# FrozenWolf-Cyber/Indic-CL-ASR

Hardware: AMD Instinct MI355X
Metric: utterances/sec (15 s @16 kHz) Conformer-M RNNT-CTC+EWC train step (higher is better)
Workload: dtype bf16; 1 GPU; BASELINE configs[1]: Conformer-medium (d=256, 16L, H=640) hybrid RNNT-CTC + EWC, bs=32/GPU x 15 s, bf16 projections, freeze_encoder_till=12, 22x257 heads, fused_batch_size=4; global_batch=32, parallelism=dp1

## Files before the change

include/indicasr.h:

```cpp
#ifndef INDICASR_H
#define INDICASR_H

#include <stddef.h>
#include <stdint.h>

#ifdef __cplusplus
extern "C" {
#endif

typedef void* ia_stream_t;

enum ia_status {
    IA_OK = 0,
    IA_INVALID_VALUE = -1,
    IA_WORKSPACE_TOO_SMALL = -2,
    IA_LAUNCH_FAILED = -3,
    IA_UNSUPPORTED = -4,
};

const char* ia_version(void);

size_t ia_rnnt_workspace_bytes(int B, int T, int U1);
int ia_rnnt_loss(const float* logits, const int64_t* labels, const int64_t* act_lens, const int64_t* label_lens,
                 int B, int T, int U1, int V, int blank, float fastemit_lambda, float clamp,
                 float* costs, float* grads, void* workspace, size_t workspace_bytes, ia_stream_t stream);
int ia_rnnt_forward(const float* logits, const int64_t* labels, const int64_t* act_lens, const int64_t* label_lens,
                    int B, int T, int U1, int V, int blank, float fastemit_lambda, int need_backward, float* costs,
                    void* workspace, size_t workspace_bytes, ia_stream_t stream);
int ia_rnnt_backward(const float* logits, const int64_t* labels, const int64_t* act_lens, const int64_t* label_lens,
                     int B, int T, int U1, int V, int blank, float fastemit_lambda, float clamp,
                     const float* cost_grad, float* grads, void* workspace, size_t workspace_bytes, ia_stream_t stream,
                     void* grad_kernel_start_event, void* grad_kernel_stop_event);
int ia_rnnt_export_alphas_betas(const void* workspace, size_t workspace_bytes, const int64_t* act_lens,
                                const int64_t* label_lens, int B, int T, int U1, float* alphas, float* betas,
                                ia_stream_t stream);

int ia_joint_ld(int V);
int ia_joint_fwd(const void* f, const void* g, const void* W, const float* bias, const int64_t* labels,
                 const int64_t* act_lens, const int64_t* label_lens, int B, int T, int U1, int H, int V, int blank,
                 float dropout_p, unsigned seed, void* logits, int LD, void* workspace, size_t workspace_bytes,
                 ia_stream_t stream);
int ia_joint_fwd_box(const void* f, const void* g, const void* W, const float* bias, const int64_t* labels,
                     const int64_t* act_lens, const int64_t* label_lens, const int64_t* box_t, const int64_t* box_u, int B,
                     int T, int U1, int H, int V, int blank, float dropout_p, unsigned seed, void* logits, int LD,
                     void* workspace, size_t workspace_bytes, ia_stream_t stream);
int64_t ia_joint_extra_scratch_elems(void);
int ia_joint_extra_reduce(const void* logits, const void* teacher, const int64_t* box_t, const int64_t* box_u,
                          const float* w_sq, const float* w_kd, int B, int T, int U1, int V, int LD, float* sums4,
                          float* scratch, ia_stream_t stream);
int ia_joint_extra_grad(const void* logits, const void* teacher, const int64_t* box_t, const int64_t* box_u, const float* w_sq,
                        const float* w_kd, const float* upstream2, int B, int T, int U1, int V, int LD, void* E,
                        ia_stream_t stream);
int ia_lattice_add_f16(void* G, const void* E, int64_t n, ia_stream_t stream);
int ia_rnnt_lattice(const int64_t* act_lens, const int64_t* label_lens, int B, int T, int U1, float fastemit_lambda,
                    int need_backward, float* costs, void* workspace, size_t workspace_bytes, ia_stream_t stream);
int ia_joint_backward_g(void* logits_inout, const int64_t* labels, const int64_t* act_lens, const int64_t* label_lens,
                        int B, int T, int U1, int V, int LD, int blank, float fastemit_lambda, const float* cost_grad,
                        float kappa, void* gt_out, int S, int Kc, float* dbias_out, float* dbias_scratch, void* workspace,
                        size_t workspace_bytes, ia_stream_t stream, void* grad_kernel_start_event,
                        void* grad_kernel_stop_event);
int ia_joint_backward_g_skip(void* logits_inout, const int64_t* labels, const int64_t* act_lens, const int64_t* label_lens, int B,
                             int T, int U1, int V, int LD, int blank, float fastemit, const float* cost_grad, float kappa,
                             void* gt_out, int S, int Kc, float* dbias_out, float* dbias_scratch, void* workspace,
                             size_t workspace_bytes, int skip_dead_frames, ia_stream_t stream, void* ev_start, void* ev_stop);
int64_t ia_joint_backward_g_dbias_scratch_elems(int LD);
int ia_joint_hidden_t(const void* f, const void* g, void* hidden_t, int B, int T, int U1, int H, int LDH, int S, int Kc,
                      float dropout_p, unsigned seed, ia_stream_t stream);
int ia_joint_hidden(const void* f, const void* g, void* hidden, int B, int T, int U1, int H, int LDH, float dropout_p,
                    unsigned seed, ia_stream_t stream);
int ia_joint_dh_reduce(const void* dh, const void* f, const void* g, const int64_t* act_lens,
                       const int64_t* label_lens, float* df, float* dg, int B, int T, int U1, int H, float inv_kappa,
                       float dropout_p, unsigned seed, void* scratch, ia_stream_t stream);
size_t ia_joint_dh_reduce_scratch_bytes(int B, int T, int U1, int H);
int ia_joint_dh_fused_supported(int U1, int H, int LD);
int ia_joint_dh_k(void);
size_t ia_joint_dh_fused_scratch_bytes(int B, int T, int U1, int H);
int ia_joint_dh_fused(const void* G, const void* Wt, const void* f, const void* g, const int64_t* act_lens,
                      const int64_t* label_lens, float* df, float* dg, int B, int T, int U1, int H, int LD,
                      float inv_kappa, float dropout_p, unsigned seed, void* scratch, ia_stream_t stream);
int ia_joint_dh_fused_ex(const void* G, const void* Wt, const void* f, const void* g, const int64_t* act_lens,
                         const int64_t* label_lens, float* df, float* dg, void* df_bf16, void* dg_bf16, int zero_dead_df, int B,
                         int T, int U1, int H, int LD, float inv_kappa, float dropout_p, unsigned seed, void* scratch,
                         ia_stream_t stream);
int ia_joint_dw_fused_supported(int U1, int H, int LD);
int64_t ia_joint_dw_fused_scratch_elems(int B, int T, int U1, int H, int LD);
int ia_joint_dw_fused(const void* G, const void* f, const void* g, const int64_t* act_lens, int B, int T, int U1, int H, int LD,
                      float dropout_p, unsigned seed, float* dW, float* scratch, ia_stream_t stream);
int ia_joint_dw_fused_ex(const void* G, const void* f, const void* g, const int64_t* act_lens, const int64_t* label_lens, int B,
                         int T, int U1, int H, int LD, float dropout_p, unsigned seed, float* dW, float* scratch,
                         ia_stream_t stream);

int ia_gemm_bf16(const void* A, int lda, const void* W, int ldw, int M, int N, int K, const float* bias, int act,
                 float dropout_p, unsigned seed, float alpha, const float* R, int ldr, float* outF, int ldof,
                 void* outH, int ldoh, ia_stream_t stream);
int ia_gemm_bf16_ex(const void* A, int lda, const void* W, int ldw, int M, int N, int K, const float* bias, int act,
                    float dropout_p, unsigned seed, float alpha, const float* R, int ldr, float* outF, int ldof, void* outH,
                    int ldoh, void* out_pre, int ldpre, const void* aux, int ldaux, ia_stream_t stream);
int ia_gemm_bf16_ex2(const void* A, int lda, const void* W, int ldw, int M, int N, int K, const float* bias, int act,
                     float dropout_p, unsigned seed, float alpha, const float* R, int ldr, float* outF, int ldof, void* outH,
                     int ldoh, void* out_pre, int ldpre, const void* aux, int ldaux, int flags, ia_stream_t stream);
int ia_quantize_mxfp8(const void* x, int is_f32, int ld, int64_t M, int K, void* q, int ldq, void* scales, int lds, ia_stream_t stream);
int ia_gemm_mxfp8(const void* Aq, int lda, const void* a_scales, int ldsa, const void* Wq, int ldw, const void* w_scales, int ldsw,
                  int M, int N, int K, const float* bias, int act, float dropout_p, unsigned seed, float alpha, const float* R, int ldr,
                  float* outF, int ldof, void* outH, int ldoh, ia_stream_t stream);

int ia_greedy_decode_lds_bytes(int Hp, int Hj, int V);
int ia_greedy_rnnt_decode(const float* f_all, const int64_t* out_len, const float* EW, const float* Whh, const float* Wpred,
                          const float* bpred, const float* Whead, const float* bhead, int B, int T, int Hp, int Hj, int V,
                          int blank, int row_blank, int row_sos, int max_symbols, int* tokens, int cap, int* counts,
                          int* overflow, ia_stream_t stream);
int ia_greedy_rnnt_decode_bf16w(const float* f_all, const int64_t* out_len, const float* EW, const void* Whh_bf16,
                                const void* Wpred_bf16, const float* bpred, const void* Whead_bf16, const float* bhead, int B, int T,
                                int Hp, int Hj, int V, int blank, int row_blank, int row_sos, int max_symbols, int* tokens, int cap,
                                int* counts, int* overflow, ia_stream_t stream);
size_t ia_greedy_decode_scratch_bytes(int B, int Hp, int Hj);
int ia_greedy_decode_cluster(int B, int Hp, int Hj);
int ia_greedy_rnnt_decode_bf16w_ex(const float* f_all, const int64_t* out_len, const float* EW, const void* Whh_bf16,
                                   const void* Wpred_bf16, const float* bpred, const void* Whead_bf16, const float* bhead, int B,
                                   int T, int Hp, int Hj, int V, int blank, int row_blank, int row_sos, int max_symbols, int* tokens,
                                   int cap, int* counts, int* overflow, int cluster, void* scratch, size_t scratch_bytes,
                                   ia_stream_t stream);

int ia_edit_distance_batch(const int32_t* a, const int64_t* a_off, const int32_t* b, const int64_t* b_off, int n, int64_t* out);

int ia_quantize_fp8_rows(const void* x, int is_f32, int ld, int64_t M, int K, void* q, int ldq, float* scale, ia_stream_t stream);
int ia_gemm_fp8(const void* Aq, int lda, const float* a_scale, const void* Wq, int ldw, const float* w_scale, int M, int N, int K,
                const float* bias, int act, float dropout_p, unsigned seed, float alpha, const float* R, int ldr, float* outF,
                int ldof, void* outH, int ldoh, ia_stream_t stream);
int ia_subsample_conv1(const float* feats, int B, int Fm, int Tm, int C, const float* w1, const float* b1, void* out,
                       ia_stream_t stream);
int ia_subsample_conv2(const void* in_cl, int B, int T1, int F1, int C, const void* w2r, const float* b2, int N, void* out,
                       ia_stream_t stream);
int ia_gemm_bf16_ln_supported(int N, int K);
int ia_gemm_bf16_ln(const void* A, int lda, const void* W, int ldw, int M, int N, int K, const float* bias, float dropout_p,
                    unsigned seed, float alpha, const float* R, int ldr, float* outF, int ldof, const float* ln_g,
                    const float* ln_b, float ln_eps, void* outH, int ldoh, ia_stream_t stream);
int ia_layernorm(const float* x, int ldx, int N, int d, const float* g1, const float* b1, float eps, float* outF,
                 int ldf, const float* g2, const float* b2, void* outH, int ldh, ia_stream_t stream);
int ia_glu_dwconv(const void* x2, const int64_t* lens, int B, int T, int d, int ksz, const float* w, const float* bias,
                  float* z, float* bn_sum, float* bn_sumsq, float* scratch, ia_stream_t stream);
int64_t ia_dwconv_scratch_elems(int B, int T, int d, int ksz);
int ia_colsum_bf16(const void* x, int M, int N, int ld, float* out, ia_stream_t stream);
int ia_dwconv_time(const float* x, int B, int T, int d, int ksz, const float* w, const float* bias, int flip, float* y,
                   ia_stream_t stream);
int ia_dwconv_time_wgrad(const float* x, const float* dy, int B, int T, int d, int ksz, float* dw, float* db,
                         float* scratch, ia_stream_t stream);
int ia_dwconv_glu_bwd(const float* dz, const void* c2, const int64_t* lens, int B, int T, int d, int ksz, const float* w, void* dc2,
                      ia_stream_t stream);
int ia_dwconv_glu_wgrad(const void* c2, const int64_t* lens, const float* dy, int B, int T, int d, int ksz, float* dw, float* db,
                        float* scratch, ia_stream_t stream);
int ia_bn_silu(const float* z, int64_t n_rows, int d, const float* bn_sum, const float* bn_sumsq, const float* gamma,
               const float* beta, float* running_mean, float* running_var, int64_t* num_batches_tracked,
               float momentum, float eps, int training, void* out, ia_stream_t stream);

int ia_gemm_bnsilu_supported(int K);
int ia_gemm_bnsilu_bf16(const float* z, int ldz, int64_t n_rows, const float* bn_sum, const float* bn_sumsq,
                        const float* gamma, const float* beta, float* running_mean, float* running_var,
                        int64_t* num_batches_tracked, float momentum, float eps, int training, const void* W, int ldw, int M,
                        int N, int K, const float* bias, float dropout_p, unsigned seed, float alpha, const float* R, int ldr,
                        float* outF, int ldof, void* outH, int ldoh, const long long* bn_sums_fixed, ia_stream_t stream);
int ia_gemm_bnsilu_bf16_keep(const float* z, int ldz, int64_t n_rows, const float* bn_sum, const float* bn_sumsq,
                             const float* gamma, const float* beta, float* running_mean, float* running_var,
                             int64_t* num_batches_tracked, float momentum, float eps, int training, const void* W, int ldw, int M,
                             int N, int K, const float* bias, float dropout_p, unsigned seed, float alpha, const float* R, int ldr,
                             float* outF, int ldof, void* outH, int ldoh, const long long* bn_sums_fixed, void* outA, int ldoa,
                             ia_stream_t stream);
int ia_dwconv_gated_fixed(const void* g, const int64_t* lens, int B, int T, int d, int ksz, const float* w, const float* bias,
                          float* z, long long* bn_sums_fixed, ia_stream_t stream);
int ia_glu_dwconv_fixed(const void* x2, const int64_t* lens, int B, int T, int d, int ksz, const float* w, const float* bias,
                        float* z, long long* bn_sums_fixed, ia_stream_t stream);

int ia_relpos_attention_flash_supported(int T, int dk);
int ia_relpos_attention_flash(const void* qkv, const void* pos_proj, const float* bias_u, const float* bias_v,
                              const int64_t* lens, int B, int T, int H, int dk, float dropout_p, unsigned seed, void* ctx,
                              ia_stream_t stream);
int ia_relpos_attention_flash_lse(const void* qkv, const void* pos_proj, const float* bias_u, const float* bias_v,
                                  const int64_t* lens, int B, int T, int H, int dk, float dropout_p, unsigned seed, void* ctx,
                                  float* lse, ia_stream_t stream);
int ia_relpos_attention_flash_bwd_dims(int T, int* Rs, int* pad0);
int64_t ia_relpos_attention_flash_bwd_ws_elems(int B, int T, int H, int dk);
int ia_relpos_attention_flash_bwd(const void* qkv, const void* pos_proj, const float* bias_u, const float* bias_v,
                                  const int64_t* lens, const void* ctx, const void* dctx, const float* lse, int B, int T, int H,
                                  int dk, float dropout_p, unsigned seed, void* dqkv, void* dpl, int pl_rows, float* dbias_u,
                                  float* dbias_v, void* dBand, void* QvHM, float* ws, ia_stream_t stream);
size_t ia_attn_vt_elems(int B, int T, int H);
int ia_relpos_attention(const void* qkv, const void* pos_proj, const float* bias_u, const float* bias_v,
                        const int64_t* lens, int B, int T, int H, int dk, float dropout_p, unsigned seed,
                        void* vt_scratch, void* ctx, ia_stream_t stream);

size_t ia_lstm_scratch_bytes(int B, int H);
int ia_lstm_lds_bytes(int H, int backward);
int ia_lstm_forward(const float* Gx, const void* Whh_bf16, float* Hout, float* gates, float* Cs, int U, int B, int H,
                    void* scratch, size_t scratch_bytes, ia_stream_t stream);
int ia_lstm_backward(const float* dHout, const float* gates, const float* Cs, const void* WhhT_bf16, float* dG, int U,
                     int B, int H, void* scratch, size_t scratch_bytes, ia_stream_t stream);

int ia_feat_frames(const float* audio, int B, int L, int Tm, int win, int n_fft, int hop, float preemph, float dither,
                   unsigned seed, float* frames, int ldf, ia_stream_t stream);
int ia_gemm_f32(const float* A, int lda, const float* W, int ldw, int M, int N, int K, float* C, int ldc,
                ia_stream_t stream);
int ia_feat_power(const float* spec, int64_t M, int lds, int half, int nbins, float* power, int ldp, ia_stream_t stream);
int ia_feat_logmel_t(const float* mel, int B, int Tm, int F, int ldm, float guard, float* out, ia_stream_t stream);
int ia_feat_preemph(const float* audio, int B, int L, float preemph, float dither, unsigned seed, float* y,
                    ia_stream_t stream);
int ia_feat_logmel_fft_supported(int n_fft, int win, int n_mels, int n_chunks);
int ia_feat_logmel_fft(const float* y, int B, int L, int Tm, const float* window, int win, int n_fft, int hop,
                       const float* twiddle, const int* chunk_start, const float* chunk_vals, const int* filt_chunks,
                       int n_mels, int n_chunks, float guard, float* out, ia_stream_t stream);
int ia_feat_normalize(const float* x, const int64_t* seq_len, int B, int F, int T, float eps, const int* freq_starts,
                      const int* freq_widths, int n_freq_masks, const int* time_starts, const int* time_widths,
                      int n_time_masks, float mask_value, float* y, ia_stream_t stream);

size_t ia_ctc_workspace_bytes(int B, int T, int S);
int ia_ctc_forward(const float* log_probs, const int64_t* targets, const int64_t* input_lens, const int64_t* target_lens,
                   int B, int T, int V, int S, int blank, int zero_infinity, float* nll, void* workspace,
                   size_t workspace_bytes, ia_stream_t stream);
int ia_ctc_backward(const float* log_probs, const int64_t* targets, const int64_t* input_lens, const int64_t* target_lens,
                    int B, int T, int V, int S, int blank, const float* nll_grad, float* grad, void* workspace,
                    size_t workspace_bytes, ia_stream_t stream);

typedef struct ia_tn_problem {
    const void* dY; const void* X; float* dW; float* db;
    int ldy, ldx, M, n, k;
} ia_tn_problem;
int64_t ia_gemm_tn_grouped_scratch_elems(const ia_tn_problem* problems, int count);
int ia_gemm_tn_bf16_grouped(const ia_tn_problem* problems, int count, float* scratch, ia_stream_t stream);
int64_t ia_gemm_tn_scratch_elems(int M, int n, int k);
int ia_gemm_tn_bf16(const void* dY, int ldy, const void* X, int ldx, int M, int n, int k, float* dW, float* db,
                    float* scratch, ia_stream_t stream);

int ia_ffn_fused_supported(int d, int d_ff);
int ia_ffn_fused(float* x, int N, int d, int d_ff, const float* ln_g, const float* ln_b, float eps, const void* W1,
                 const float* b1, const void* W2, const float* b2, float alpha, float p_ff, unsigned seed_ff, float p_res,
                 unsigned seed_res, const float* ln2_g, const float* ln2_b, void* y_out, int ln2_to_y_only,
                 ia_stream_t stream);
int ia_ffn_fused_tail_supported(int d, int d_ff, int nt);
int ia_ffn_fused_tail(float* x, int N, int d, int d_ff, const float* ln_g, const float* ln_b, float eps, const void* W1,
                      const float* b1, const void* W2, const float* b2, float alpha, float p_ff, unsigned seed_ff, float p_res,
                      unsigned seed_res, const float* ln2_g, const float* ln2_b, void* y_out, int ln2_to_y_only, const void* Wt,
                      const float* bt, void* t_out, int nt, ia_stream_t stream);

typedef struct ia_block_params {
    const void *w_ff1a, *w_ff1b, *w_qkv, *w_pos, *w_out, *w_pw1, *w_pw2, *w_ff2a, *w_ff2b;
    const float *b_ff1a, *b_ff1b, *b_qkv, *b_out, *b_pw1, *b_pw2, *b_ff2a, *b_ff2b;
    const float *ln_ff1_g, *ln_ff1_b, *ln_att_g, *ln_att_b, *ln_conv_g, *ln_conv_b, *ln_ff2_g, *ln_ff2_b, *ln_out_g, *ln_out_b;
    const float *pos_u, *pos_v, *dw_w, *dw_b, *bn_g, *bn_b;
    float *bn_rm, *bn_rv;
    int64_t* bn_nbt;
    float ln_eps, bn_eps, bn_momentum, p_drop, p_ff, p_att, fc_factor;
    int d, d_ff, n_heads, ksz;
    const void* pl_cached;
    const void* w_pw1_glu;
    const float* b_pw1_glu;
} ia_block_params;
size_t ia_conformer_prefix_ws_bytes(int B, int T, int d, int d_ff, int H, int ksz, int pos_rows);
int ia_conformer_prefix_fwd(const ia_block_params* layers, int n_layers, float* x, const void* pos_emb, int pos_rows,
                            const int64_t* lens, int B, int T, unsigned seed_base, unsigned seed_stride, int training,
                            void* workspace, size_t workspace_bytes, ia_stream_t stream);
size_t ia_conformer_prefix_ws_sums_offset(int B, int T, int d, int d_ff, int H, int ksz, int pos_rows);
int ia_conformer_prefix_fwd_seg(const ia_block_params* layers, int n_layers, float* x, const void* pos_emb, int pos_rows,
                                const int64_t* lens, int B, int T, unsigned seed_base, unsigned seed_stride, int training,
                                int seg_begin, int seg_end, int bn_synced, void* workspace, size_t workspace_bytes,
                                ia_stream_t stream);

typedef struct ia_block_saved {
    void *y1, *h1p, *h1; float* x1;
    void *y2, *qkv, *pl, *ctxv; float* x2;
    void *y3, *c2; float *z, *sums; void* c3; float* x3;
    void *y4, *h4p, *h4; float* x4;
    float* lse;
} ia_block_saved;
typedef struct ia_block_grads {
    float *w_ff1a, *b_ff1a, *w_ff1b, *b_ff1b, *w_qkv, *b_qkv, *w_pos, *w_out, *b_out, *w_pw1, *b_pw1, *w_pw2, *b_pw2;
    float *w_ff2a, *b_ff2a, *w_ff2b, *b_ff2b;
    float *ln_ff1_g, *ln_ff1_b, *ln_att_g, *ln_att_b, *ln_conv_g, *ln_conv_b, *ln_ff2_g, *ln_ff2_b, *ln_out_g, *ln_out_b;
    float *dw_w, *dw_b, *bn_g, *bn_b;
} ia_block_grads;
struct ia_block_params;
int ia_conformer_block_supported(int d, int d_ff, int H, int ksz, int T);
size_t ia_conformer_block_bwd_ws_bytes(int B, int T, int d, int d_ff, int ksz);
int ia_conformer_block_fwd(const struct ia_block_params* layer, const float* x0, const void* pos_emb, int pos_rows,
                           const int64_t* lens, int B, int T, unsigned seed, const ia_block_saved* saved, float* out,
                           float* dw_scratch, ia_stream_t stream);
int ia_conformer_block_bwd_a(const struct ia_block_params* layer, const ia_block_saved* saved, const ia_block_grads* grads,
                             const float* dout, const int64_t* lens, int B, int T, unsigned seed, void* workspace,
                             size_t workspace_bytes, float** dx2_out, void** dctx_out, ia_stream_t stream);
int ia_conformer_block_fwd_phase(const struct ia_block_params* layer, const float* x0, const void* pos_emb, int pos_rows,
                                 const int64_t* lens, int B, int T, unsigned seed, const ia_block_saved* saved, float* out,
                                 float* dw_scratch, int phase, ia_stream_t stream);
int ia_conformer_block_bwd_a_phase(const struct ia_block_params* layer, const ia_block_saved* saved, const ia_block_grads* grads,
                                   const float* dout, const int64_t* lens, int B, int T, unsigned seed, void* workspace,
                                   size_t workspace_bytes, float** dx2_out, void** dctx_out, int phase, const float* bn_S12,
                                   ia_stream_t stream);
int ia_conformer_block_bwd_b(const struct ia_block_params* layer, const ia_block_saved* saved, const ia_block_grads* grads,
                             const float* x0, const void* pos_emb, int pos_rows, const void* dqkv, const void* dpl, int B,
                             int T, unsigned seed, void* workspace, size_t workspace_bytes, float* dx0,
                             const void* add_table, int n_add, ia_stream_t stream);

int ia_layernorm_bwd(const float* x, int ldx, const float* dy_f32, const void* dy_bf16, int ldy, int N, int d,
                     const float* gamma, float eps, const float* dx_in, float* dx_out, int lddx, float* dgamma,
                     float* dbeta, float* scratch, ia_stream_t stream);
int ia_layernorm_bwd_drop(const float* x, int ldx, const float* dy_f32, const void* dy_bf16, int ldy, int N, int d,
                          const float* gamma, float eps, const float* dx_in, float* dx_out, int lddx, float* dgamma,
                          float* dbeta, float alpha, float dropout_p, unsigned seed, void* dx_bf16, int lddxh, float* scratch,
                          ia_stream_t stream);
typedef struct ia_finish_job { const float* part; int G, C, C0; float* out0; float* out1; } ia_finish_job;
int ia_layernorm_bwd_partial_rows(int N);
int ia_partials_finish_multi(const ia_finish_job* jobs, int count, ia_stream_t stream);
int64_t ia_layernorm_bwd_scratch_elems(int N, int d);
int ia_silu_dropout(const void* h_pre, int64_t M, int N, float dropout_p, unsigned seed, void* out, ia_stream_t stream);
int ia_silu_dropout_bwd(const void* h_pre, const void* dh, int64_t M, int N, float dropout_p, unsigned seed, void* out,
                        ia_stream_t stream);
int ia_scale_dropout_bf16(const float* dy, int64_t M, int N, float alpha, float dropout_p, unsigned seed, void* out,
                          ia_stream_t stream);
int ia_cast_pad_bf16(const float* src, int lds, int64_t M, int N, void* dst, int ldd, ia_stream_t stream);
int ia_bn_silu_bwd(const float* z, const void* dc3, int64_t n_rows, int d, const float* bn_sum, const float* bn_sumsq,
                   const float* gamma, const float* beta, float eps, float* S1, float* S2, float* dz, float* scratch,
                   ia_stream_t stream);
int64_t ia_bn_silu_bwd_scratch_elems(int64_t n_rows, int d);
int ia_bn_sync_finish(float* sums_and_count, int d, int64_t n_local_rows, float* running_mean, float* running_var,
                      int64_t* num_batches_tracked, float momentum, ia_stream_t stream);
int ia_bn_silu_bwd_reduce(const float* z, const void* dc3, int64_t n_rows, int d, const float* bn_sum, const float* bn_sumsq,
                          const float* gamma, const float* beta, float eps, float* S1, float* S2, float* scratch,
                          ia_stream_t stream);
int ia_bn_silu_bwd_apply(const float* z, const void* dc3, int64_t n_rows, int d, const float* bn_sum, const float* bn_sumsq,
                         const float* gamma, const float* beta, float eps, const float* S1, const float* S2, float* dz,
                         ia_stream_t stream);
int ia_glu_mask(const void* c2, const int64_t* lens, int B, int T, int d, float* G, ia_stream_t stream);
int ia_glu_bwd(const void* c2, const float* dG, const int64_t* lens, int B, int T, int d, void* dc2, ia_stream_t stream);

int ia_cl_chunk_elems(void);
int ia_cl_penalty(const float* theta, const float* theta_star, const float* weight, float coef, float* grad,
                  int accumulate, const int32_t* chunk_table, int nchunks, const float* seg_inv_numel,
                  float* seg_abs_mean, float* penalty_sum, ia_stream_t stream);
int ia_cl_fisher_accumulate(float* fisher, const float* grad, const float* loss_scalar, int64_t n, ia_stream_t stream);
int ia_cl_abs_accumulate(float* omega, const float* grad, int64_t n, ia_stream_t stream);
int ia_adamw_step(float* theta, const float* grad, float* exp_avg, float* exp_avg_sq, int64_t n, float lr, float beta1,
                  float beta2, float eps, float weight_decay, int step, float grad_scale, void* shadow_bf16,
                  ia_stream_t stream);
int ia_adamw_step_segmented(float* theta, const float* grad, float* exp_avg, float* exp_avg_sq, const int32_t* chunk_table,
                            int nchunks, int32_t* seg_active, int32_t* seg_step, int nseg, int all_active, float lr,
                            float beta1, float beta2, float eps, float weight_decay, float grad_scale, void* shadow_bf16,
                            ia_stream_t stream);
size_t ia_grad_norm_workspace_bytes(int nchunks);
int ia_grad_norm(const float* grad, const int32_t* chunk_table, int nchunks, const int32_t* seg_chunk_begin, int nseg,
                 float grad_scale, float max_norm, int32_t* seg_active, float* seg_norm, float* norm_state, void* workspace,
                 size_t workspace_bytes, ia_stream_t stream);
int ia_adamw_step_segmented_clipped(float* theta, const float* grad, float* exp_avg, float* exp_avg_sq,
                                    const int32_t* chunk_table, int nchunks, int32_t* seg_active, int32_t* seg_step, int nseg,
                                    int all_active, float lr, float beta1, float beta2, float eps, float weight_decay,
                                    float grad_scale, void* shadow_bf16, const float* norm_state, int skip_nonfinite,
                                    int32_t* counters, ia_stream_t stream);
int ia_adamw_step_segmented_si(float* theta, const float* grad, float* exp_avg, float* exp_avg_sq, const int32_t* chunk_table,
                               int nchunks, int32_t* seg_active, int32_t* seg_step, int nseg, int all_active, float lr,
                               float beta1, float beta2, float eps, float weight_decay, float grad_scale, void* shadow_bf16,
                               const float* norm_state, int skip_nonfinite, int32_t* counters, float* path_w,
                               const float* omega, const float* theta_star, float penalty_coef, ia_stream_t stream);
int ia_si_consolidate(const float* theta, float* theta_star, float* path_w, float* omega, float xi, int64_t n,
                      ia_stream_t stream);
size_t ia_agem_workspace_bytes(int nchunks);
int ia_agem_dots(const float* grad, const float* ref, const int32_t* chunk_table, int nchunks, int nseg, float grad_scale,
                 int32_t* seg_active, float* proj_state, void* workspace, size_t workspace_bytes, ia_stream_t stream);
int ia_grad_norm_projected(const float* grad, const int32_t* chunk_table, int nchunks, const int32_t* seg_chunk_begin, int nseg,
                           float grad_scale, float max_norm, const int32_t* seg_active, float* seg_norm, float* norm_state,
                           void* workspace, size_t workspace_bytes, const float* ref, const float* proj_state,
                           ia_stream_t stream);
int ia_adamw_step_segmented_projected(float* theta, const float* grad, float* exp_avg, float* exp_avg_sq,
                                      const int32_t* chunk_table, int nchunks, int32_t* seg_active, int32_t* seg_step, int nseg,
                                      int all_active, float lr, float beta1, float beta2, float eps, float weight_decay,
                                      float grad_scale, void* shadow_bf16, const float* norm_state, int skip_nonfinite,
                                      int32_t* counters, const float* ref, const float* proj_state, int32_t* proj_counters,
                                      ia_stream_t stream);
#define IA_GEM_MAX_TASKS 16
#define IA_GEM_STATE_FLOATS 20
#define IA_GEM_SUMS_DOUBLES 272
size_t ia_gem_workspace_bytes(int nchunks, int max_tasks);
int ia_gem_dots(const float* x, const float* refs, int64_t stride, int ntasks, const int32_t* chunk_table, int nchunks, int nseg,
                float grad_scale, int32_t* seg_active, int gram_row, double* gem_sums, void* workspace, size_t workspace_bytes,
                ia_stream_t stream);
int ia_gem_solve(const double* gem_sums, float* gem_state, int ntasks, float memory_strength, float eps, ia_stream_t stream);
int ia_grad_norm_gem(const float* grad, const int32_t* chunk_table, int nchunks, const int32_t* seg_chunk_begin, int nseg,
                     float grad_scale, float max_norm, const int32_t* seg_active, float* seg_norm, float* norm_state,
                     void* workspace, size_t workspace_bytes, const float* refs, int64_t stride, int ntasks,
                     const float* gem_state, ia_stream_t stream);
int ia_adamw_step_segmented_gem(float* theta, const float* grad, float* exp_avg, float* exp_avg_sq, const int32_t* chunk_table,
                                int nchunks, int32_t* seg_active, int32_t* seg_step, int nseg, int all_active, float beta1,
                                float beta2, float eps, float grad_scale, void* shadow_bf16, const int32_t* seg_group, int ngroups,
                                const float* group_lr, const float* group_weight_decay, const float* norm_state,
                                int skip_nonfinite, int32_t* counters, const float* refs, int64_t stride, int ntasks,
                                const float* gem_state, int32_t* gem_counters, ia_stream_t stream);
#define IA_MAX_PARAM_GROUPS 64
int ia_adamw_step_segmented_grouped(float* theta, const float* grad, float* exp_avg, float* exp_avg_sq,
                                    const int32_t* chunk_table, int nchunks, int32_t* seg_active, int32_t* seg_step, int nseg,
                                    int all_active, float beta1, float beta2, float eps, float grad_scale, void* shadow_bf16,
                                    const int32_t* seg_group, int ngroups, const float* group_lr,
                                    const float* group_weight_decay, const float* norm_state, int skip_nonfinite,
                                    int32_t* counters, float* path_w, const float* omega, const float* theta_star,
                                    float penalty_coef, const float* ref, const float* proj_state, int32_t* proj_counters,
                                    ia_stream_t stream);
#define IA_MASK_FREE 0
#define IA_MASK_MASKED 1
#define IA_MASK_FROZEN 2
int ia_adamw_step_segmented_masked(float* theta, const float* grad, float* exp_avg, float* exp_avg_sq, const int32_t* chunk_table,
                                   int nchunks, int32_t* seg_active, int32_t* seg_step, int nseg, int all_active, float beta1,
                                   float beta2, float eps, float grad_scale, void* shadow_bf16, const int32_t* seg_group,
                                   int ngroups, const float* group_lr, const float* group_weight_decay, const float* norm_state,
                                   int skip_nonfinite, int32_t* counters, const float* base, float* scores,
                                   const int32_t* seg_kind, float threshold, ia_stream_t stream);
int ia_mask_pack(const float* scores, const int32_t* chunk_table, int nchunks, const int32_t* seg_kind, int nseg, float threshold,
                 uint64_t* bits, int64_t nwords, int32_t* seg_kept, ia_stream_t stream);
int ia_mask_apply(float* theta, const float* base, const uint64_t* bits, int64_t nwords, const int32_t* chunk_table, int nchunks,
                  const int32_t* seg_kind, int nseg, void* shadow_bf16, ia_stream_t stream);
int ia_adamw_step_segmented_packed(float* theta, const float* grad, float* exp_avg, float* exp_avg_sq, const int32_t* chunk_table,
                                   int nchunks, int32_t* seg_active, int32_t* seg_step, int nseg, int all_active, float beta1,
                                   float beta2, float eps, float grad_scale, void* shadow_bf16, const int32_t* seg_group,
                                   int ngroups, const float* group_lr, const float* group_weight_decay, const float* norm_state,
                                   int skip_nonfinite, int32_t* counters, const uint8_t* owner, const int32_t* seg_kind,
                                   int train_owner, ia_stream_t stream);
int ia_grad_norm_packed(const float* grad, const int32_t* chunk_table, int nchunks, const int32_t* seg_chunk_begin, int nseg,
                        float grad_scale, float max_norm, int32_t* seg_active, float* seg_norm, float* norm_state,
                        void* workspace, size_t workspace_bytes, const uint8_t* owner, const int32_t* seg_kind, int train_owner,
                        ia_stream_t stream);
size_t ia_pack_prune_workspace_bytes(int nseg);
int ia_pack_prune(float* theta, float* exp_avg, float* exp_avg_sq, uint8_t* owner, const int32_t* chunk_table, int nchunks,
                  const int32_t* seg_kind, int nseg, float fraction, int task, void* shadow_bf16, int32_t* seg_counts,
                  void* workspace, size_t workspace_bytes, ia_stream_t stream);
int ia_pack_apply(float* theta, const float* base, const uint8_t* owner, const int32_t* chunk_table, int nchunks,
                  const int32_t* seg_kind, int nseg, int lo, int hi, void* shadow_bf16, ia_stream_t stream);

int ia_ctc_row_lse(const float* logits, int ld, int64_t M, int V, float* lse, ia_stream_t stream);
int ia_ctc_forward_logits(const float* logits, int ld, const float* lse, const int64_t* targets, const int64_t* input_lens,
                          const int64_t* target_lens, int B, int T, int V, int S, int blank, int zero_infinity, float* nll,
                          void* workspace, size_t workspace_bytes, ia_stream_t stream);
int ia_ctc_backward_logits(const float* logits, int ld, const float* lse, const int64_t* targets, const int64_t* input_lens,
                           const int64_t* target_lens, int B, int T, int V, int S, int blank, const float* nll_grad,
                           float grad_scale, void* grad_bf16, int ldg, void* workspace, size_t workspace_bytes, ia_stream_t stream);

typedef struct ia_axpy_row {
    float* dst; const float* src; long long n; float scale; int pad;
} ia_axpy_row;
typedef struct ia_tr_job { const void* in; void* out; int rows, cols; } ia_tr_job;
int ia_transpose16_multi(const ia_tr_job* jobs_host, int njobs, ia_stream_t stream);
int ia_swap01_cast(const void* in, int in_bf16, int n0, int n1, int H, void* out, int out_bf16, ia_stream_t stream);
int ia_select_rows_cast(const float* W, int ldw, const float* bias, int row0, int nrows, int extra_row, int K, int rows_out,
                        float scale, int out_f16, void* out, void* outT, int ldt, float* bias_out, ia_stream_t stream);
int ia_rows_scatter_add(float* dst, int ldd, const float* src, int lds, int row0, int nrows, int extra_row, int K, float scale,
                        float* bias_dst, const float* bias_src, ia_stream_t stream);
int ia_loss_combine(const float* costs, const float* nll, int B, float ctc_weight, const int* flag0, const int* flag1,
                    const int* flag2, const int* flag3, float* out4, float* total, ia_stream_t stream);
int ia_loss_combine_bwd(const float* gout, int B, float ctc_weight, float* g_costs, float* g_nll, ia_stream_t stream);
int ia_embed_sos(const float* E, const int64_t* tokens, int B, int U, int H, int n_rows, int time_major, int out_bf16, void* out,
                 ia_stream_t stream);
int ia_embed_sos_bwd(const void* dX, int dx_bf16, const int64_t* tokens, int B, int U, int H, int n_rows, int pad_row,
                     int time_major, float scale, float* dE, ia_stream_t stream);
int ia_multi_axpy(const ia_axpy_row* rows_host, int nrows, int max_blocks_per_row, ia_stream_t stream);

int ia_peak_stream_copy(const void* src, void* dst, size_t bytes, ia_stream_t stream);
int ia_peak_mfma_bf16(float* sink, int workgroups, int iters, ia_stream_t stream);
double ia_peak_mfma_bf16_flops(int workgroups, int iters);

#ifdef __cplusplus
}
#endif
#endif
```

indic_cl_asr_amd/_lib.py:

```python
import ctypes
import os
import subprocess

_HERE = os.path.dirname(os.path.abspath(__file__))
LIB_PATH = os.environ.get("IA_LIB_PATH") or os.path.join(_HERE, "libindicasr_hip.so")

IA_OK = 0
_STATUS = {-1: "IA_INVALID_VALUE", -2: "IA_WORKSPACE_TOO_SMALL", -3: "IA_LAUNCH_FAILED", -4: "IA_UNSUPPORTED"}

_c = ctypes
_vp, _i, _f, _sz = _c.c_void_p, _c.c_int, _c.c_float, _c.c_size_t
_i64 = _c.c_int64

class BlockParams(_c.Structure):
    _fields_ = ([(n, _c.c_void_p) for n in (
        "w_ff1a", "w_ff1b", "w_qkv", "w_pos", "w_out", "w_pw1", "w_pw2", "w_ff2a", "w_ff2b",
        "b_ff1a", "b_ff1b", "b_qkv", "b_out", "b_pw1", "b_pw2", "b_ff2a", "b_ff2b",
        "ln_ff1_g", "ln_ff1_b", "ln_att_g", "ln_att_b", "ln_conv_g", "ln_conv_b", "ln_ff2_g", "ln_ff2_b", "ln_out_g", "ln_out_b",
        "pos_u", "pos_v", "dw_w", "dw_b", "bn_g", "bn_b", "bn_rm", "bn_rv", "bn_nbt")]
        + [(n, _c.c_float) for n in ("ln_eps", "bn_eps", "bn_momentum", "p_drop", "p_ff", "p_att", "fc_factor")]
        + [(n, _c.c_int) for n in ("d", "d_ff", "n_heads", "ksz")]
        + [("pl_cached", _c.c_void_p), ("w_pw1_glu", _c.c_void_p), ("b_pw1_glu", _c.c_void_p)])


class BlockSaved(_c.Structure):
    _fields_ = [(n, _c.c_void_p) for n in ("y1", "h1p", "h1", "x1", "y2", "qkv", "pl", "ctxv", "x2", "y3", "c2", "z", "sums",
                                           "c3", "x3", "y4", "h4p", "h4", "x4", "lse")]


class TnProblem(_c.Structure):
    _fields_ = [("dY", _c.c_void_p), ("X", _c.c_void_p), ("dW", _c.c_void_p), ("db", _c.c_void_p),
                ("ldy", _c.c_int), ("ldx", _c.c_int), ("M", _c.c_int), ("n", _c.c_int), ("k", _c.c_int)]


class BlockGrads(_c.Structure):
    _fields_ = [(n, _c.c_void_p) for n in (
        "w_ff1a", "b_ff1a", "w_ff1b", "b_ff1b", "w_qkv", "b_qkv", "w_pos", "w_out", "b_out", "w_pw1", "b_pw1", "w_pw2", "b_pw2",
        "w_ff2a", "b_ff2a", "w_ff2b", "b_ff2b",
        "ln_ff1_g", "ln_ff1_b", "ln_att_g", "ln_att_b", "ln_conv_g", "ln_conv_b", "ln_ff2_g", "ln_ff2_b", "ln_out_g", "ln_out_b",
        "dw_w", "dw_b", "bn_g", "bn_b")]


SIGNATURES = {
    "ia_version": (_c.c_char_p, []),
    "ia_gemm_bf16_ex2": (_i, [_vp, _i, _vp, _i, _i, _i, _i, _vp, _i, _f, _c.c_uint, _f, _vp, _i, _vp, _i, _vp, _i, _vp, _i, _vp, _i, _i, _vp]),
    "ia_transpose16_multi": (_i, [_vp, _i, _vp]),
    "ia_swap01_cast": (_i, [_vp, _i, _i, _i, _i, _vp, _i, _vp]),
    "ia_ctc_row_lse": (_i, [_vp, _i, _i64, _i, _vp, _vp]),
    "ia_ctc_forward_logits": (_i, [_vp, _i, _vp, _vp, _vp, _vp, _i, _i, _i, _i, _i, _i, _vp, _vp, _sz, _vp]),
    "ia_ctc_backward_logits": (_i, [_vp, _i, _vp, _vp, _vp, _vp, _i, _i, _i, _i, _i, _vp, _f, _vp, _i, _vp, _sz, _vp]),
    "ia_select_rows_cast": (_i, [_vp, _i, _vp, _i, _i, _i, _i, _i, _f, _i, _vp, _vp, _i, _vp, _vp]),
    "ia_rows_scatter_add": (_i, [_vp, _i, _vp, _i, _i, _i, _i, _i, _f, _vp, _vp, _vp]),
    "ia_loss_combine": (_i, [_vp, _vp, _i, _f, _vp, _vp, _vp, _vp, _vp, _vp, _vp]),
    "ia_loss_combine_bwd": (_i, [_vp, _i, _f, _vp, _vp, _vp]),
    "ia_embed_sos": (_i, [_vp, _vp, _i, _i, _i, _i, _i, _i, _vp, _vp]),
    "ia_embed_sos_bwd": (_i, [_vp, _i, _vp, _i, _i, _i, _i, _i, _i, _f, _vp, _vp]),
    "ia_multi_axpy": (_i, [_vp, _i, _i, _vp]),
    "ia_peak_stream_copy": (_i, [_vp, _vp, _sz, _vp]),
    "ia_peak_mfma_bf16": (_i, [_vp, _i, _i, _vp]),
    "ia_peak_mfma_bf16_flops": (_c.c_double, [_i, _i]),
    "ia_rnnt_workspace_bytes": (_sz, [_i, _i, _i]),
    "ia_rnnt_loss": (_i, [_vp, _vp, _vp, _vp, _i, _i, _i, _i, _i, _f, _f, _vp, _vp, _vp, _sz, _vp]),
    "ia_rnnt_forward": (_i, [_vp, _vp, _vp, _vp, _i, _i, _i, _i, _i, _f, _i, _vp, _vp, _sz, _vp]),
    "ia_rnnt_backward": (_i, [_vp, _vp, _vp, _vp, _i, _i, _i, _i, _i, _f, _f, _vp, _vp, _vp, _sz, _vp, _vp, _vp]),
    "ia_rnnt_export_alphas_betas": (_i, [_vp, _sz, _vp, _vp, _i, _i, _i, _vp, _vp, _vp]),
    "ia_joint_ld": (_i, [_i]),
    "ia_joint_fwd": (_i, [_vp, _vp, _vp, _vp, _vp, _vp, _vp, _i, _i, _i, _i, _i, _i, _f, _c.c_uint, _vp, _i, _vp, _sz, _vp]),
    "ia_joint_fwd_box": (_i, [_vp, _vp, _vp, _vp, _vp, _vp, _vp, _vp, _vp, _i, _i, _i, _i, _i, _i, _f, _c.c_uint, _vp, _i, _vp, _sz, _vp]),
    "ia_joint_extra_scratch_elems": (_i64, []),
    "ia_joint_extra_reduce": (_i, [_vp, _vp, _vp, _vp, _vp, _vp, _i, _i, _i, _i, _i, _vp, _vp, _vp]),
    "ia_joint_extra_grad": (_i, [_vp, _vp, _vp, _vp, _vp, _vp, _vp, _i, _i, _i, _i, _i, _vp, _vp]),
    "ia_lattice_add_f16": (_i, [_vp, _vp, _i64, _vp]),
    "ia_relpos_attention_flash_lse": (_i, [_vp, _vp, _vp, _vp, _vp, _i, _i, _i, _i, _f, _c.c_uint, _vp, _vp, _vp]),
    "ia_relpos_attention_flash_bwd_dims": (_i, [_i, _c.POINTER(_c.c_int), _c.POINTER(_c.c_int)]),
    "ia_relpos_attention_flash_bwd_ws_elems": (_i64, [_i, _i, _i, _i]),
    "ia_relpos_attention_flash_bwd": (_i, [_vp, _vp, _vp, _vp, _vp, _vp, _vp, _vp, _i, _i, _i, _i, _f, _c.c_uint, _vp, _vp, _i, _vp,
                                           _vp, _vp, _vp, _vp, _vp]),
    "ia_quantize_fp8_rows": (_i, [_vp, _i, _i, _i64, _i, _vp, _i, _vp, _vp]),
    "ia_gemm_fp8": (_i, [_vp, _i, _vp, _vp, _i, _vp, _i, _i, _i, _vp, _i, _f, _c.c_uint, _f, _vp, _i, _vp, _i, _vp, _i, _vp]),
    "ia_gemm_tn_grouped_scratch_elems": (_i64, [_vp, _i]),
    "ia_gemm_tn_bf16_grouped": (_i, [_vp, _i, _vp, _vp]),
    "ia_greedy_decode_lds_bytes": (_i, [_i, _i, _i]),
    "ia_greedy_rnnt_decode": (_i, [_vp, _vp, _vp, _vp, _vp, _vp, _vp, _vp, _i, _i, _i, _i, _i, _i, _i, _i, _i, _vp, _i, _vp, _vp, _vp]),
    "ia_greedy_rnnt_decode_bf16w": (_i, [_vp, _vp, _vp, _vp, _vp, _vp, _vp, _vp, _i, _i, _i, _i, _i, _i, _i, _i, _i, _vp, _i, _vp, _vp, _vp]),
    "ia_edit_distance_batch": (_i, [_vp, _vp, _vp, _vp, _i, _vp]),
    "ia_greedy_decode_scratch_bytes": (_sz, [_i, _i, _i]),
    "ia_greedy_decode_cluster": (_i, [_i, _i, _i]),
    "ia_greedy_rnnt_decode_bf16w_ex": (_i, [_vp, _vp, _vp, _vp, _vp, _vp, _vp, _vp, _i, _i, _i, _i, _i, _i, _i, _i, _i, _vp, _i, _vp, _vp, _i, _vp, _sz, _vp]),
    "ia_quantize_mxfp8": (_i, [_vp, _i, _i, _i64, _i, _vp, _i, _vp, _i, _vp]),
    "ia_gemm_mxfp8": (_i, [_vp, _i, _vp, _i, _vp, _i, _vp, _i, _i, _i, _i, _vp, _i, _f, _c.c_uint, _f, _vp, _i, _vp, _i, _vp, _i, _vp]),
    "ia_cast_pad_bf16": (_i, [_vp, _i, _i64, _i, _vp, _i, _vp]),
    "ia_rnnt_lattice": (_i, [_vp, _vp, _i, _i, _i, _f, _i, _vp, _vp, _sz, _vp]),
    "ia_joint_backward_g": (_i, [_vp, _vp, _vp, _vp, _i, _i, _i, _i, _i, _i, _f, _vp, _f, _vp, _i, _i, _vp, _vp, _vp, _sz, _vp, _vp,
                                 _vp]),
    "ia_joint_backward_g_skip": (_i, [_vp, _vp, _vp, _vp, _i, _i, _i, _i, _i, _i, _f, _vp, _f, _vp, _i, _i, _vp, _vp, _vp, _sz, _i, _vp,
                                      _vp, _vp]),
    "ia_joint_backward_g_dbias_scratch_elems": (_i64, [_i]),
    "ia_joint_hidden_t": (_i, [_vp, _vp, _vp, _i, _i, _i, _i, _i, _i, _i, _f, _c.c_uint, _vp]),
    "ia_joint_hidden": (_i, [_vp, _vp, _vp, _i, _i, _i, _i, _i, _f, _c.c_uint, _vp]),
    "ia_joint_dh_reduce": (_i, [_vp, _vp, _vp, _vp, _vp, _vp, _vp, _i, _i, _i, _i, _f, _f, _c.c_uint, _vp, _vp]),
    "ia_joint_dh_reduce_scratch_bytes": (_sz, [_i, _i, _i, _i]),
    "ia_joint_dh_fused_supported": (_i, [_i, _i, _i]),
    "ia_joint_dh_k": (_i, []),
    "ia_joint_dh_fused": (_i, [_vp, _vp, _vp, _vp, _vp, _vp, _vp, _vp, _i, _i, _i, _i, _i, _f, _f, _c.c_uint, _vp, _vp]),
    "ia_joint_dh_fused_ex": (_i, [_vp, _vp, _vp, _vp, _vp, _vp, _vp, _vp, _vp, _vp, _i, _i, _i, _i, _i, _i, _f, _f, _c.c_uint, _vp, _vp]),
    "ia_joint_dh_fused_scratch_bytes": (_sz, [_i, _i, _i, _i]),
    "ia_joint_dw_fused_supported": (_i, [_i, _i, _i]),
    "ia_joint_dw_fused_scratch_elems": (_i64, [_i, _i, _i, _i, _i]),
    "ia_joint_dw_fused": (_i, [_vp, _vp, _vp, _vp, _i, _i, _i, _i, _i, _f, _c.c_uint, _vp, _vp, _vp]),
    "ia_gemm_bf16_ln_supported": (_i, [_i, _i]),
    "ia_gemm_bf16_ln": (_i, [_vp, _i, _vp, _i, _i, _i, _i, _vp, _f, _c.c_uint, _f, _vp, _i, _vp, _i, _vp, _vp, _f, _vp, _i, _vp]),
    "ia_joint_dw_fused_ex": (_i, [_vp, _vp, _vp, _vp, _vp, _i, _i, _i, _i, _i, _f, _c.c_uint, _vp, _vp, _vp]),
    "ia_gemm_bf16": (_i, [_vp, _i, _vp, _i, _i, _i, _i, _vp, _i, _f, _c.c_uint, _f, _vp, _i, _vp, _i, _vp, _i, _vp]),
    "ia_gemm_bf16_ex": (_i, [_vp, _i, _vp, _i, _i, _i, _i, _vp, _i, _f, _c.c_uint, _f, _vp, _i, _vp, _i, _vp, _i, _vp, _i, _vp, _i, _vp]),
    "ia_subsample_conv1": (_i, [_vp, _i, _i, _i, _i, _vp, _vp, _vp, _vp]),
    "ia_subsample_conv2": (_i, [_vp, _i, _i, _i, _i, _vp, _vp, _i, _vp, _vp]),
    "ia_layernorm": (_i, [_vp, _i, _i, _i, _vp, _vp, _f, _vp, _i, _vp, _vp, _vp, _i, _vp]),
    "ia_glu_dwconv": (_i, [_vp, _vp, _i, _i, _i, _i, _vp, _vp, _vp, _vp, _vp, _vp, _vp]),
    "ia_dwconv_scratch_elems": (_i64, [_i, _i, _i, _i]),
    "ia_colsum_bf16": (_i, [_vp, _i, _i, _i, _vp, _vp]),
    "ia_dwconv_time": (_i, [_vp, _i, _i, _i, _i, _vp, _vp, _i, _vp, _vp]),
    "ia_dwconv_time_wgrad": (_i, [_vp, _vp, _i, _i, _i, _i, _vp, _vp, _vp, _vp]),
    "ia_dwconv_glu_bwd": (_i, [_vp, _vp, _vp, _i, _i, _i, _i, _vp, _vp, _vp]),
    "ia_dwconv_glu_wgrad": (_i, [_vp, _vp, _vp, _i, _i, _i, _i, _vp, _vp, _vp, _vp]),
    "ia_bn_silu": (_i, [_vp, _i64, _i, _vp, _vp, _vp, _vp, _vp, _vp, _vp, _f, _f, _i, _vp, _vp]),
    "ia_gemm_bnsilu_supported": (_i, [_i]),
    "ia_gemm_bnsilu_bf16": (_i, [_vp, _i, _i64, _vp, _vp, _vp, _vp, _vp, _vp, _vp, _f, _f, _i, _vp, _i, _i, _i, _i, _vp, _f, _c.c_uint, _f,
                                 _vp, _i, _vp, _i, _vp, _i, _vp, _vp]),
    "ia_gemm_bnsilu_bf16_keep": (_i, [_vp, _i, _i64, _vp, _vp, _vp, _vp, _vp, _vp, _vp, _f, _f, _i, _vp, _i, _i, _i, _i, _vp, _f, _c.c_uint,
                                      _f, _vp, _i, _vp, _i, _vp, _i, _vp, _vp, _i, _vp]),
    "ia_glu_dwconv_fixed": (_i, [_vp, _vp, _i, _i, _i, _i, _vp, _vp, _vp, _vp, _vp]),
    "ia_dwconv_gated_fixed": (_i, [_vp, _vp, _i, _i, _i, _i, _vp, _vp, _vp, _vp, _vp]),
    "ia_attn_vt_elems": (_sz, [_i, _i, _i]),
    "ia_relpos_attention": (_i, [_vp, _vp, _vp, _vp, _vp, _i, _i, _i, _i, _f, _c.c_uint, _vp, _vp, _vp]),
    "ia_relpos_attention_flash_supported": (_i, [_i, _i]),
    "ia_relpos_attention_flash": (_i, [_vp, _vp, _vp, _vp, _vp, _i, _i, _i, _i, _f, _c.c_uint, _vp, _vp]),
    "ia_lstm_scratch_bytes": (_sz, [_i, _i]),
    "ia_lstm_lds_bytes": (_i, [_i, _i]),
    "ia_lstm_forward": (_i, [_vp, _vp, _vp, _vp, _vp, _i, _i, _i, _vp, _sz, _vp]),
    "ia_lstm_backward": (_i, [_vp, _vp, _vp, _vp, _vp, _i, _i, _i, _vp, _sz, _vp]),
    "ia_feat_frames": (_i, [_vp, _i, _i, _i, _i, _i, _i, _f, _f, _c.c_uint, _vp, _i, _vp]),
    "ia_gemm_f32": (_i, [_vp, _i, _vp, _i, _i, _i, _i, _vp, _i, _vp]),
    "ia_feat_power": (_i, [_vp, _i64, _i, _i, _i, _vp, _i, _vp]),
    "ia_feat_logmel_t": (_i, [_vp, _i, _i, _i, _i, _f, _vp, _vp]),
    "ia_feat_preemph": (_i, [_vp, _i, _i, _f, _f, _c.c_uint, _vp, _vp]),
    "ia_feat_logmel_fft_supported": (_i, [_i, _i, _i, _i]),
    "ia_feat_logmel_fft": (_i, [_vp, _i, _i, _i, _vp, _i, _i, _i, _vp, _vp, _vp, _vp, _i, _i, _f, _vp, _vp]),
    "ia_feat_normalize": (_i, [_vp, _vp, _i, _i, _i, _f, _vp, _vp, _i, _vp, _vp, _i, _f, _vp, _vp]),
    "ia_ctc_workspace_bytes": (_sz, [_i, _i, _i]),
    "ia_ctc_forward": (_i, [_vp, _vp, _vp, _vp, _i, _i, _i, _i, _i, _i, _vp, _vp, _sz, _vp]),
    "ia_ctc_backward": (_i, [_vp, _vp, _vp, _vp, _i, _i, _i, _i, _i, _vp, _vp, _vp, _sz, _vp]),
    "ia_gemm_tn_scratch_elems": (_i64, [_i, _i, _i]),
    "ia_gemm_tn_bf16": (_i, [_vp, _i, _vp, _i, _i, _i, _i, _vp, _vp, _vp, _vp]),
    "ia_ffn_fused_supported": (_i, [_i, _i]),
    "ia_ffn_fused": (_i, [_vp, _i, _i, _i, _vp, _vp, _f, _vp, _vp, _vp, _vp, _f, _f, _c.c_uint, _f, _c.c_uint, _vp, _vp, _vp, _i, _vp]),
    "ia_ffn_fused_tail_supported": (_i, [_i, _i, _i]),
    "ia_ffn_fused_tail": (_i, [_vp, _i, _i, _i, _vp, _vp, _f, _vp, _vp, _vp, _vp, _f, _f, _c.c_uint, _f, _c.c_uint, _vp, _vp, _vp, _i,
                               _vp, _vp, _vp, _i, _vp]),
    "ia_conformer_prefix_ws_bytes": (_sz, [_i, _i, _i, _i, _i, _i, _i]),
    "ia_conformer_prefix_ws_sums_offset": (_sz, [_i, _i, _i, _i, _i, _i, _i]),
    "ia_conformer_prefix_fwd_seg": (_i, [_vp, _i, _vp, _vp, _i, _vp, _i, _i, _c.c_uint, _c.c_uint, _i, _i, _i, _i, _vp, _sz, _vp]),
    "ia_conformer_prefix_fwd": (_i, [_vp, _i, _vp, _vp, _i, _vp, _i, _i, _c.c_uint, _c.c_uint, _i, _vp, _sz, _vp]),
    "ia_conformer_block_supported": (_i, [_i, _i, _i, _i, _i]),
    "ia_conformer_block_bwd_ws_bytes": (_sz, [_i, _i, _i, _i, _i]),
    "ia_conformer_block_fwd": (_i, [_vp, _vp, _vp, _i, _vp, _i, _i, _c.c_uint, _vp, _vp, _vp, _vp]),
    "ia_conformer_block_fwd_phase": (_i, [_vp, _vp, _vp, _i, _vp, _i, _i, _c.c_uint, _vp, _vp, _vp, _i, _vp]),
    "ia_conformer_block_bwd_a": (_i, [_vp, _vp, _vp, _vp, _vp, _i, _i, _c.c_uint, _vp, _sz, _vp, _vp, _vp]),
    "ia_conformer_block_bwd_a_phase": (_i, [_vp, _vp, _vp, _vp, _vp, _i, _i, _c.c_uint, _vp, _sz, _vp, _vp, _i, _vp, _vp]),
    "ia_conformer_block_bwd_b": (_i, [_vp, _vp, _vp, _vp, _vp, _i, _vp, _vp, _i, _i, _c.c_uint, _vp, _sz, _vp, _vp, _i, _vp]),
    "ia_layernorm_bwd": (_i, [_vp, _i, _vp, _vp, _i, _i, _i, _vp, _f, _vp, _vp, _i, _vp, _vp, _vp, _vp]),
    "ia_layernorm_bwd_drop": (_i, [_vp, _i, _vp, _vp, _i, _i, _i, _vp, _f, _vp, _vp, _i, _vp, _vp, _f, _f, _c.c_uint, _vp, _i, _vp, _vp]),
    "ia_layernorm_bwd_partial_rows": (_i, [_i]),
    "ia_partials_finish_multi": (_i, [_vp, _i, _vp]),
    "ia_layernorm_bwd_scratch_elems": (_i64, [_i, _i]),
    "ia_silu_dropout": (_i, [_vp, _i64, _i, _f, _c.c_uint, _vp, _vp]),
    "ia_silu_dropout_bwd": (_i, [_vp, _vp, _i64, _i, _f, _c.c_uint, _vp, _vp]),
    "ia_scale_dropout_bf16": (_i, [_vp, _i64, _i, _f, _f, _c.c_uint, _vp, _vp]),
    "ia_bn_silu_bwd": (_i, [_vp, _vp, _i64, _i, _vp, _vp, _vp, _vp, _f, _vp, _vp, _vp, _vp, _vp]),
    "ia_bn_silu_bwd_scratch_elems": (_i64, [_i64, _i]),
    "ia_bn_sync_finish": (_i, [_vp, _i, _i64, _vp, _vp, _vp, _f, _vp]),
    "ia_bn_silu_bwd_reduce": (_i, [_vp, _vp, _i64, _i, _vp, _vp, _vp, _vp, _f, _vp, _vp, _vp, _vp]),
    "ia_bn_silu_bwd_apply": (_i, [_vp, _vp, _i64, _i, _vp, _vp, _vp, _vp, _f, _vp, _vp, _vp, _vp]),
    "ia_glu_mask": (_i, [_vp, _vp, _i, _i, _i, _vp, _vp]),
    "ia_glu_bwd": (_i, [_vp, _vp, _vp, _i, _i, _i, _vp, _vp]),
    "ia_cl_chunk_elems": (_i, []),
    "ia_cl_penalty": (_i, [_vp, _vp, _vp, _f, _vp, _i, _vp, _i, _vp, _vp, _vp, _vp]),
    "ia_cl_fisher_accumulate": (_i, [_vp, _vp, _vp, _i64, _vp]),
    "ia_cl_abs_accumulate": (_i, [_vp, _vp, _i64, _vp]),
    "ia_adamw_step": (_i, [_vp, _vp, _vp, _vp, _i64, _f, _f, _f, _f, _f, _i, _f, _vp, _vp]),
    "ia_adamw_step_segmented": (_i, [_vp, _vp, _vp, _vp, _vp, _i, _vp, _vp, _i, _i, _f, _f, _f, _f, _f, _f, _vp, _vp]),
    "ia_grad_norm_workspace_bytes": (_sz, [_i]),
    "ia_grad_norm": (_i, [_vp, _vp, _i, _vp, _i, _f, _f, _vp, _vp, _vp, _vp, _sz, _vp]),
    "ia_adamw_step_segmented_clipped": (_i, [_vp, _vp, _vp, _vp, _vp, _i, _vp, _vp, _i, _i, _f, _f, _f, _f, _f, _f, _vp, _vp, _i,
                                             _vp, _vp]),
    "ia_adamw_step_segmented_si": (_i, [_vp, _vp, _vp, _vp, _vp, _i, _vp, _vp, _i, _i, _f, _f, _f, _f, _f, _f, _vp, _vp, _i,
                                        _vp, _vp, _vp, _vp, _f, _vp]),
    "ia_si_consolidate": (_i, [_vp, _vp, _vp, _vp, _f, _i64, _vp]),
    "ia_agem_workspace_bytes": (_sz, [_i]),
    "ia_agem_dots": (_i, [_vp, _vp, _vp, _i, _i, _f, _vp, _vp, _vp, _sz, _vp]),
    "ia_grad_norm_projected": (_i, [_vp, _vp, _i, _vp, _i, _f, _f, _vp, _vp, _vp, _vp, _sz, _vp, _vp, _vp]),
    "ia_adamw_step_segmented_projected": (_i, [_vp, _vp, _vp, _vp, _vp, _i, _vp, _vp, _i, _i, _f, _f, _f, _f, _f, _f, _vp, _vp, _i,
                                               _vp, _vp, _vp, _vp, _vp]),
    "ia_gem_workspace_bytes": (_sz, [_i, _i]),
    "ia_gem_dots": (_i, [_vp, _vp, _i64, _i, _vp, _i, _i, _f, _vp, _i, _vp, _vp, _sz, _vp]),
    "ia_gem_solve": (_i, [_vp, _vp, _i, _f, _f, _vp]),
    "ia_grad_norm_gem": (_i, [_vp, _vp, _i, _vp, _i, _f, _f, _vp, _vp, _vp, _vp, _sz, _vp, _i64, _i, _vp, _vp]),
    "ia_adamw_step_segmented_gem": (_i, [_vp, _vp, _vp, _vp, _vp, _i, _vp, _vp, _i, _i, _f, _f, _f, _f, _vp, _vp, _i, _vp, _vp,
                                         _vp, _i, _vp, _vp, _i64, _i, _vp, _vp, _vp]),
    "ia_adamw_step_segmented_grouped": (_i, [_vp, _vp, _vp, _vp, _vp, _i, _vp, _vp, _i, _i, _f, _f, _f, _f, _vp, _vp, _i, _vp, _vp,
                                             _vp, _i, _vp, _vp, _vp, _vp, _f, _vp, _vp, _vp, _vp]),
    "ia_adamw_step_segmented_masked": (_i, [_vp, _vp, _vp, _vp, _vp, _i, _vp, _vp, _i, _i, _f, _f, _f, _f, _vp, _vp, _i, _vp, _vp,
                                            _vp, _i, _vp, _vp, _vp, _vp, _f, _vp]),
    "ia_mask_pack": (_i, [_vp, _vp, _i, _vp, _i, _f, _vp, _i64, _vp, _vp]),
    "ia_mask_apply": (_i, [_vp, _vp, _vp, _i64, _vp, _i, _vp, _i, _vp, _vp]),
    "ia_adamw_step_segmented_packed": (_i, [_vp, _vp, _vp, _vp, _vp, _i, _vp, _vp, _i, _i, _f, _f, _f, _f, _vp, _vp, _i, _vp, _vp,
                                            _vp, _i, _vp, _vp, _vp, _i, _vp]),
    "ia_grad_norm_packed": (_i, [_vp, _vp, _i, _vp, _i, _f, _f, _vp, _vp, _vp, _vp, _sz, _vp, _vp, _i, _vp]),
    "ia_pack_prune_workspace_bytes": (_sz, [_i]),
    "ia_pack_prune": (_i, [_vp, _vp, _vp, _vp, _vp, _i, _vp, _i, _f, _i, _vp, _vp, _vp, _sz, _vp]),
    "ia_pack_apply": (_i, [_vp, _vp, _vp, _vp, _i, _vp, _i, _i, _i, _vp, _vp]),
}

_lib = None


def build(verbose=False):
    out = None if verbose else subprocess.DEVNULL
    subprocess.check_call(["make", "-C", os.path.join(_HERE, "csrc")], stdout=out)


def lib():
    global _lib
    if _lib is None:
        if not os.path.exists(LIB_PATH):
            raise RuntimeError(
                f"{LIB_PATH} is missing: the HIP extension is the product path and has no fallback. "
                "Build it with `python -c 'import __graft_entry__ as g; g.build()'` or `make -C indic_cl_asr_amd/csrc`.")
        import torch
        l = ctypes.CDLL(LIB_PATH)
        for name, (res, args) in SIGNATURES.items():
            fn = getattr(l, name)
            fn.restype, fn.argtypes = res, args
        _lib = l
    return _lib


def check(status, what):
    if status != IA_OK:
        raise RuntimeError(f"{what} failed with status {status} ({_STATUS.get(status, 'unknown')})")


def version():
    return lib().ia_version().decode()


def stream_ptr():
    import torch
    return ctypes.c_void_p(torch.cuda.current_stream().cuda_stream)


def ptr(t):
    return ctypes.c_void_p(t.data_ptr()) if t is not None else None
```

indic_cl_asr_amd/csrc/block_train.hip:

```cpp
#include <hip/hip_bf16.h>
#include <hip/hip_runtime.h>

#include <cstdint>

#include <cstdlib>

#include "ia_common.h"

namespace {

inline size_t up256(size_t x) { return (x + 255) / 256 * 256; }

#define IA_TRY(call)                  \
    do {                              \
        const int rc_ = (call);       \
        if (rc_ != IA_OK) return rc_; \
    } while (0)

__global__ __launch_bounds__(256) void transpose_bf16_kernel(const unsigned short* __restrict__ in, int rows, int cols,
                                                             unsigned short* __restrict__ out) {
    __shared__ unsigned short tile[64][72];
    const int tiles_c = (cols + 63) / 64;
    const int tr = blockIdx.x / tiles_c, tc = blockIdx.x - tr * tiles_c;
    const int r0 = tr * 64, c0 = tc * 64;
    for (int i = threadIdx.x; i < 64 * 8; i += 256) {
        const int r = i >> 3, v = i & 7;
        uint4 x = make_uint4(0, 0, 0, 0);
        if (r0 + r < rows && c0 + v * 8 < cols) x = *reinterpret_cast<const uint4*>(in + (size_t)(r0 + r) * cols + c0 + v * 8);
        *reinterpret_cast<uint4*>(&tile[r][v * 8]) = x;
    }
    __syncthreads();
    for (int i = threadIdx.x; i < 64 * 8; i += 256) {
        const int c = i >> 3, v = i & 7;
        if (c0 + c < cols && r0 + v * 8 < rows) {
            union { uint4 u; unsigned short h[8]; } o;
#pragma unroll
            for (int j = 0; j < 8; ++j) o.h[j] = tile[v * 8 + j][c];
            *reinterpret_cast<uint4*>(out + (size_t)(c0 + c) * rows + r0 + v * 8) = o.u;
        }
    }
}

int transpose_bf16(const void* in, int rows, int cols, void* out, hipStream_t st) {
    if (rows % 8 != 0 || cols % 8 != 0) return IA_UNSUPPORTED;
    const int grid = ((rows + 63) / 64) * ((cols + 63) / 64);
    hipLaunchKernelGGL(transpose_bf16_kernel, dim3(grid), dim3(256), 0, st, (const unsigned short*)in, rows, cols, (unsigned short*)out);
    IA_RETURN_IF_LAUNCH_FAILED();
    return IA_OK;
}

struct TrJob { const unsigned short* in; unsigned short* out; int rows, cols, tile_begin, tiles_c; };
struct TrJobs { TrJob j[8]; int count; };
__global__ __launch_bounds__(256) void transpose_bf16_multi_kernel(TrJobs jobs) {
    __shared__ unsigned short tile[64][72];
    int ji = 0;
#pragma unroll
    for (int i = 1; i < 8; ++i)
        if (i < jobs.count && (int)blockIdx.x >= jobs.j[i].tile_begin) ji = i;
    const TrJob& J = jobs.j[ji];
    const int local = blockIdx.x - J.tile_begin;
    const int tr = local / J.tiles_c, tc = local - tr * J.tiles_c;
    const int r0 = tr * 64, c0 = tc * 64, rows = J.rows, cols = J.cols;
    for (int i = threadIdx.x; i < 64 * 8; i += 256) {
        const int r = i >> 3, v = i & 7;
        uint4 x = make_uint4(0, 0, 0, 0);
        if (r0 + r < rows && c0 + v * 8 < cols) x = *reinterpret_cast<const uint4*>(J.in + (size_t)(r0 + r) * cols + c0 + v * 8);
        *reinterpret_cast<uint4*>(&tile[r][v * 8]) = x;
    }
    __syncthreads();
    for (int i = threadIdx.x; i < 64 * 8; i += 256) {
        const int c = i >> 3, v = i & 7;
        if (c0 + c < cols && r0 + v * 8 < rows) {
            union { uint4 u; unsigned short h[8]; } o;
#pragma unroll
            for (int j = 0; j < 8; ++j) o.h[j] = tile[v * 8 + j][c];
            *reinterpret_cast<uint4*>(J.out + (size_t)(c0 + c) * rows + r0 + v * 8) = o.u;
        }
    }
}
struct TrList { TrJobs jobs; int tiles; };
inline void tr_add(TrList* l, const void* in, int rows, int cols, void* out) {
    TrJob& J = l->jobs.j[l->jobs.count++];
    J.in = (const unsigned short*)in; J.out = (unsigned short*)out; J.rows = rows; J.cols = cols;
    J.tile_begin = l->tiles; J.tiles_c = (cols + 63) / 64;
    l->tiles += ((rows + 63) / 64) * J.tiles_c;
}
int tr_launch(const TrList& l, hipStream_t st) {
    for (int i = 0; i < l.jobs.count; ++i)
        if (l.jobs.j[i].rows % 8 != 0 || l.jobs.j[i].cols % 8 != 0) return IA_UNSUPPORTED;
    hipLaunchKernelGGL(transpose_bf16_multi_kernel, dim3(l.tiles), dim3(256), 0, st, l.jobs);
    IA_RETURN_IF_LAUNCH_FAILED();
    return IA_OK;
}

struct AddRow { float* dst; const float* src; int64_t n; };
__global__ __launch_bounds__(256) void multi_add_kernel(const AddRow* __restrict__ table, int rows) {
    for (int k = blockIdx.y; k < rows; k += gridDim.y) {
        const AddRow r = table[k];
        const int64_t n4 = ((reinterpret_cast<uintptr_t>(r.dst) | reinterpret_cast<uintptr_t>(r.src)) & 15) ? 0 : (r.n >> 2);
        for (int64_t i = (int64_t)blockIdx.x * 256 + threadIdx.x; i < n4; i += (int64_t)gridDim.x * 256) {
            float4 a = reinterpret_cast<float4*>(r.dst)[i];
            const float4 b = reinterpret_cast<const float4*>(r.src)[i];
            a.x += b.x; a.y += b.y; a.z += b.z; a.w += b.w;
            reinterpret_cast<float4*>(r.dst)[i] = a;
        }
        for (int64_t i = (n4 << 2) + (int64_t)blockIdx.x * 256 + threadIdx.x; i < r.n; i += (int64_t)gridDim.x * 256) r.dst[i] += r.src[i];
    }
}

struct BwdWs {
    size_t dxa, dxb, dB, dB1, dB2, dB3, dh, dhp, dy, dc3, dz, dG, dc2, dctx, wt, scr, total;
};

size_t max3(size_t a, size_t b, size_t c) { return a > b ? (a > c ? a : c) : (b > c ? b : c); }

BwdWs bwd_ws(int B, int T, int d, int d_ff, int ksz) {
    const size_t N = (size_t)B * T;
    BwdWs w;
    size_t o = 0;
    w.dxa = o;  o = up256(o + N * d * 4);
    w.dxb = o;  o = up256(o + N * d * 4);
    w.dB = o;   o = up256(o + N * d * 2);
    w.dB1 = o;  o = up256(o + N * d * 2);
    w.dB2 = o;  o = up256(o + N * d * 2);
    w.dB3 = o;  o = up256(o + N * d * 2);
    w.dh = o;   o = up256(o + N * d_ff * 2);
    w.dhp = o;  o = up256(o + N * d_ff * 2);
    w.dy = o;   o = up256(o + N * d * 2);
    w.dc3 = o;  o = up256(o + N * d * 2);
    w.dz = o;   o = up256(o + N * d * 4);
    w.dG = o;   o = up256(o + (size_t)5 * (size_t)ia_layernorm_bwd_scratch_elems((int)N, d) * 4);
    w.dc2 = o;  o = up256(o + N * 2 * d * 2);
    w.dctx = o; o = up256(o + N * d * 2);
    w.wt = o;   o = up256(o + ((size_t)4 * d_ff * d + (size_t)7 * d * d) * 2);
    size_t scr = (size_t)ia_layernorm_bwd_scratch_elems((int)N, d);
    const int shapes[5][2] = {{d, d_ff}, {d_ff, d}, {d, d}, {2 * d, d}, {3 * d, d}};
    for (int i = 0; i < 5; ++i) {
        const size_t e = (size_t)ia_gemm_tn_scratch_elems((int)N, shapes[i][0], shapes[i][1]);
        scr = e > scr ? e : scr;
    }
    scr = max3(scr, (size_t)ia_bn_silu_bwd_scratch_elems((int64_t)N, d), (size_t)ia_dwconv_scratch_elems(B, T, d, ksz));
    {
        const ia_tn_problem ga[5] = {{nullptr, nullptr, nullptr, nullptr, d, d_ff, (int)N, d, d_ff},
                                     {nullptr, nullptr, nullptr, nullptr, d_ff, d, (int)N, d_ff, d},
                                     {nullptr, nullptr, nullptr, nullptr, d, d, (int)N, d, d},
                                     {nullptr, nullptr, nullptr, nullptr, 2 * d, d, (int)N, 2 * d, d},
                                     {nullptr, nullptr, nullptr, nullptr, d, d, (int)N, d, d}};
        const ia_tn_problem gb[4] = {{nullptr, nullptr, nullptr, nullptr, 3 * d, d, (int)N, 3 * d, d},
                                     {nullptr, nullptr, nullptr, nullptr, d, d, (int)(N > (size_t)64 * 512 ? N : (size_t)64 * 512), d, d},
                                     {nullptr, nullptr, nullptr, nullptr, d, d_ff, (int)N, d, d_ff},
                                     {nullptr, nullptr, nullptr, nullptr, d_ff, d, (int)N, d_ff, d}};
        scr = max3(scr, (size_t)ia_gemm_tn_grouped_scratch_elems(ga, 5), (size_t)ia_gemm_tn_grouped_scratch_elems(gb, 4));
        scr = max3(scr, (size_t)ia_gemm_tn_grouped_scratch_elems(gb, 2), (size_t)ia_gemm_tn_grouped_scratch_elems(gb + 2, 2));
        ia_tn_problem gall[9];
        for (int i = 0; i < 5; ++i) gall[i] = ga[i];
        for (int i = 0; i < 4; ++i) gall[5 + i] = gb[i];
        scr = scr > (size_t)ia_gemm_tn_grouped_scratch_elems(gall, 9) ? scr : (size_t)ia_gemm_tn_grouped_scratch_elems(gall, 9);
    }
    w.scr = o;  o = up256(o + scr * 4);
    w.total = o;
    return w;
}

int linear_bwd(const void* dY, const void* X, const void* W, int M, int n, int k, void* dX, float* dW, float* db, void* wt,
               float* scr, ia_stream_t stream) {
    if (dX) {
        IA_TRY(transpose_bf16(W, n, k, wt, (hipStream_t)stream));
        IA_TRY(ia_gemm_bf16(dY, n, wt, n, M, k, n, nullptr, 0, 0.f, 0, 1.f, nullptr, 0, nullptr, 0, dX, k, stream));
    }
    return ia_gemm_tn_bf16(dY, n, X, k, M, n, k, dW, db, scr, stream);
}

bool tn_grouping_enabled() {
    static const bool on = [] { const char* e = getenv("IA_TN_GROUPED"); return !(e && e[0] == '0'); }();
    return on;
}
int flush_group(const ia_tn_problem* grp, int ngrp, float* scr, ia_stream_t stream) {
    if (tn_grouping_enabled()) return ia_gemm_tn_bf16_grouped(grp, ngrp, scr, stream);
    for (int i = 0; i < ngrp; ++i)
        IA_TRY(ia_gemm_tn_bf16(grp[i].dY, grp[i].ldy, grp[i].X, grp[i].ldx, grp[i].M, grp[i].n, grp[i].k, grp[i].dW, grp[i].db, scr, stream));
    return IA_OK;
}
int linear_bwd_deferred(const void* dY, const void* X, const void* W, int M, int n, int k, void* dX, float* dW, float* db, const void* wt,
                        ia_tn_problem* grp, int* ngrp, ia_stream_t stream) {
    (void)W;
    if (dX) IA_TRY(ia_gemm_bf16(dY, n, wt, n, M, k, n, nullptr, 0, 0.f, 0, 1.f, nullptr, 0, nullptr, 0, dX, k, stream));
    grp[*ngrp] = ia_tn_problem{dY, X, dW, db, n, k, M, n, k};
    ++*ngrp;
    return IA_OK;
}

struct SideCtx {
    hipStream_t s = nullptr;
    hipEvent_t ev[8] = {};
    bool ok = false, tried = false;
    bool a_pending = false;
};
SideCtx* side_ctx() {
    static SideCtx ctx[16];
    const char* e = getenv("IA_WGRAD_SIDE");
    if (!(e && e[0] == '1')) return nullptr;
    int dev = 0;
    if (hipGetDevice(&dev) != hipSuccess || dev < 0 || dev >= 16) return nullptr;
    SideCtx& c = ctx[dev];
    if (!c.tried) {
        c.tried = true;
        bool ok = hipStreamCreateWithFlags(&c.s, hipStreamNonBlocking) == hipSuccess;
        for (int i = 0; ok && i < 8; ++i) ok = hipEventCreateWithFlags(&c.ev[i], hipEventDisableTiming) == hipSuccess;
        c.ok = ok;
    }
    return c.ok ? &c : nullptr;
}
struct PendingGroup { ia_tn_problem grp[8]; int n = 0; const void* ws = nullptr; };
PendingGroup* pending_group() {
    static PendingGroup pg[16];
    int dev = 0;
    if (hipGetDevice(&dev) != hipSuccess || dev < 0 || dev >= 16) return nullptr;
    return &pg[dev];
}
bool merged_wgrads() {
    const char* e = getenv("IA_TN_MERGE");
    return !(e && e[0] == '0') && tn_grouping_enabled();
}

int stream_after(hipStream_t from, hipStream_t to, hipEvent_t ev) {
    if (hipEventRecord(ev, from) != hipSuccess || hipStreamWaitEvent(to, ev, 0) != hipSuccess) return IA_LAUNCH_FAILED;
    return IA_OK;
}

}

extern "C" size_t ia_conformer_block_bwd_ws_bytes(int B, int T, int d, int d_ff, int ksz) {
    if (B <= 0 || T <= 0 || d <= 0 || d_ff <= 0 || ksz <= 0) return 0;
    return bwd_ws(B, T, d, d_ff, ksz).total;
}

extern "C" int ia_conformer_block_supported(int d, int d_ff, int H, int ksz, int T) {
    if (d <= 0 || H <= 0 || d % H != 0) return 0;
    const int dk = d / H;
    return (d % 8 == 0 && d <= 1024 && d_ff % 8 == 0 && ksz <= 31 && (ksz & 1) == 1 && dk <= 64 && dk % 4 == 0 && T >= 1) ? 1 : 0;
}

extern "C" int ia_conformer_block_fwd(const ia_block_params* Lp, const float* x0, const void* pos_emb, int pos_rows,
                                      const int64_t* lens, int B, int T, unsigned seed, const ia_block_saved* Sp, float* out,
                                      float* dw_scratch, ia_stream_t stream) {
    return ia_conformer_block_fwd_phase(Lp, x0, pos_emb, pos_rows, lens, B, T, seed, Sp, out, dw_scratch, 0, stream);
}

extern "C" int ia_conformer_block_fwd_phase(const ia_block_params* Lp, const float* x0, const void* pos_emb, int pos_rows,
                                            const int64_t* lens, int B, int T, unsigned seed, const ia_block_saved* Sp,
                                            float* out, float* dw_scratch, int phase, ia_stream_t stream) {
    if (phase < 0 || phase > 2) return IA_INVALID_VALUE;
    if (!Lp || !x0 || !pos_emb || !lens || !Sp || !out || !dw_scratch || B <= 0 || T <= 0) return IA_INVALID_VALUE;
    const ia_block_params& L = *Lp;
    const ia_block_saved& S = *Sp;
    const int d = L.d, d_ff = L.d_ff, H = L.n_heads, dk = d / (H > 0 ? H : 1), ksz = L.ksz, N = B * T;
    if (!ia_conformer_block_supported(d, d_ff, H, ksz, T) || pos_rows < 2 * T - 1) return IA_UNSUPPORTED;
    const float p = L.p_drop, pff = L.p_ff, patt = L.p_att;
    if (phase != 2) {
    IA_TRY(ia_layernorm(x0, d, N, d, L.ln_ff1_g, L.ln_ff1_b, L.ln_eps, nullptr, 0, nullptr, nullptr, S.y1, d, stream));
    IA_TRY(ia_gemm_bf16_ex(S.y1, d, L.w_ff1a, d, N, d_ff, d, L.b_ff1a, 1, pff, seed + 1, 1.f, nullptr, 0, nullptr, 0, S.h1, d_ff,
                           S.h1p, d_ff, nullptr, 0, stream));
    IA_TRY(ia_gemm_bf16(S.h1, d_ff, L.w_ff1b, d_ff, N, d, d_ff, L.b_ff1b, 0, p, seed + 2, L.fc_factor, x0, d, S.x1, d, nullptr, 0, stream));
    IA_TRY(ia_layernorm(S.x1, d, N, d, L.ln_att_g, L.ln_att_b, L.ln_eps, nullptr, 0, nullptr, nullptr, S.y2, d, stream));
    IA_TRY(ia_gemm_bf16(S.y2, d, L.w_qkv, d, N, 3 * d, d, L.b_qkv, 0, 0.f, 0, 1.f, nullptr, 0, nullptr, 0, S.qkv, 3 * d, stream));
    IA_TRY(ia_gemm_bf16(pos_emb, d, L.w_pos, d, pos_rows, d, d, nullptr, 0, 0.f, 0, 1.f, nullptr, 0, nullptr, 0, S.pl, d, stream));
    IA_TRY(ia_relpos_attention_flash_lse(S.qkv, S.pl, L.pos_u, L.pos_v, lens, B, T, H, dk, patt, seed + 7, S.ctxv, S.lse, stream));
    IA_TRY(ia_gemm_bf16(S.ctxv, d, L.w_out, d, N, d, d, L.b_out, 0, p, seed + 3, 1.f, S.x1, d, S.x2, d, nullptr, 0, stream));
    IA_TRY(ia_layernorm(S.x2, d, N, d, L.ln_conv_g, L.ln_conv_b, L.ln_eps, nullptr, 0, nullptr, nullptr, S.y3, d, stream));
    IA_TRY(ia_gemm_bf16(S.y3, d, L.w_pw1, d, N, 2 * d, d, L.b_pw1, 0, 0.f, 0, 1.f, nullptr, 0, nullptr, 0, S.c2, 2 * d, stream));
    IA_TRY(ia_glu_dwconv(S.c2, lens, B, T, d, ksz, L.dw_w, L.dw_b, S.z, S.sums, S.sums + d, dw_scratch, stream));
    }
    if (phase == 1) return IA_OK;
    const bool synced = phase == 2;
    if (ia_gemm_bnsilu_supported(d)) {
        IA_TRY(ia_gemm_bnsilu_bf16_keep(S.z, d, N, S.sums, S.sums + d, L.bn_g, L.bn_b, synced ? nullptr : L.bn_rm,
                                        synced ? nullptr : L.bn_rv, synced ? nullptr : L.bn_nbt, L.bn_momentum, L.bn_eps, 1, L.w_pw2,
                                        d, N, d, d, L.b_pw2, p, seed + 4, 1.f, S.x2, d, S.x3, d, nullptr, 0, nullptr, S.c3, d, stream));
    } else {
        IA_TRY(ia_bn_silu(S.z, N, d, S.sums, S.sums + d, L.bn_g, L.bn_b, synced ? nullptr : L.bn_rm, synced ? nullptr : L.bn_rv,
                          synced ? nullptr : L.bn_nbt, L.bn_momentum, L.bn_eps, 1, S.c3, stream));
        IA_TRY(ia_gemm_bf16(S.c3, d, L.w_pw2, d, N, d, d, L.b_pw2, 0, p, seed + 4, 1.f, S.x2, d, S.x3, d, nullptr, 0, stream));
    }
    IA_TRY(ia_layernorm(S.x3, d, N, d, L.ln_ff2_g, L.ln_ff2_b, L.ln_eps, nullptr, 0, nullptr, nullptr, S.y4, d, stream));
    IA_TRY(ia_gemm_bf16_ex(S.y4, d, L.w_ff2a, d, N, d_ff, d, L.b_ff2a, 1, pff, seed + 5, 1.f, nullptr, 0, nullptr, 0, S.h4, d_ff,
                           S.h4p, d_ff, nullptr, 0, stream));
    IA_TRY(ia_gemm_bf16(S.h4, d_ff, L.w_ff2b, d_ff, N, d, d_ff, L.b_ff2b, 0, p, seed + 6, L.fc_factor, S.x3, d, S.x4, d, nullptr, 0, stream));
    return ia_layernorm(S.x4, d, N, d, L.ln_out_g, L.ln_out_b, L.ln_eps, out, d, nullptr, nullptr, nullptr, 0, stream);
}

extern "C" int ia_conformer_block_bwd_a(const ia_block_params* Lp, const ia_block_saved* Sp, const ia_block_grads* Gp,
                                        const float* dout, const int64_t* lens, int B, int T, unsigned seed, void* workspace,
                                        size_t workspace_bytes, float** dx2_out, void** dctx_out, ia_stream_t stream) {
    return ia_conformer_block_bwd_a_phase(Lp, Sp, Gp, dout, lens, B, T, seed, workspace, workspace_bytes, dx2_out, dctx_out, 0, nullptr,
                                          stream);
}

extern "C" int ia_conformer_block_bwd_a_phase(const ia_block_params* Lp, const ia_block_saved* Sp, const ia_block_grads* Gp,
                                              const float* dout, const int64_t* lens, int B, int T, unsigned seed,
                                              void* workspace, size_t workspace_bytes, float** dx2_out, void** dctx_out,
                                              int phase, const float* bn_S12, ia_stream_t stream) {
    if (phase < 0 || phase > 2 || (phase == 2 && !bn_S12)) return IA_INVALID_VALUE;
    if (!Lp || !Sp || !Gp || !dout || !lens || !workspace || !dx2_out || !dctx_out || B <= 0 || T <= 0) return IA_INVALID_VALUE;
    const ia_block_params& L = *Lp;
    const ia_block_saved& S = *Sp;
    const ia_block_grads& G = *Gp;
    const int d = L.d, d_ff = L.d_ff, ksz = L.ksz, N = B * T;
    const BwdWs w = bwd_ws(B, T, d, d_ff, ksz);
    if (workspace_bytes < w.total) return IA_WORKSPACE_TOO_SMALL;
    char* ws = (char*)workspace;
    float *dxa = (float*)(ws + w.dxa), *dxb = (float*)(ws + w.dxb), *dz = (float*)(ws + w.dz), *scr = (float*)(ws + w.scr);
    float* lnp = (float*)(ws + w.dG);
    const size_t lnp_set = (size_t)ia_layernorm_bwd_scratch_elems(N, d);
    void *dB = ws + w.dB, *dB1 = ws + w.dB1, *dB2 = ws + w.dB2, *dhp = ws + w.dhp, *dy = ws + w.dy, *dc3 = ws + w.dc3, *dc2 = ws + w.dc2,
         *dctx = ws + w.dctx, *wt = ws + w.wt;
    const float p = L.p_drop, pff = L.p_ff;
    ia_tn_problem grp[8];
    int ngrp = 0;
    char* wtb = (char*)wt;
    void *wt_ff2b = wtb, *wt_ff2a = wtb + (size_t)d * d_ff * 2, *wt_pw2 = wtb + (size_t)2 * d * d_ff * 2,
         *wt_pw1 = wtb + ((size_t)2 * d * d_ff + (size_t)d * d) * 2, *wt_out = wtb + ((size_t)2 * d * d_ff + (size_t)3 * d * d) * 2;
    if (phase != 2) {
        TrList tl{};
        tr_add(&tl, L.w_ff2b, d, d_ff, wt_ff2b); tr_add(&tl, L.w_ff2a, d_ff, d, wt_ff2a); tr_add(&tl, L.w_pw2, d, d, wt_pw2);
        tr_add(&tl, L.w_pw1, 2 * d, d, wt_pw1); tr_add(&tl, L.w_out, d, d, wt_out);
        IA_TRY(tr_launch(tl, (hipStream_t)stream));
    }
    if (phase != 2) {
    IA_TRY(ia_layernorm_bwd_drop(S.x4, d, dout, nullptr, d, N, d, L.ln_out_g, L.ln_eps, nullptr, dxa, d, nullptr, nullptr,
                                 L.fc_factor, p, seed + 6, dB, d, lnp + 0 * lnp_set, stream));
    IA_TRY(ia_gemm_bf16_ex(dB, d, wt_ff2b, d, N, d_ff, d, nullptr, 3, pff, seed + 5, 1.f, nullptr, 0, nullptr, 0, dhp, d_ff, nullptr, 0,
                           S.h4p, d_ff, stream));
    IA_TRY(linear_bwd_deferred(dB, S.h4, L.w_ff2b, N, d, d_ff, nullptr, G.w_ff2b, G.b_ff2b, wt_ff2b, grp, &ngrp, stream));
    IA_TRY(linear_bwd_deferred(dhp, S.y4, L.w_ff2a, N, d_ff, d, dy, G.w_ff2a, G.b_ff2a, wt_ff2a, grp, &ngrp, stream));
    IA_TRY(ia_layernorm_bwd_drop(S.x3, d, nullptr, dy, d, N, d, L.ln_ff2_g, L.ln_eps, dxa, dxb, d, nullptr, nullptr, 1.f, p,
                                 seed + 4, dB1, d, lnp + 1 * lnp_set, stream));
    IA_TRY(linear_bwd_deferred(dB1, S.c3, L.w_pw2, N, d, d, dc3, G.w_pw2, G.b_pw2, wt_pw2, grp, &ngrp, stream));
    if (phase == 0)
        IA_TRY(ia_bn_silu_bwd(S.z, dc3, N, d, S.sums, S.sums + d, L.bn_g, L.bn_b, L.bn_eps, G.bn_b, G.bn_g, dz, scr, stream));
    else
        IA_TRY(ia_bn_silu_bwd_reduce(S.z, dc3, N, d, S.sums, S.sums + d, L.bn_g, L.bn_b, L.bn_eps, G.bn_b, G.bn_g, scr, stream));
    }
    if (phase == 1) {
        IA_TRY(flush_group(grp, ngrp, scr, stream));
        return IA_OK;
    }
    if (phase == 2)
        IA_TRY(ia_bn_silu_bwd_apply(S.z, dc3, N, d, S.sums, S.sums + d, L.bn_g, L.bn_b, L.bn_eps, bn_S12, bn_S12 + d, dz, stream));
    IA_TRY(ia_dwconv_glu_bwd(dz, S.c2, lens, B, T, d, ksz, L.dw_w, dc2, stream));
    SideCtx* side = phase == 0 ? side_ctx() : nullptr;
    hipStream_t main = (hipStream_t)stream;
    if (side) {
        IA_TRY(stream_after(main, side->s, side->ev[0]));
        IA_TRY(ia_dwconv_glu_wgrad(S.c2, lens, dz, B, T, d, ksz, G.dw_w, G.dw_b, scr, (ia_stream_t)side->s));
    } else {
        IA_TRY(ia_dwconv_glu_wgrad(S.c2, lens, dz, B, T, d, ksz, G.dw_w, G.dw_b, scr, stream));
    }
    IA_TRY(linear_bwd_deferred(dc2, S.y3, L.w_pw1, N, 2 * d, d, dy, G.w_pw1, G.b_pw1, wt_pw1, grp, &ngrp, stream));
    IA_TRY(ia_layernorm_bwd_drop(S.x2, d, nullptr, dy, d, N, d, L.ln_conv_g, L.ln_eps, dxb, dxa, d, nullptr, nullptr, 1.f, p,
                                 seed + 3, dB2, d, lnp + 2 * lnp_set, stream));
    IA_TRY(linear_bwd_deferred(dB2, S.ctxv, L.w_out, N, d, d, dctx, G.w_out, G.b_out, wt_out, grp, &ngrp, stream));
    if (side) {
        IA_TRY(stream_after(main, side->s, side->ev[1]));
        IA_TRY(flush_group(grp, ngrp, scr, (ia_stream_t)side->s));
        if (hipEventRecord(side->ev[2], side->s) != hipSuccess) return IA_LAUNCH_FAILED;
        side->a_pending = true;
    } else if (phase == 0 && merged_wgrads() && pending_group()) {
        PendingGroup* pg = pending_group();
        for (int i = 0; i < ngrp; ++i) pg->grp[i] = grp[i];
        pg->n = ngrp; pg->ws = workspace;
    } else {
        IA_TRY(flush_group(grp, ngrp, scr, stream));
    }
    *dx2_out = dxa;
    *dctx_out = dctx;
    return IA_OK;
}

extern "C" int ia_conformer_block_bwd_b(const ia_block_params* Lp, const ia_block_saved* Sp, const ia_block_grads* Gp,
                                        const float* x0, const void* pos_emb, int pos_rows, const void* dqkv, const void* dpl,
                                        int B, int T, unsigned seed, void* workspace, size_t workspace_bytes, float* dx0,
                                        const void* add_table, int n_add, ia_stream_t stream) {
    if (!Lp || !Sp || !Gp || !x0 || !pos_emb || !dqkv || !dpl || !workspace || !dx0 || B <= 0 || T <= 0) return IA_INVALID_VALUE;
    const ia_block_params& L = *Lp;
    const ia_block_saved& S = *Sp;
    const ia_block_grads& G = *Gp;
    const int d = L.d, d_ff = L.d_ff, ksz = L.ksz, N = B * T;
    const BwdWs w = bwd_ws(B, T, d, d_ff, ksz);
    if (workspace_bytes < w.total) return IA_WORKSPACE_TOO_SMALL;
    char* ws = (char*)workspace;
    float *dxa = (float*)(ws + w.dxa), *dxb = (float*)(ws + w.dxb), *scr = (float*)(ws + w.scr);
    float* lnp = (float*)(ws + w.dG);
    const size_t lnp_set = (size_t)ia_layernorm_bwd_scratch_elems(N, d);
    PendingGroup* pg = pending_group();
    const bool carried = pg && pg->n > 0 && pg->ws == workspace;
    void *dB = ws + (carried ? w.dB3 : w.dB), *dhp = ws + (carried ? w.dh : w.dhp), *dy = ws + w.dy, *wt = ws + w.wt;
    const float p = L.p_drop, pff = L.p_ff;
    ia_tn_problem grp[12];
    int ngrp = 0;
    if (carried) {
        for (int i = 0; i < pg->n; ++i) grp[ngrp++] = pg->grp[i];
        pg->n = 0;
    }
    char* wtb = (char*)wt + ((size_t)2 * d * d_ff + (size_t)4 * d * d) * 2;
    void *wt_qkv = wtb, *wt_ff1b = wtb + (size_t)3 * d * d * 2, *wt_ff1a = wtb + ((size_t)3 * d * d + (size_t)d * d_ff) * 2;
    {
        TrList tl{};
        tr_add(&tl, L.w_qkv, 3 * d, d, wt_qkv); tr_add(&tl, L.w_ff1b, d, d_ff, wt_ff1b); tr_add(&tl, L.w_ff1a, d_ff, d, wt_ff1a);
        IA_TRY(tr_launch(tl, (hipStream_t)stream));
    }
    SideCtx* side = carried ? nullptr : side_ctx();
    hipStream_t main = (hipStream_t)stream;
    IA_TRY(linear_bwd_deferred(dqkv, S.y2, L.w_qkv, N, 3 * d, d, dy, G.w_qkv, G.b_qkv, wt_qkv, grp, &ngrp, stream));
    grp[ngrp++] = ia_tn_problem{dpl, pos_emb, G.w_pos, nullptr, d, d, pos_rows, d, d};
    if (side) {
        IA_TRY(stream_after(main, side->s, side->ev[3]));
        IA_TRY(flush_group(grp, ngrp, scr, (ia_stream_t)side->s));
        ngrp = 0;
        if (side->a_pending) {
            if (hipStreamWaitEvent(main, side->ev[2], 0) != hipSuccess) return IA_LAUNCH_FAILED;
            side->a_pending = false;
        }
    }
    IA_TRY(ia_layernorm_bwd_drop(S.x1, d, nullptr, dy, d, N, d, L.ln_att_g, L.ln_eps, dxa, dxb, d, nullptr, nullptr, L.fc_factor,
                                 p, seed + 2, dB, d, lnp + 3 * lnp_set, stream));
    IA_TRY(ia_gemm_bf16_ex(dB, d, wt_ff1b, d, N, d_ff, d, nullptr, 3, pff, seed + 1, 1.f, nullptr, 0, nullptr, 0, dhp, d_ff, nullptr, 0,
                           S.h1p, d_ff, stream));
    IA_TRY(linear_bwd_deferred(dB, S.h1, L.w_ff1b, N, d, d_ff, nullptr, G.w_ff1b, G.b_ff1b, wt_ff1b, grp, &ngrp, stream));
    if (side) {
        grp[ngrp++] = ia_tn_problem{dhp, S.y1, G.w_ff1a, G.b_ff1a, d_ff, d, N, d_ff, d};
        IA_TRY(stream_after(main, side->s, side->ev[4]));
        IA_TRY(flush_group(grp, ngrp, scr, (ia_stream_t)side->s));
        ngrp = 0;
        IA_TRY(ia_gemm_bf16(dhp, d_ff, wt_ff1a, d_ff, N, d, d_ff, nullptr, 0, 0.f, 0, 1.f, nullptr, 0, nullptr, 0, dy, d, stream));
    } else {
        IA_TRY(linear_bwd_deferred(dhp, S.y1, L.w_ff1a, N, d_ff, d, dy, G.w_ff1a, G.b_ff1a, wt_ff1a, grp, &ngrp, stream));
    }
    IA_TRY(ia_layernorm_bwd(x0, d, nullptr, dy, d, N, d, L.ln_ff1_g, L.ln_eps, dxb, dx0, d, nullptr, nullptr, lnp + 4 * lnp_set, stream));
    if (side) {
        IA_TRY(stream_after(main, side->s, side->ev[5]));
        stream = (ia_stream_t)side->s;
    } else {
        IA_TRY(flush_group(grp, ngrp, scr, stream));
    }
    {
        const int rows = ia_layernorm_bwd_partial_rows(N);
        const ia_finish_job jobs[5] = {{lnp + 0 * lnp_set, rows, 2 * d, d, G.ln_out_g, G.ln_out_b},
                                       {lnp + 1 * lnp_set, rows, 2 * d, d, G.ln_ff2_g, G.ln_ff2_b},
                                       {lnp + 2 * lnp_set, rows, 2 * d, d, G.ln_conv_g, G.ln_conv_b},
                                       {lnp + 3 * lnp_set, rows, 2 * d, d, G.ln_att_g, G.ln_att_b},
                                       {lnp + 4 * lnp_set, rows, 2 * d, d, G.ln_ff1_g, G.ln_ff1_b}};
        IA_TRY(ia_partials_finish_multi(jobs, 5, stream));
    }
    if (add_table && n_add > 0) {
        hipLaunchKernelGGL(multi_add_kernel, dim3(64, n_add < 64 ? n_add : 64), dim3(256), 0, (hipStream_t)stream,
                           (const AddRow*)add_table, n_add);
        IA_RETURN_IF_LAUNCH_FAILED();
    }
    if (side) IA_TRY(stream_after(side->s, main, side->ev[6]));
    return IA_OK;
}
```

indic_cl_asr_amd/csrc/dwconv.hip:

```cpp
#include <hip/hip_bf16.h>

#include <cstdint>
#include <cstdlib>

#include "ia_common.h"
#include "indicasr.h"
#include "partials.h"

namespace {

constexpr int DW_TT = 16;
constexpr int DW_TB = 4 * DW_TT;

template <int KMAX>
__device__ __forceinline__ void load_taps(float (&wt)[KMAX], const float* __restrict__ w, int c, int ksz, int flip) {
    const int off = (KMAX - 1) / 2 - (ksz - 1) / 2;
#pragma unroll
    for (int jj = 0; jj < KMAX; ++jj) {
        const int j = jj - off;
        wt[jj] = (j >= 0 && j < ksz) ? w[c * ksz + (flip ? ksz - 1 - j : j)] : 0.f;
    }
}

template <int KMAX, int GLU>
__global__ __launch_bounds__(256) void dwconv_fwd_kernel(const void* __restrict__ xin, const int64_t* __restrict__ lens, int B,
                                                         int T, int d, int ksz, const float* __restrict__ w,
                                                         const float* __restrict__ bias, int flip, float* __restrict__ y,
                                                         float* __restrict__ part, long long* __restrict__ acc,
                                                         const __bf16* __restrict__ c2 = nullptr, __bf16* __restrict__ dc2 = nullptr) {
    constexpr int HM = (KMAX - 1) / 2, WIN = DW_TT + KMAX - 1;
    const int lane = threadIdx.x & 63, wv = threadIdx.x >> 6;
    const int ntb = (T + DW_TB - 1) / DW_TB;
    const int b = blockIdx.x / ntb, t0 = (blockIdx.x - b * ntb) * DW_TB + wv * DW_TT;
    const int c = blockIdx.y * 64 + lane;
    const bool cok = c < d;
    const int cc = cok ? c : d - 1;
    int tmax = T;
    if (GLU == 1 || GLU == 2) { const int len = (int)lens[b]; tmax = len < T ? len : T; }
    float wt[KMAX];
    load_taps<KMAX>(wt, w, cc, ksz, flip);
    float win[WIN];
#pragma unroll
    for (int r = 0; r < WIN; ++r) {
        const int t = t0 - HM + r;
        const bool ok = t >= 0 && t < tmax;
        const int tt = t < 0 ? 0 : (t >= T ? T - 1 : t);
        float v;
        if (GLU == 1) {
            const __bf16* p = reinterpret_cast<const __bf16*>(xin) + ((size_t)b * T + tt) * (2 * d);
            const float a = (float)p[cc], gate = (float)p[d + cc];
            v = a * ia_sigmoid_fast(gate);
        } else if (GLU == 2) {
            v = (float)reinterpret_cast<const __bf16*>(xin)[((size_t)b * T + tt) * d + cc];
        } else {
            v = reinterpret_cast<const float*>(xin)[((size_t)b * T + tt) * d + cc];
        }
        win[r] = ok ? v : 0.f;
    }
    const float bb = bias ? bias[cc] : 0.f;
    float s = 0.f, s2 = 0.f;
#pragma unroll
    for (int i = 0; i < DW_TT; ++i) {
        float acc = bb;
#pragma unroll
        for (int jj = 0; jj < KMAX; ++jj) acc += wt[jj] * win[i + jj];
        const int t = t0 + i;
        if (t < T && cok) {
            if (GLU == 3) {
                const size_t row = (size_t)b * T + t;
                const float av = (float)c2[row * 2 * d + c], gv = (float)c2[row * 2 * d + d + c];
                const float sg = ia_sigmoid_fast(gv);
                const float dg = (t < (int)lens[b]) ? acc : 0.f;
                dc2[row * 2 * d + c] = (__bf16)(dg * sg);
                dc2[row * 2 * d + d + c] = (__bf16)(dg * av * sg * (1.f - sg));
            } else {
                y[((size_t)b * T + t) * d + c] = acc;
                s += acc; s2 += acc * acc;
            }
        }
    }
    if (GLU == 1 || GLU == 2) {
        __shared__ float red[4][2][64];
        red[wv][0][lane] = s; red[wv][1][lane] = s2;
        __syncthreads();
        if (wv == 0 && cok) {
            const float t1 = (red[0][0][lane] + red[1][0][lane]) + (red[2][0][lane] + red[3][0][lane]);
            const float t2 = (red[0][1][lane] + red[1][1][lane]) + (red[2][1][lane] + red[3][1][lane]);
            if (acc) {
                long long* mine = acc + (size_t)(blockIdx.x & (IA_BN_ACC_COPIES - 1)) * 2 * d;
                atomicAdd(reinterpret_cast<unsigned long long*>(mine + c), (unsigned long long)__float2ll_rn(t1 * 16777216.f));
                atomicAdd(reinterpret_cast<unsigned long long*>(mine + d + c), (unsigned long long)__float2ll_rn(t2 * 16777216.f));
            } else {
                part[(size_t)blockIdx.x * 2 * d + c] = t1;
                part[(size_t)blockIdx.x * 2 * d + d + c] = t2;
            }
        }
    }
}

template <int KMAX, bool XGLU>
__global__ __launch_bounds__(256) void dwconv_wgrad_kernel(const float* __restrict__ x, const float* __restrict__ dy, int B,
                                                           int T, int d, int nsplit, float* __restrict__ part,
                                                           const __bf16* __restrict__ c2 = nullptr,
                                                           const int64_t* __restrict__ lens = nullptr) {
    constexpr int HM = (KMAX - 1) / 2, WIN = DW_TT + KMAX - 1;
    const int lane = threadIdx.x & 63, wv = threadIdx.x >> 6;
    const int b = blockIdx.x / nsplit, sp = blockIdx.x - b * nsplit;
    const int per = (((T + nsplit - 1) / nsplit + DW_TT - 1) / DW_TT) * DW_TT;
    const int ts = sp * per, te = (ts + per < T) ? ts + per : T;
    const int c = blockIdx.y * 64 + lane;
    const bool cok = c < d;
    const int cc = cok ? c : d - 1;
    float acc[KMAX];
#pragma unroll
    for (int jj = 0; jj < KMAX; ++jj) acc[jj] = 0.f;
    float sb = 0.f;
    int tlen = T;
    if constexpr (XGLU) { const int len = (int)lens[b]; tlen = len < T ? len : T; }
    for (int t0 = ts + wv * DW_TT; t0 < te; t0 += 4 * DW_TT) {
        float g[DW_TT], win[WIN];
#pragma unroll
        for (int i = 0; i < DW_TT; ++i) {
            const int t = t0 + i;
            const float v = dy[((size_t)b * T + (t < T ? t : T - 1)) * d + cc];
            g[i] = (t < te) ? v : 0.f;
        }
#pragma unroll
        for (int r = 0; r < WIN; ++r) {
            const int t = t0 - HM + r;
            const int tt = t < 0 ? 0 : (t >= T ? T - 1 : t);
            if constexpr (XGLU) {
                const size_t row = (size_t)b * T + tt;
                const float av = (float)c2[row * 2 * d + cc], gv = (float)c2[row * 2 * d + d + cc];
                win[r] = (t >= 0 && t < tlen) ? av * ia_sigmoid_fast(gv) : 0.f;
            } else {
                const float v = x[((size_t)b * T + tt) * d + cc];
                win[r] = (t >= 0 && t < T) ? v : 0.f;
            }
        }
#pragma unroll
        for (int i = 0; i < DW_TT; ++i) {
            sb += g[i];
#pragma unroll
            for (int jj = 0; jj < KMAX; ++jj) acc[jj] += g[i] * win[i + jj];
        }
    }
    __shared__ float red[3][KMAX + 1][64];
    if (wv > 0) {
#pragma unroll
        for (int jj = 0; jj < KMAX; ++jj) red[wv - 1][jj][lane] = acc[jj];
        red[wv - 1][KMAX][lane] = sb;
    }
    __syncthreads();
    if (wv == 0 && cok) {
        float* row = part + (size_t)blockIdx.x * (KMAX + 1) * d;
#pragma unroll
        for (int jj = 0; jj < KMAX; ++jj)
            row[(size_t)jj * d + c] = (acc[jj] + red[0][jj][lane]) + (red[1][jj][lane] + red[2][jj][lane]);
        row[(size_t)KMAX * d + c] = (sb + red[0][KMAX][lane]) + (red[1][KMAX][lane] + red[2][KMAX][lane]);
    }
}

__global__ __launch_bounds__(256) void dwconv_wgrad_finish_kernel(const float* __restrict__ part, int G, int d, int kmax, int ksz,
                                                                  float* __restrict__ dw, float* __restrict__ db) {
    __shared__ float red[8][32];
    const int o = threadIdx.x & 31, sl = threadIdx.x >> 5;
    const int idx = blockIdx.x * 32 + o, total = (kmax + 1) * d;
    float a0 = 0.f, a1 = 0.f;
    if (idx < total) {
        int g = sl;
        for (; g + 8 < G; g += 16) { a0 += part[(size_t)g * total + idx]; a1 += part[(size_t)(g + 8) * total + idx]; }
        for (; g < G; g += 8) a0 += part[(size_t)g * total + idx];
    }
    red[sl][o] = a0 + a1;
    __syncthreads();
    if (sl != 0 || idx >= total) return;
    const float s = ((red[0][o] + red[1][o]) + (red[2][o] + red[3][o])) + ((red[4][o] + red[5][o]) + (red[6][o] + red[7][o]));
    const int jj = idx / d, c = idx - jj * d;
    if (jj == kmax) {
        if (db) db[c] = s;
    } else {
        const int j = jj - ((kmax - 1) / 2 - (ksz - 1) / 2);
        if (j >= 0 && j < ksz) dw[c * ksz + j] = s;
    }
}

inline int kmax_for(int ksz) { return ksz <= 9 ? 9 : (ksz <= 15 ? 15 : 31); }

inline int wgrad_splits(int B, int T, int d) {
    const int cg = (d + 63) / 64;
    int ns = (768 + B * cg - 1) / (B * cg);
    const int cap = (T + DW_TB - 1) / DW_TB;
    if (ns > cap) ns = cap;
    return ns < 1 ? 1 : ns;
}

inline bool dw_shape_ok(int d, int ksz) { return d > 0 && d <= 4096 && ksz >= 1 && ksz <= 31 && (ksz & 1) == 1; }

}

extern "C" int64_t ia_dwconv_scratch_elems(int B, int T, int d, int ksz) {
    if (B <= 0 || T <= 0 || !dw_shape_ok(d, ksz)) return 0;
    const int64_t fwd = (int64_t)B * ((T + DW_TB - 1) / DW_TB) * 2 * d;
    const int64_t wg = (int64_t)B * wgrad_splits(B, T, d) * (kmax_for(ksz) + 1) * d;
    return fwd > wg ? fwd : wg;
}

extern "C" int ia_glu_dwconv(const void* x2, const int64_t* lens, int B, int T, int d, int ksz, const float* w,
                             const float* bias, float* z, float* bn_sum, float* bn_sumsq, float* scratch,
                             ia_stream_t stream) {
    if (!x2 || !lens || !w || !bias || !z || !bn_sum || !bn_sumsq || !scratch || B <= 0 || T <= 0) return IA_INVALID_VALUE;
    if (!dw_shape_ok(d, ksz)) return IA_UNSUPPORTED;
    hipStream_t st = (hipStream_t)stream;
    const dim3 grid(B * ((T + DW_TB - 1) / DW_TB), (d + 63) / 64), blk(256);
#define IA_DWF(K) hipLaunchKernelGGL((dwconv_fwd_kernel<K, 1>), grid, blk, 0, st, x2, lens, B, T, d, ksz, w, bias, 0, z, scratch, (long long*)nullptr)
    switch (kmax_for(ksz)) {
        case 9: IA_DWF(9); break;
        case 15: IA_DWF(15); break;
        default: IA_DWF(31); break;
    }
#undef IA_DWF
    IA_RETURN_IF_LAUNCH_FAILED();
    ia_partials_finish(scratch, (int)grid.x, 2 * d, d, bn_sum, bn_sumsq, st);
    IA_RETURN_IF_LAUNCH_FAILED();
    return IA_OK;
}

extern "C" int ia_glu_dwconv_fixed(const void* x2, const int64_t* lens, int B, int T, int d, int ksz, const float* w,
                                   const float* bias, float* z, long long* bn_sums_fixed, ia_stream_t stream) {
    if (!x2 || !lens || !w || !bias || !z || !bn_sums_fixed || B <= 0 || T <= 0) return IA_INVALID_VALUE;
    if (!dw_shape_ok(d, ksz)) return IA_UNSUPPORTED;
    hipStream_t st = (hipStream_t)stream;
    const dim3 grid(B * ((T + DW_TB - 1) / DW_TB), (d + 63) / 64), blk(256);
#define IA_DWF(K) hipLaunchKernelGGL((dwconv_fwd_kernel<K, 1>), grid, blk, 0, st, x2, lens, B, T, d, ksz, w, bias, 0, z, (float*)nullptr, bn_sums_fixed)
    switch (kmax_for(ksz)) {
        case 9: IA_DWF(9); break;
        case 15: IA_DWF(15); break;
        default: IA_DWF(31); break;
    }
#undef IA_DWF
    IA_RETURN_IF_LAUNCH_FAILED();
    return IA_OK;
}

extern "C" int ia_dwconv_gated_fixed(const void* g, const int64_t* lens, int B, int T, int d, int ksz, const float* w,
                                     const float* bias, float* z, long long* bn_sums_fixed, ia_stream_t stream) {
    if (!g || !lens || !w || !bias || !z || !bn_sums_fixed || B <= 0 || T <= 0) return IA_INVALID_VALUE;
    if (!dw_shape_ok(d, ksz)) return IA_UNSUPPORTED;
    hipStream_t st = (hipStream_t)stream;
    const dim3 grid(B * ((T + DW_TB - 1) / DW_TB), (d + 63) / 64), blk(256);
#define IA_DWF(K) hipLaunchKernelGGL((dwconv_fwd_kernel<K, 2>), grid, blk, 0, st, g, lens, B, T, d, ksz, w, bias, 0, z, (float*)nullptr, bn_sums_fixed)
    switch (kmax_for(ksz)) {
        case 9: IA_DWF(9); break;
        case 15: IA_DWF(15); break;
        default: IA_DWF(31); break;
    }
#undef IA_DWF
    IA_RETURN_IF_LAUNCH_FAILED();
    return IA_OK;
}

extern "C" int ia_dwconv_time(const float* x, int B, int T, int d, int ksz, const float* w, const float* bias, int flip,
                              float* y, ia_stream_t stream) {
    if (!x || !w || !y || B <= 0 || T <= 0) return IA_INVALID_VALUE;
    if (!dw_shape_ok(d, ksz)) return IA_UNSUPPORTED;
    hipStream_t st = (hipStream_t)stream;
    const dim3 grid(B * ((T + DW_TB - 1) / DW_TB), (d + 63) / 64), blk(256);
#define IA_DWF(K) hipLaunchKernelGGL((dwconv_fwd_kernel<K, 0>), grid, blk, 0, st, (const void*)x, (const int64_t*)nullptr, B, T, d, ksz, w, bias, flip, y, (float*)nullptr, (long long*)nullptr)
    switch (kmax_for(ksz)) {
        case 9: IA_DWF(9); break;
        case 15: IA_DWF(15); break;
        default: IA_DWF(31); break;
    }
#undef IA_DWF
    IA_RETURN_IF_LAUNCH_FAILED();
    return IA_OK;
}

extern "C" int ia_dwconv_time_wgrad(const float* x, const float* dy, int B, int T, int d, int ksz, float* dw, float* db,
                                    float* scratch, ia_stream_t stream) {
    if (!x || !dy || !dw || !scratch || B <= 0 || T <= 0) return IA_INVALID_VALUE;
    if (!dw_shape_ok(d, ksz)) return IA_UNSUPPORTED;
    hipStream_t st = (hipStream_t)stream;
    const int ns = wgrad_splits(B, T, d), kmax = kmax_for(ksz);
    const dim3 grid(B * ns, (d + 63) / 64), blk(256);
#define IA_DWG(K) hipLaunchKernelGGL((dwconv_wgrad_kernel<K, false>), grid, blk, 0, st, x, dy, B, T, d, ns, scratch, (const __bf16*)nullptr, (const int64_t*)nullptr)
    switch (kmax) {
        case 9: IA_DWG(9); break;
        case 15: IA_DWG(15); break;
        default: IA_DWG(31); break;
    }
#undef IA_DWG
    IA_RETURN_IF_LAUNCH_FAILED();
    hipLaunchKernelGGL(dwconv_wgrad_finish_kernel, dim3(((kmax + 1) * d + 31) / 32), dim3(256), 0, st, scratch, (int)grid.x, d,
                       kmax, ksz, dw, db);
    IA_RETURN_IF_LAUNCH_FAILED();
    return IA_OK;
}

extern "C" int ia_dwconv_glu_bwd(const float* dz, const void* c2, const int64_t* lens, int B, int T, int d, int ksz, const float* w,
                                 void* dc2, ia_stream_t stream) {
    if (!dz || !c2 || !lens || !w || !dc2 || B <= 0 || T <= 0) return IA_INVALID_VALUE;
    if (!dw_shape_ok(d, ksz)) return IA_UNSUPPORTED;
    hipStream_t st = (hipStream_t)stream;
    const dim3 grid(B * ((T + DW_TB - 1) / DW_TB), (d + 63) / 64), blk(256);
#define IA_DWF(K) hipLaunchKernelGGL((dwconv_fwd_kernel<K, 3>), grid, blk, 0, st, (const void*)dz, lens, B, T, d, ksz, w, (const float*)nullptr, 1, (float*)nullptr, (float*)nullptr, (long long*)nullptr, (const __bf16*)c2, (__bf16*)dc2)
    switch (kmax_for(ksz)) {
        case 9: IA_DWF(9); break;
        case 15: IA_DWF(15); break;
        default: IA_DWF(31); break;
    }
#undef IA_DWF
    IA_RETURN_IF_LAUNCH_FAILED();
    return IA_OK;
}

extern "C" int ia_dwconv_glu_wgrad(const void* c2, const int64_t* lens, const float* dy, int B, int T, int d, int ksz, float* dw,
                                   float* db, float* scratch, ia_stream_t stream) {
    if (!c2 || !lens || !dy || !dw || !scratch || B <= 0 || T <= 0) return IA_INVALID_VALUE;
    if (!dw_shape_ok(d, ksz)) return IA_UNSUPPORTED;
    hipStream_t st = (hipStream_t)stream;
    const int ns = wgrad_splits(B, T, d), kmax = kmax_for(ksz);
    const dim3 grid(B * ns, (d + 63) / 64), blk(256);
#define IA_DWG(K) hipLaunchKernelGGL((dwconv_wgrad_kernel<K, true>), grid, blk, 0, st, (const float*)nullptr, dy, B, T, d, ns, scratch, (const __bf16*)c2, lens)
    switch (kmax) {
        case 9: IA_DWG(9); break;
        case 15: IA_DWG(15); break;
        default: IA_DWG(31); break;
    }
#undef IA_DWG
    IA_RETURN_IF_LAUNCH_FAILED();
    hipLaunchKernelGGL(dwconv_wgrad_finish_kernel, dim3(((kmax + 1) * d + 31) / 32), dim3(256), 0, st, scratch, (int)grid.x, d,
                       kmax, ksz, dw, db);
    IA_RETURN_IF_LAUNCH_FAILED();
    return IA_OK;
}
```

indic_cl_asr_amd/csrc/encoder_bwd.hip:

```cpp
#include <hip/hip_bf16.h>

#include "dropout_mask.h"
#include <stdlib.h>

#include "ia_common.h"
#include "partials.h"

namespace {

__device__ __forceinline__ float silu_grad(float x) {
    const float s = ia_sigmoid_fast(x);
    return s * (1.f + x * (1.f - s));
}

template <int NV>
__global__ __launch_bounds__(256) void layernorm_bwd_kernel(const float* __restrict__ x, int ldx, const float* __restrict__ dyF,
                                                            const __bf16* __restrict__ dyH, int ldy, int N, int d,
                                                            const float* __restrict__ gamma, float eps,
                                                            const float* __restrict__ dx_in, float* __restrict__ dx_out,
                                                            int lddx, float* __restrict__ part, __bf16* __restrict__ dxh,
                                                            int lddxh, float hscale, unsigned hseed, unsigned hthr, float hks) {
    const int lane = threadIdx.x & 63;
    const int wave0 = blockIdx.x * 4 + (threadIdx.x >> 6), nwaves = gridDim.x * 4;
    const float inv_d = 1.f / (float)d;
    float4 gam[NV], dg[NV], db[NV];
#pragma unroll
    for (int i = 0; i < NV; ++i) {
        const int col = (lane + 64 * i) * 4;
        gam[i] = (col < d) ? *reinterpret_cast<const float4*>(gamma + col) : make_float4(0.f, 0.f, 0.f, 0.f);
        dg[i] = db[i] = make_float4(0.f, 0.f, 0.f, 0.f);
    }
    for (int row = wave0; row < N; row += nwaves) {
        float4 v[NV], g[NV];
        float s = 0.f;
#pragma unroll
        for (int i = 0; i < NV; ++i) {
            const int col = (lane + 64 * i) * 4;
            v[i] = g[i] = make_float4(0.f, 0.f, 0.f, 0.f);
            if (col < d) {
                v[i] = *reinterpret_cast<const float4*>(x + (size_t)row * ldx + col);
                if (dyF) g[i] = *reinterpret_cast<const float4*>(dyF + (size_t)row * ldy + col);
                else {
                    union { uint2 u; __bf16 h[4]; } t;
                    t.u = *reinterpret_cast<const uint2*>(dyH + (size_t)row * ldy + col);
                    g[i] = make_float4((float)t.h[0], (float)t.h[1], (float)t.h[2], (float)t.h[3]);
                }
            }
            s += v[i].x + v[i].y + v[i].z + v[i].w;
        }
        const float mean = ia_wave_sum_dpp(s) * inv_d;
        float q = 0.f;
#pragma unroll
        for (int i = 0; i < NV; ++i)
            if ((lane + 64 * i) * 4 < d) {
                const float a = v[i].x - mean, b = v[i].y - mean, c = v[i].z - mean, e = v[i].w - mean;
                q += a * a + b * b + c * c + e * e;
            }
        const float rstd = rsqrtf(ia_wave_sum_dpp(q) * inv_d + eps);
        float s1 = 0.f, s2 = 0.f;
#pragma unroll
        for (int i = 0; i < NV; ++i)
            if ((lane + 64 * i) * 4 < d) {
                v[i] = make_float4((v[i].x - mean) * rstd, (v[i].y - mean) * rstd, (v[i].z - mean) * rstd, (v[i].w - mean) * rstd);
                dg[i].x += g[i].x * v[i].x; dg[i].y += g[i].y * v[i].y; dg[i].z += g[i].z * v[i].z; dg[i].w += g[i].w * v[i].w;
                db[i].x += g[i].x; db[i].y += g[i].y; db[i].z += g[i].z; db[i].w += g[i].w;
                g[i] = make_float4(g[i].x * gam[i].x, g[i].y * gam[i].y, g[i].z * gam[i].z, g[i].w * gam[i].w);
                s1 += g[i].x + g[i].y + g[i].z + g[i].w;
                s2 += g[i].x * v[i].x + g[i].y * v[i].y + g[i].z * v[i].z + g[i].w * v[i].w;
            }
        const float m1 = ia_wave_sum_dpp(s1) * inv_d, m2 = ia_wave_sum_dpp(s2) * inv_d;
#pragma unroll
        for (int i = 0; i < NV; ++i) {
            const int col = (lane + 64 * i) * 4;
            if (col < d) {
                float4 o = make_float4(rstd * (g[i].x - m1 - v[i].x * m2), rstd * (g[i].y - m1 - v[i].y * m2),
                                       rstd * (g[i].z - m1 - v[i].z * m2), rstd * (g[i].w - m1 - v[i].w * m2));
                if (dx_in) {
                    const float4 p = *reinterpret_cast<const float4*>(dx_in + (size_t)row * lddx + col);
                    o.x += p.x; o.y += p.y; o.z += p.z; o.w += p.w;
                }
                *reinterpret_cast<float4*>(dx_out + (size_t)row * lddx + col) = o;
                if (dxh) {
                    const unsigned m = hthr > 0 ? (ia_keep8(hseed, (unsigned)row, (unsigned)d, (unsigned)(col & ~7), hthr) >> (col & 4)) : 0xFu;
                    union { uint2 u; __bf16 h[4]; } t;
                    t.h[0] = (__bf16)((m & 1u) ? o.x * hscale * hks : 0.f);
                    t.h[1] = (__bf16)((m & 2u) ? o.y * hscale * hks : 0.f);
                    t.h[2] = (__bf16)((m & 4u) ? o.z * hscale * hks : 0.f);
                    t.h[3] = (__bf16)((m & 8u) ? o.w * hscale * hks : 0.f);
                    *reinterpret_cast<uint2*>(dxh + (size_t)row * lddxh + col) = t.u;
                }
            }
        }
    }
    __shared__ float4 red[3][2][NV * 64];
    const int wv = threadIdx.x >> 6;
    if (wv > 0) {
#pragma unroll
        for (int i = 0; i < NV; ++i) { red[wv - 1][0][lane + 64 * i] = dg[i]; red[wv - 1][1][lane + 64 * i] = db[i]; }
    }
    __syncthreads();
    if (wv == 0) {
#pragma unroll
        for (int i = 0; i < NV; ++i) {
            const int col = (lane + 64 * i) * 4;
#pragma unroll
            for (int w = 0; w < 3; ++w) {
                const float4 a = red[w][0][lane + 64 * i], b = red[w][1][lane + 64 * i];
                dg[i].x += a.x; dg[i].y += a.y; dg[i].z += a.z; dg[i].w += a.w;
                db[i].x += b.x; db[i].y += b.y; db[i].z += b.z; db[i].w += b.w;
            }
            if (col < d) {
                *reinterpret_cast<float4*>(part + (size_t)blockIdx.x * 2 * d + col) = dg[i];
                *reinterpret_cast<float4*>(part + (size_t)blockIdx.x * 2 * d + d + col) = db[i];
            }
        }
    }
}

template <int MODE>
__global__ __launch_bounds__(256) void silu_dropout_kernel(const __bf16* __restrict__ a, const __bf16* __restrict__ b, int64_t M,
                                                           int N, unsigned seed, unsigned thr, float keep_scale,
                                                           __bf16* __restrict__ out) {
    const int nv = N / 8;
    const int64_t total = M * nv;
    for (int64_t i = (int64_t)blockIdx.x * 256 + threadIdx.x; i < total; i += (int64_t)gridDim.x * 256) {
        const int64_t gm = i / nv;
        const int gn = (int)(i - gm * nv) * 8;
        union { uint4 u; __bf16 h[8]; } x, y, o;
        x.u = reinterpret_cast<const uint4*>(a)[i];
        if (MODE == 1) y.u = reinterpret_cast<const uint4*>(b)[i];
        const unsigned m = thr > 0 ? ia_keep8(seed, (unsigned)gm, (unsigned)N, (unsigned)gn, thr) : 0xFFu;
#pragma unroll
        for (int j = 0; j < 8; ++j) {
            const float v = (float)x.h[j];
            float r;
            if (MODE == 0) r = ia_silu_fast(v);
            else r = (float)y.h[j] * silu_grad(v);
            o.h[j] = (__bf16)(((m >> j) & 1u) ? r * keep_scale : 0.f);
        }
        reinterpret_cast<uint4*>(out)[i] = o.u;
    }
}

__global__ __launch_bounds__(256) void scale_dropout_bf16_kernel(const float* __restrict__ dy, int64_t M, int N, float alpha,
                                                                 unsigned seed, unsigned thr, float keep_scale,
                                                                 __bf16* __restrict__ out) {
    const int nv = N / 8;
    const int64_t total = M * nv;
    for (int64_t i = (int64_t)blockIdx.x * 256 + threadIdx.x; i < total; i += (int64_t)gridDim.x * 256) {
        const int64_t gm = i / nv;
        const int gn = (int)(i - gm * nv) * 8;
        const float4 p0 = reinterpret_cast<const float4*>(dy)[2 * i], p1 = reinterpret_cast<const float4*>(dy)[2 * i + 1];
        const float v[8] = {p0.x, p0.y, p0.z, p0.w, p1.x, p1.y, p1.z, p1.w};
        const unsigned m = thr > 0 ? ia_keep8(seed, (unsigned)gm, (unsigned)N, (unsigned)gn, thr) : 0xFFu;
        union { uint4 u; __bf16 h[8]; } o;
#pragma unroll
        for (int j = 0; j < 8; ++j) o.h[j] = (__bf16)(((m >> j) & 1u) ? v[j] * alpha * keep_scale : 0.f);
        reinterpret_cast<uint4*>(out)[i] = o.u;
    }
}

__global__ __launch_bounds__(256) void bn_silu_bwd_reduce_kernel(const float* __restrict__ z, const __bf16* __restrict__ dc3,
                                                                 int64_t n_rows, int d, const float* __restrict__ bn_sum,
                                                                 const float* __restrict__ bn_sumsq, const float* __restrict__ gamma,
                                                                 const float* __restrict__ beta, float eps,
                                                                 float* __restrict__ part, int rows_per_block) {
    const int cg = d / 4, nrl = 256 / cg;
    const bool active = (int)threadIdx.x < nrl * cg;
    const int c0 = (active ? (int)threadIdx.x % cg : 0) * 4, rl = active ? (int)threadIdx.x / cg : nrl;
    const float inv_n = 1.f / (float)n_rows;
    float mean[4], rstd[4], gm[4], bt[4], a1[4] = {0, 0, 0, 0}, a2[4] = {0, 0, 0, 0};
#pragma unroll
    for (int j = 0; j < 4; ++j) {
        mean[j] = bn_sum[c0 + j] * inv_n;
        rstd[j] = rsqrtf(fmaxf(bn_sumsq[c0 + j] * inv_n - mean[j] * mean[j], 0.f) + eps);
        gm[j] = gamma[c0 + j]; bt[j] = beta[c0 + j];
    }
    const int64_t r0 = (int64_t)blockIdx.x * rows_per_block;
    const int64_t r1 = (r0 + rows_per_block < n_rows) ? r0 + rows_per_block : n_rows;
    for (int64_t r = r0 + rl; active && r < r1; r += nrl) {
        const float4 zz = *reinterpret_cast<const float4*>(z + r * d + c0);
        union { uint2 u; __bf16 h[4]; } g;
        g.u = *reinterpret_cast<const uint2*>(dc3 + r * d + c0);
        const float zv[4] = {zz.x, zz.y, zz.z, zz.w};
#pragma unroll
        for (int j = 0; j < 4; ++j) {
            const float xh = (zv[j] - mean[j]) * rstd[j];
            const float dyb = (float)g.h[j] * silu_grad(xh * gm[j] + bt[j]);
            a1[j] += dyb; a2[j] += dyb * xh;
        }
    }
    __shared__ float red[2][256][4];
#pragma unroll
    for (int j = 0; j < 4; ++j) { red[0][threadIdx.x][j] = a1[j]; red[1][threadIdx.x][j] = a2[j]; }
    __syncthreads();
    if (rl == 0) {
        for (int k = 1; k < nrl; ++k)
#pragma unroll
            for (int j = 0; j < 4; ++j) { a1[j] += red[0][threadIdx.x + k * cg][j]; a2[j] += red[1][threadIdx.x + k * cg][j]; }
        float* row = part + (size_t)blockIdx.x * 2 * d;
        *reinterpret_cast<float4*>(row + c0) = make_float4(a1[0], a1[1], a1[2], a1[3]);
        *reinterpret_cast<float4*>(row + d + c0) = make_float4(a2[0], a2[1], a2[2], a2[3]);
    }
}
__global__ __launch_bounds__(256) void bn_silu_bwd_apply_kernel(const float* __restrict__ z, const __bf16* __restrict__ dc3,
                                                                int64_t n_rows, int d, const float* __restrict__ bn_sum,
                                                                const float* __restrict__ bn_sumsq, const float* __restrict__ gamma,
                                                                const float* __restrict__ beta, float eps, const float* __restrict__ S1,
                                                                const float* __restrict__ S2, float* __restrict__ dz) {
    const int64_t total4 = n_rows * d / 4;
    const float inv_n = 1.f / (float)n_rows;
    for (int64_t i = (int64_t)blockIdx.x * 256 + threadIdx.x; i < total4; i += (int64_t)gridDim.x * 256) {
        const int c0 = (int)((i * 4) % d);
        const float4 zz = reinterpret_cast<const float4*>(z)[i];
        union { uint2 u; __bf16 h[4]; } g;
        g.u = reinterpret_cast<const uint2*>(dc3)[i];
        const float zv[4] = {zz.x, zz.y, zz.z, zz.w};
        float o[4];
#pragma unroll
        for (int j = 0; j < 4; ++j) {
            const float mean = bn_sum[c0 + j] * inv_n;
            const float rstd = rsqrtf(fmaxf(bn_sumsq[c0 + j] * inv_n - mean * mean, 0.f) + eps);
            const float xh = (zv[j] - mean) * rstd;
            const float dyb = (float)g.h[j] * silu_grad(xh * gamma[c0 + j] + beta[c0 + j]);
            o[j] = gamma[c0 + j] * rstd * (dyb - S1[c0 + j] * inv_n - xh * S2[c0 + j] * inv_n);
        }
        reinterpret_cast<float4*>(dz)[i] = make_float4(o[0], o[1], o[2], o[3]);
    }
}

template <int MODE>
__global__ __launch_bounds__(256) void glu_kernel(const __bf16* __restrict__ c2, const float* __restrict__ dG,
                                                  const int64_t* __restrict__ lens, int B, int T, int d,
                                                  float* __restrict__ G, __bf16* __restrict__ dc2) {
    const int64_t total = (int64_t)B * T * d;
    for (int64_t i = (int64_t)blockIdx.x * 256 + threadIdx.x; i < total; i += (int64_t)gridDim.x * 256) {
        const int c = (int)(i % d);
        const int64_t row = i / d;
        const int t = (int)(row % T), b = (int)(row / T);
        const bool valid = t < (int)lens[b];
        const float a = (float)c2[row * 2 * d + c], g = (float)c2[row * 2 * d + d + c];
        const float sg = ia_sigmoid_fast(g);
        if (MODE == 0) {
            G[i] = valid ? a * sg : 0.f;
        } else {
            const float dg = valid ? dG[i] : 0.f;
            dc2[row * 2 * d + c] = (__bf16)(dg * sg);
            dc2[row * 2 * d + d + c] = (__bf16)(dg * a * sg * (1.f - sg));
        }
    }
}

inline int ew_grid(int64_t items) {
    const int64_t b = (items + 255) / 256;
    return (int)(b < 1 ? 1 : (b > 8192 ? 8192 : b));
}

inline int lnb_blocks(int N) {
    const int b = (N + 7) / 8;
    return b < 1 ? 1 : (b > 1024 ? 1024 : b);
}
}

extern "C" int64_t ia_layernorm_bwd_scratch_elems(int N, int d) { return (N <= 0 || d <= 0) ? 0 : (int64_t)lnb_blocks(N) * 2 * d; }

extern "C" int ia_layernorm_bwd(const float* x, int ldx, const float* dy_f32, const void* dy_bf16, int ldy, int N, int d,
                                const float* gamma, float eps, const float* dx_in, float* dx_out, int lddx, float* dgamma,
                                float* dbeta, float* scratch, ia_stream_t stream) {
    return ia_layernorm_bwd_drop(x, ldx, dy_f32, dy_bf16, ldy, N, d, gamma, eps, dx_in, dx_out, lddx, dgamma, dbeta, 1.f, 0.f, 0,
                                 nullptr, 0, scratch, stream);
}

extern "C" int ia_layernorm_bwd_drop(const float* x, int ldx, const float* dy_f32, const void* dy_bf16, int ldy, int N, int d,
                                     const float* gamma, float eps, const float* dx_in, float* dx_out, int lddx, float* dgamma,
                                     float* dbeta, float alpha, float dropout_p, unsigned seed, void* dx_bf16, int lddxh,
                                     float* scratch, ia_stream_t stream) {
    if (!x || (!dy_f32 && !dy_bf16) || !gamma || !dx_out || ((dgamma == nullptr) != (dbeta == nullptr)) || !scratch || N <= 0 || d <= 0)
        return IA_INVALID_VALUE;
    if (d % 4 != 0 || d > 1024 || ldx % 4 != 0 || ldy % 4 != 0 || lddx % 4 != 0) return IA_UNSUPPORTED;
    if (dx_bf16 && (d % 8 != 0 || lddxh % 4 != 0 || dropout_p < 0.f || dropout_p >= 1.f)) return IA_INVALID_VALUE;
    static const bool split = [] { const char* e = getenv("IA_LN_DROP"); return e && e[0] == '0'; }();
    if (split && dx_bf16) {
        const int st0 = ia_layernorm_bwd_drop(x, ldx, dy_f32, dy_bf16, ldy, N, d, gamma, eps, dx_in, dx_out, lddx, dgamma, dbeta, 1.f, 0.f,
                                              0, nullptr, 0, scratch, stream);
        if (st0 != IA_OK) return st0;
        if (lddx != d || lddxh != d) return IA_UNSUPPORTED;
        return ia_scale_dropout_bf16(dx_out, N, d, alpha, dropout_p, seed, dx_bf16, stream);
    }
    const auto [hthr, hks] = ia_dropout_rule(dropout_p);
    const int G = lnb_blocks(N);
    const dim3 grid(G), blk(256);
    hipStream_t st = (hipStream_t)stream;
    const int nv = (d + 255) / 256;
#define IA_LNB(NV) hipLaunchKernelGGL((layernorm_bwd_kernel<NV>), grid, blk, 0, st, x, ldx, dy_f32, (const __bf16*)dy_bf16, ldy, N, d, gamma, eps, dx_in, dx_out, lddx, scratch, (__bf16*)dx_bf16, lddxh, alpha, seed, hthr, hks)
    switch (nv) {
        case 1: IA_LNB(1); break;
        case 2: IA_LNB(2); break;
        case 3: IA_LNB(3); break;
        default: IA_LNB(4); break;
    }
#undef IA_LNB
    IA_RETURN_IF_LAUNCH_FAILED();
    if (!dgamma) return IA_OK;
    ia_partials_finish(scratch, G, 2 * d, d, dgamma, dbeta, st);
    IA_RETURN_IF_LAUNCH_FAILED();
    return IA_OK;
}

extern "C" int ia_layernorm_bwd_partial_rows(int N) { return N > 0 ? lnb_blocks(N) : 0; }

namespace {
struct FinishJobs { ia_finish_job j[8]; int first_block[9]; int n; };
__global__ __launch_bounds__(1024) void partials_finish_multi_kernel(FinishJobs f) {
    __shared__ float red[16][64];
    int k = 0;
    while (k + 1 < f.n && (int)blockIdx.x >= f.first_block[k + 1]) ++k;
    const ia_finish_job J = f.j[k];
    const int cl = threadIdx.x & 63, rg = threadIdx.x >> 6;
    const int c = ((int)blockIdx.x - f.first_block[k]) * 64 + cl;
    float a0 = 0.f, a1 = 0.f;
    if (c < J.C) {
        int r = rg;
        for (; r + 112 < J.G; r += 128) {
            float v[8];
#pragma unroll
            for (int q = 0; q < 8; ++q) v[q] = J.part[(size_t)(r + 16 * q) * J.C + c];
            a0 += (v[0] + v[2]) + (v[4] + v[6]);
            a1 += (v[1] + v[3]) + (v[5] + v[7]);
        }
        for (; r < J.G; r += 16) a0 += J.part[(size_t)r * J.C + c];
    }
    red[rg][cl] = a0 + a1;
    __syncthreads();
    if (rg == 0 && c < J.C) {
        float s = 0.f;
#pragma unroll
        for (int q = 0; q < 16; ++q) s += red[q][cl];
        if (c < J.C0) J.out0[c] = s; else J.out1[c - J.C0] = s;
    }
}
}

extern "C" int ia_partials_finish_multi(const ia_finish_job* jobs, int count, ia_stream_t stream) {
    if (!jobs || count <= 0 || count > 8) return IA_INVALID_VALUE;
    FinishJobs f;
    f.n = count;
    int blocks = 0;
    for (int i = 0; i < count; ++i) {
        const ia_finish_job& J = jobs[i];
        if (!J.part || !J.out0 || J.G <= 0 || J.C <= 0 || J.C0 < 0 || J.C0 > J.C || (J.C0 < J.C && !J.out1)) return IA_INVALID_VALUE;
        f.j[i] = J;
        f.first_block[i] = blocks;
        blocks += (J.C + 63) / 64;
    }
    f.first_block[count] = blocks;
    hipLaunchKernelGGL(partials_finish_multi_kernel, dim3(blocks), dim3(1024), 0, (hipStream_t)stream, f);
    IA_RETURN_IF_LAUNCH_FAILED();
    return IA_OK;
}

extern "C" int ia_silu_dropout(const void* h_pre, int64_t M, int N, float dropout_p, unsigned seed, void* out, ia_stream_t stream) {
    if (!h_pre || !out || M <= 0 || N <= 0 || N % 8 != 0 || dropout_p < 0.f || dropout_p >= 1.f) return IA_INVALID_VALUE;
    const auto [thr, ks] = ia_dropout_rule(dropout_p);
    hipLaunchKernelGGL((silu_dropout_kernel<0>), dim3(ew_grid(M * (N / 8))), dim3(256), 0, (hipStream_t)stream,
                       (const __bf16*)h_pre, (const __bf16*)nullptr, M, N, seed, thr, ks, (__bf16*)out);
    IA_RETURN_IF_LAUNCH_FAILED();
    return IA_OK;
}

extern "C" int ia_silu_dropout_bwd(const void* h_pre, const void* dh, int64_t M, int N, float dropout_p, unsigned seed, void* out,
                                   ia_stream_t stream) {
    if (!h_pre || !dh || !out || M <= 0 || N <= 0 || N % 8 != 0 || dropout_p < 0.f || dropout_p >= 1.f) return IA_INVALID_VALUE;
    const auto [thr, ks] = ia_dropout_rule(dropout_p);
    hipLaunchKernelGGL((silu_dropout_kernel<1>), dim3(ew_grid(M * (N / 8))), dim3(256), 0, (hipStream_t)stream,
                       (const __bf16*)h_pre, (const __bf16*)dh, M, N, seed, thr, ks, (__bf16*)out);
    IA_RETURN_IF_LAUNCH_FAILED();
    return IA_OK;
}

extern "C" int ia_scale_dropout_bf16(const float* dy, int64_t M, int N, float alpha, float dropout_p, unsigned seed, void* out,
                                     ia_stream_t stream) {
    if (!dy || !out || M <= 0 || N <= 0 || N % 8 != 0 || dropout_p < 0.f || dropout_p >= 1.f) return IA_INVALID_VALUE;
    const auto [thr, ks] = ia_dropout_rule(dropout_p);
    hipLaunchKernelGGL(scale_dropout_bf16_kernel, dim3(ew_grid(M * (N / 8))), dim3(256), 0, (hipStream_t)stream, dy, M, N, alpha,
                       seed, thr, ks, (__bf16*)out);
    IA_RETURN_IF_LAUNCH_FAILED();
    return IA_OK;
}

namespace {
__global__ __launch_bounds__(256) void cast_pad_bf16_kernel(const float* __restrict__ src, int lds, int64_t M, int N,
                                                            __bf16* __restrict__ dst, int ldd) {
    const int vpr = ldd / 8;
    const int64_t total = M * vpr;
    for (int64_t i = (int64_t)blockIdx.x * 256 + threadIdx.x; i < total; i += (int64_t)gridDim.x * 256) {
        const int64_t m = i / vpr;
        const int n0 = (int)(i - m * vpr) * 8;
        const float* s = src + m * lds + n0;
        union { uint4 u; __bf16 h[8]; } o;
#pragma unroll
        for (int j = 0; j < 8; ++j) o.h[j] = (__bf16)((n0 + j < N) ? s[j] : 0.f);
        *reinterpret_cast<uint4*>(dst + m * ldd + n0) = o.u;
    }
}
}

extern "C" int ia_cast_pad_bf16(const float* src, int lds, int64_t M, int N, void* dst, int ldd, ia_stream_t stream) {
    if (!src || !dst || M <= 0 || N <= 0 || lds < N || ldd < N || ldd % 8 != 0 || !ia_is_aligned(dst, 16)) return IA_INVALID_VALUE;
    hipLaunchKernelGGL(cast_pad_bf16_kernel, dim3(ew_grid(M * (ldd / 8))), dim3(256), 0, (hipStream_t)stream, src, lds, M, N,
                       (__bf16*)dst, ldd);
    IA_RETURN_IF_LAUNCH_FAILED();
    return IA_OK;
}

namespace {
inline int bnb_rows_per_block(int64_t n_rows) {
    int64_t rpb = (n_rows + 1023) / 1024;
    return (int)(rpb < 32 ? 32 : rpb);
}
}

extern "C" int64_t ia_bn_silu_bwd_scratch_elems(int64_t n_rows, int d) {
    if (n_rows <= 0 || d <= 0) return 0;
    const int rpb = bnb_rows_per_block(n_rows);
    return ((n_rows + rpb - 1) / rpb) * 2 * (int64_t)d;
}

extern "C" int ia_bn_silu_bwd(const float* z, const void* dc3, int64_t n_rows, int d, const float* bn_sum, const float* bn_sumsq,
                              const float* gamma, const float* beta, float eps, float* S1, float* S2, float* dz,
                              float* scratch, ia_stream_t stream) {
    if (!z || !dc3 || !bn_sum || !bn_sumsq || !gamma || !beta || !S1 || !S2 || !dz || !scratch || n_rows <= 1 || d <= 0)
        return IA_INVALID_VALUE;
    if (d % 4 != 0 || d > 1024) return IA_UNSUPPORTED;
    hipStream_t st = (hipStream_t)stream;
    const int rpb = bnb_rows_per_block(n_rows);
    const int G = (int)((n_rows + rpb - 1) / rpb);
    hipLaunchKernelGGL(bn_silu_bwd_reduce_kernel, dim3((unsigned)G), dim3(256), 0, st, z, (const __bf16*)dc3, n_rows, d, bn_sum,
                       bn_sumsq, gamma, beta, eps, scratch, rpb);
    IA_RETURN_IF_LAUNCH_FAILED();
    ia_partials_finish(scratch, G, 2 * d, d, S1, S2, st);
    IA_RETURN_IF_LAUNCH_FAILED();
    hipLaunchKernelGGL(bn_silu_bwd_apply_kernel, dim3(ew_grid(n_rows * d / 4)), dim3(256), 0, st, z, (const __bf16*)dc3, n_rows, d,
                       bn_sum, bn_sumsq, gamma, beta, eps, S1, S2, dz);
    IA_RETURN_IF_LAUNCH_FAILED();
    return IA_OK;
}

extern "C" int ia_bn_silu_bwd_reduce(const float* z, const void* dc3, int64_t n_rows, int d, const float* bn_sum,
                                     const float* bn_sumsq, const float* gamma, const float* beta, float eps, float* S1, float* S2,
                                     float* scratch, ia_stream_t stream) {
    if (!z || !dc3 || !bn_sum || !bn_sumsq || !gamma || !beta || !S1 || !S2 || !scratch || n_rows <= 1 || d <= 0)
        return IA_INVALID_VALUE;
    if (d % 4 != 0 || d > 1024) return IA_UNSUPPORTED;
    hipStream_t st = (hipStream_t)stream;
    const int rpb = bnb_rows_per_block(n_rows);
    const int G = (int)((n_rows + rpb - 1) / rpb);
    hipLaunchKernelGGL(bn_silu_bwd_reduce_kernel, dim3((unsigned)G), dim3(256), 0, st, z, (const __bf16*)dc3, n_rows, d, bn_sum,
                       bn_sumsq, gamma, beta, eps, scratch, rpb);
    IA_RETURN_IF_LAUNCH_FAILED();
    ia_partials_finish(scratch, G, 2 * d, d, S1, S2, st);
    IA_RETURN_IF_LAUNCH_FAILED();
    return IA_OK;
}

extern "C" int ia_bn_silu_bwd_apply(const float* z, const void* dc3, int64_t n_rows, int d, const float* bn_sum,
                                    const float* bn_sumsq, const float* gamma, const float* beta, float eps, const float* S1,
                                    const float* S2, float* dz, ia_stream_t stream) {
    if (!z || !dc3 || !bn_sum || !bn_sumsq || !gamma || !beta || !S1 || !S2 || !dz || n_rows <= 1 || d <= 0) return IA_INVALID_VALUE;
    if (d % 4 != 0) return IA_UNSUPPORTED;
    hipLaunchKernelGGL(bn_silu_bwd_apply_kernel, dim3(ew_grid(n_rows * d / 4)), dim3(256), 0, (hipStream_t)stream, z,
                       (const __bf16*)dc3, n_rows, d, bn_sum, bn_sumsq, gamma, beta, eps, S1, S2, dz);
    IA_RETURN_IF_LAUNCH_FAILED();
    return IA_OK;
}

extern "C" int ia_glu_mask(const void* c2, const int64_t* lens, int B, int T, int d, float* G, ia_stream_t stream) {
    if (!c2 || !lens || !G || B <= 0 || T <= 0 || d <= 0) return IA_INVALID_VALUE;
    hipLaunchKernelGGL((glu_kernel<0>), dim3(ew_grid((int64_t)B * T * d)), dim3(256), 0, (hipStream_t)stream, (const __bf16*)c2,
                       (const float*)nullptr, lens, B, T, d, G, (__bf16*)nullptr);
    IA_RETURN_IF_LAUNCH_FAILED();
    return IA_OK;
}

extern "C" int ia_glu_bwd(const void* c2, const float* dG, const int64_t* lens, int B, int T, int d, void* dc2, ia_stream_t stream) {
    if (!c2 || !dG || !lens || !dc2 || B <= 0 || T <= 0 || d <= 0) return IA_INVALID_VALUE;
    hipLaunchKernelGGL((glu_kernel<1>), dim3(ew_grid((int64_t)B * T * d)), dim3(256), 0, (hipStream_t)stream, (const __bf16*)c2, dG,
                       lens, B, T, d, (float*)nullptr, (__bf16*)dc2);
    IA_RETURN_IF_LAUNCH_FAILED();
    return IA_OK;
}
```

indic_cl_asr_amd/csrc/gemm_tn.hip:

```cpp
#include <hip/hip_bf16.h>

#include "ia_common.h"
#include "lds_transpose.h"
#include "partials.h"

namespace {

typedef __bf16 bf8 __attribute__((ext_vector_type(8)));
typedef __bf16 bf4 __attribute__((ext_vector_type(4)));
typedef float f4 __attribute__((ext_vector_type(4)));

constexpr int TN_BN = 128;
constexpr int TN_BK = 128;
constexpr int TN_MS = 64;
constexpr int TN_ROWB = 256;
constexpr int TN_TILE = TN_MS * TN_ROWB;


__device__ __forceinline__ bool tn_map(int local, int tiles, int S, int* tile, int* split) {
    const int xcd = local & 7, slot = local >> 3;
    if (S >= 8) {
        *split = (slot / tiles) * 8 + xcd; *tile = slot % tiles;
        return *split < S;
    }
    const int G = 8 / S;
    *split = xcd % S; *tile = slot * G + xcd / S;
    return *tile < tiles;
}
inline int tn_round_splits(int s) { return s >= 8 ? s / 8 * 8 : (s >= 4 ? 4 : (s >= 2 ? 2 : 1)); }
inline int tn_plan_splits(int M, int wanted, int* rps_out) {
    int S = tn_round_splits(wanted < 1 ? 1 : wanted);
    for (;;) {
        int rps = (M + S - 1) / S;
        rps = (rps + TN_MS - 1) / TN_MS * TN_MS;
        const int Seff = (M + rps - 1) / rps;
        if (Seff >= 8 || Seff == tn_round_splits(Seff)) { *rps_out = rps; return Seff; }
        S = tn_round_splits(Seff);
    }
}
inline int tn_wgs(int tiles, int S) { return S >= 8 ? 8 * ((S + 7) / 8) * tiles : 8 * ((tiles + 8 / S - 1) / (8 / S)); }

__device__ __forceinline__ void tn_tile_body(const __bf16* __restrict__ dY, int ldy, const __bf16* __restrict__ X, int ldx, int M,
                                             int n, int k, int rows_per_split, float* __restrict__ part,
                                             float* __restrict__ part_b, size_t row_stride, int tile, int split,
                                             unsigned char* smem) {
    unsigned char* sY = smem;
    unsigned char* sX = smem + TN_TILE;
    const unsigned ldsY = (unsigned)(size_t)((__attribute__((address_space(3))) unsigned char*)sY);
    const unsigned ldsX = ldsY + TN_TILE;
    const int tid = threadIdx.x, lane = tid & 63, wave = tid >> 6;
    const int c = lane & 15, q4 = lane >> 4;
    const int wn = wave >> 1, wk = wave & 1;
    const int ntk = (k + TN_BK - 1) / TN_BK;
    const int n0 = (tile / ntk) * TN_BN, k0 = (tile % ntk) * TN_BK;
    const int m_beg = split * rows_per_split;
    int m_end = m_beg + rows_per_split; m_end = m_end < M ? m_end : M;
    const bool do_bias = part_b != nullptr && k0 == 0 && wk == 0;

    f4 acc[4][4], accb[4];
#pragma unroll
    for (int i = 0; i < 4; ++i) {
        accb[i] = (f4){0.f, 0.f, 0.f, 0.f};
#pragma unroll
        for (int j = 0; j < 4; ++j) acc[i][j] = (f4){0.f, 0.f, 0.f, 0.f};
    }
    bf8 ones;
#pragma unroll
    for (int j = 0; j < 8; ++j) ones[j] = (__bf16)1.f;

    auto multiply_stage = [&](unsigned lY, unsigned lX) {
#pragma unroll
        for (int ks = 0; ks < TN_MS / 32; ++ks) {
            bf4 alo[4], ahi[4], blo[4], bhi[4];
#pragma unroll
            for (int i = 0; i < 4; ++i) {
                unsigned a0, a1;
                trl_frag_addr<false>(lY, TN_ROWB, ks * 32 + q4 * 8, wn * 64 + i * 16, lane, &a0, &a1);
                alo[i] = trl_read<bf4>(a0); ahi[i] = trl_read<bf4>(a1);
                trl_frag_addr<false>(lX, TN_ROWB, ks * 32 + q4 * 8, wk * 64 + i * 16, lane, &a0, &a1);
                blo[i] = trl_read<bf4>(a0); bhi[i] = trl_read<bf4>(a1);
            }
            asm volatile("s_waitcnt lgkmcnt(0)"
                         : "+v"(alo[0]), "+v"(alo[1]), "+v"(alo[2]), "+v"(alo[3]), "+v"(ahi[0]), "+v"(ahi[1]), "+v"(ahi[2]),
                           "+v"(ahi[3]), "+v"(blo[0]), "+v"(blo[1]), "+v"(blo[2]), "+v"(blo[3]), "+v"(bhi[0]), "+v"(bhi[1]),
                           "+v"(bhi[2]), "+v"(bhi[3])
                         :
                         : "memory");
            bf8 af[4], bfr[4];
#pragma unroll
            for (int i = 0; i < 4; ++i) { af[i] = trl_join(alo[i], ahi[i]); bfr[i] = trl_join(blo[i], bhi[i]); }
#pragma unroll
            for (int i = 0; i < 4; ++i) {
#pragma unroll
                for (int j = 0; j < 4; ++j) acc[i][j] = __builtin_amdgcn_mfma_f32_16x16x32_bf16(af[i], bfr[j], acc[i][j], 0, 0, 0);
                if (do_bias) accb[i] = __builtin_amdgcn_mfma_f32_16x16x32_bf16(af[i], ones, accb[i], 0, 0, 0);
            }
        }
    };

    const bool dma_path = n0 + TN_BN <= n && k0 + TN_BK <= k && (m_end - m_beg) % TN_MS == 0 && m_end > m_beg;
    if (dma_path) {
        const unsigned char* gy = reinterpret_cast<const unsigned char*>(dY + (size_t)m_beg * ldy + n0);
        const unsigned char* gx = reinterpret_cast<const unsigned char*>(X + (size_t)m_beg * ldx + k0);
        const int wv = __builtin_amdgcn_readfirstlane(wave);
        unsigned oy[4], ox[4];
#pragma unroll
        for (int i = 0; i < 4; ++i) {
            const int row = 4 * (wv * 4 + i) + (lane >> 4);
            const unsigned ch = (unsigned)((lane & 15) ^ (((lane >> 4) << 2) | i));
            oy[i] = (unsigned)row * (unsigned)(ldy * 2) + ch * 16u;
            ox[i] = (unsigned)row * (unsigned)(ldx * 2) + ch * 16u;
        }
        auto issue = [&](int st, int buf) {
            const unsigned char* py = gy + (size_t)st * TN_MS * ldy * 2;
            const unsigned char* px = gx + (size_t)st * TN_MS * ldx * 2;
            unsigned char* dy_ = smem + buf * 2 * TN_TILE + wv * 4096;
#pragma unroll
            for (int i = 0; i < 4; ++i)
                __builtin_amdgcn_global_load_lds((const __attribute__((address_space(1))) void*)(py + oy[i]),
                                                 (__attribute__((address_space(3))) void*)(dy_ + i * 1024), 16, 0, 0);
#pragma unroll
            for (int i = 0; i < 4; ++i)
                __builtin_amdgcn_global_load_lds((const __attribute__((address_space(1))) void*)(px + ox[i]),
                                                 (__attribute__((address_space(3))) void*)(dy_ + TN_TILE + i * 1024), 16, 0, 0);
        };
        const int nst = (m_end - m_beg) / TN_MS;
        issue(0, 0);
        for (int st = 0; st < nst; ++st) {
            asm volatile("s_waitcnt vmcnt(0)" ::: "memory");
            __builtin_amdgcn_s_barrier();
            if (st + 1 < nst) issue(st + 1, (st + 1) & 1);
            const unsigned base = ldsY + (unsigned)((st & 1) * 2 * TN_TILE);
            multiply_stage(base, base + TN_TILE);
        }
    } else {
    uint4 ry[4], rx[4];
#define TN_LOAD(m0_)                                                                                               \
    do {                                                                                                           \
        _Pragma("unroll") for (int i = 0; i < 4; ++i) {                                                            \
            const int idx_ = tid + 256 * i, row_ = idx_ >> 4, ch_ = idx_ & 15;                                     \
            const int m_ = (m0_) + row_;                                                                           \
            const bool okm_ = m_ < m_end;                                                                          \
            const int cy_ = n0 + ch_ * 8, cx_ = k0 + ch_ * 8;                                                      \
            ry[i] = (okm_ && cy_ < n) ? *reinterpret_cast<const uint4*>(dY + (size_t)m_ * ldy + cy_) : make_uint4(0, 0, 0, 0); \
            rx[i] = (okm_ && cx_ < k) ? *reinterpret_cast<const uint4*>(X + (size_t)m_ * ldx + cx_) : make_uint4(0, 0, 0, 0);  \
        }                                                                                                          \
    } while (0)
#define TN_STORE()                                                                                                 \
    do {                                                                                                           \
        _Pragma("unroll") for (int i = 0; i < 4; ++i) {                                                            \
            const int idx_ = tid + 256 * i, row_ = idx_ >> 4, ch_ = idx_ & 15;                                     \
            *reinterpret_cast<uint4*>(sY + trl_off<false>(TN_ROWB, row_, ch_)) = ry[i];                                             \
            *reinterpret_cast<uint4*>(sX + trl_off<false>(TN_ROWB, row_, ch_)) = rx[i];                                             \
        }                                                                                                          \
    } while (0)

    TN_LOAD(m_beg);
    for (int m0 = m_beg; m0 < m_end; m0 += TN_MS) {
        __syncthreads();
        TN_STORE();
        __syncthreads();
        if (m0 + TN_MS < m_end) TN_LOAD(m0 + TN_MS);
        multiply_stage(ldsY, ldsX);
    }
    }
#undef TN_LOAD
#undef TN_STORE
    float* prow = part + (size_t)split * row_stride;
#pragma unroll
    for (int i = 0; i < 4; ++i)
#pragma unroll
        for (int r = 0; r < 4; ++r) {
            const int gn = n0 + wn * 64 + i * 16 + q4 * 4 + r;
            if (gn < n) {
#pragma unroll
                for (int j = 0; j < 4; ++j) {
                    const int gk = k0 + wk * 64 + j * 16 + c;
                    if (gk < k) prow[(size_t)gn * k + gk] = acc[i][j][r];
                }
                if (do_bias && c == 0) part_b[(size_t)split * row_stride + gn] = accb[i][r];
            }
        }
}

__global__ __launch_bounds__(256, 2) void gemm_tn_kernel(const __bf16* __restrict__ dY, int ldy, const __bf16* __restrict__ X,
                                                         int ldx, int M, int n, int k, int rows_per_split,
                                                         float* __restrict__ part, float* __restrict__ part_b,
                                                         size_t row_stride) {
    __shared__ __attribute__((aligned(16))) unsigned char smem[4 * TN_TILE];
    const int tiles = ((n + TN_BN - 1) / TN_BN) * ((k + TN_BK - 1) / TN_BK);
    const int S = (M + rows_per_split - 1) / rows_per_split;
    int tile, split;
    if (!tn_map((int)blockIdx.x, tiles, S, &tile, &split)) return;
    tn_tile_body(dY, ldy, X, ldx, M, n, k, rows_per_split, part, part_b, row_stride, tile, split, smem);
}

constexpr int TN_MAX_GROUP = 12;
struct TnProblem {
    const __bf16* dY; const __bf16* X; float* part; float* part_b; float* dW; float* db;
    size_t row_stride; int ldy, ldx, M, n, k, rps, S, tiles, wg_begin; int64_t out_begin;
};
struct TnGroup { TnProblem p[TN_MAX_GROUP]; int count; };

__global__ __launch_bounds__(256, 2) void gemm_tn_grouped_kernel(TnGroup g) {
    __shared__ __attribute__((aligned(16))) unsigned char smem[4 * TN_TILE];
    int pi = 0;
#pragma unroll
    for (int i = 1; i < TN_MAX_GROUP; ++i)
        if (i < g.count && (int)blockIdx.x >= g.p[i].wg_begin) pi = i;
    pi = __builtin_amdgcn_readfirstlane(pi);
    const TnProblem& P = g.p[pi];
    int tile, split;
    if (!tn_map((int)blockIdx.x - P.wg_begin, P.tiles, P.S, &tile, &split)) return;
    tn_tile_body(P.dY, P.ldy, P.X, P.ldx, P.M, P.n, P.k, P.rps, P.part, P.part_b, P.row_stride, tile, split, smem);
}

__global__ __launch_bounds__(256) void gemm_tn_grouped_finish_kernel(TnGroup g, int64_t total4) {
    for (int64_t i = (int64_t)blockIdx.x * 256 + threadIdx.x; i < total4; i += (int64_t)gridDim.x * 256) {
        const int64_t e = i * 4;
        int pi = 0;
#pragma unroll
        for (int j = 1; j < TN_MAX_GROUP; ++j)
            if (j < g.count && e >= g.p[j].out_begin) pi = j;
        const TnProblem& P = g.p[pi];
        const int64_t off = e - P.out_begin;
        const int64_t nk = (int64_t)P.n * P.k;
        if (off >= nk && !P.db) continue;
        float4 a = make_float4(0.f, 0.f, 0.f, 0.f);
        const float* src = P.part + off;
        for (int s_ = 0; s_ < P.S; ++s_) {
            const float4 x = *reinterpret_cast<const float4*>(src + (size_t)s_ * P.row_stride);
            a.x += x.x; a.y += x.y; a.z += x.z; a.w += x.w;
        }
        float* dst = off < nk ? P.dW + off : P.db + (off - nk);
        *reinterpret_cast<float4*>(dst) = a;
    }
}

inline int tn_splits(int M, int n, int k) {
    const int tiles = ((n + TN_BN - 1) / TN_BN) * ((k + TN_BK - 1) / TN_BK);
    int s = (320 + tiles - 1) / tiles;
    const int cap = (M + TN_MS - 1) / TN_MS;
    s = s < 1 ? 1 : (s > cap ? cap : s);
    return s;
}
}

extern "C" int64_t ia_gemm_tn_scratch_elems(int M, int n, int k) {
    if (M <= 0 || n <= 0 || k <= 0) return 0;
    return (int64_t)tn_splits(M, n, k) * ((int64_t)n * k + n);
}

extern "C" int ia_gemm_tn_bf16(const void* dY, int ldy, const void* X, int ldx, int M, int n, int k, float* dW, float* db,
                               float* scratch, ia_stream_t stream) {
    if (!dY || !X || !dW || !scratch || M <= 0 || n <= 0 || k <= 0) return IA_INVALID_VALUE;
    if (n % 8 != 0 || k % 8 != 0 || ldy % 8 != 0 || ldx % 8 != 0 || !ia_is_aligned(dY, 16) || !ia_is_aligned(X, 16)) return IA_UNSUPPORTED;
    int rps;
    const int Seff = tn_plan_splits(M, tn_splits(M, n, k), &rps);
    const size_t row_stride = (size_t)n * k + n;
    float* part = scratch;
    float* part_b = db ? scratch + (size_t)n * k : nullptr;
    hipStream_t st = (hipStream_t)stream;
    const dim3 grid(tn_wgs(((n + TN_BN - 1) / TN_BN) * ((k + TN_BK - 1) / TN_BK), Seff)), blk(256);
    hipLaunchKernelGGL(gemm_tn_kernel, grid, blk, 0, st, (const __bf16*)dY, ldy, (const __bf16*)X, ldx, M, n, k, rps, part, part_b,
                       row_stride);
    IA_RETURN_IF_LAUNCH_FAILED();
    if (db == dW + (size_t)n * k) {
        ia_partials_finish_wide(part, Seff, (int64_t)row_stride, dW, st);
    } else {
        ia_partials_finish_wide_strided(part, Seff, (int64_t)n * k, (int64_t)row_stride, dW, st);
        if (db) {
            IA_RETURN_IF_LAUNCH_FAILED();
            ia_partials_finish_wide_strided(part_b, Seff, (int64_t)n, (int64_t)row_stride, db, st);
        }
    }
    IA_RETURN_IF_LAUNCH_FAILED();
    return IA_OK;
}

namespace {
inline int tn_group_plan(const ia_tn_problem* pr, int count, TnGroup* g, int64_t* scratch_elems, int64_t* out_elems, int* blocks) {
    if (!pr || count <= 0 || count > TN_MAX_GROUP) return IA_INVALID_VALUE;
    int tiles_total = 0;
    for (int i = 0; i < count; ++i) {
        const ia_tn_problem& q = pr[i];
        if (q.M <= 0 || q.n <= 0 || q.k <= 0) return IA_INVALID_VALUE;
        if (q.n % 8 != 0 || q.k % 8 != 0 || q.ldy % 8 != 0 || q.ldx % 8 != 0) return IA_UNSUPPORTED;
        tiles_total += ((q.n + TN_BN - 1) / TN_BN) * ((q.k + TN_BK - 1) / TN_BK);
    }
    int S0 = 512 / tiles_total;
    S0 = S0 < 1 ? 1 : S0;
    int64_t so = 0, oo = 0;
    int wg = 0;
    g->count = count;
    for (int i = 0; i < count; ++i) {
        const ia_tn_problem& q = pr[i];
        TnProblem& P = g->p[i];
        const int cap = (q.M + TN_MS - 1) / TN_MS;
        int rps;
        const int S = tn_plan_splits(q.M, S0 > cap ? cap : S0, &rps);
        P.dY = (const __bf16*)q.dY; P.X = (const __bf16*)q.X; P.ldy = q.ldy; P.ldx = q.ldx; P.M = q.M; P.n = q.n; P.k = q.k;
        P.rps = rps; P.S = S; P.tiles = ((q.n + TN_BN - 1) / TN_BN) * ((q.k + TN_BK - 1) / TN_BK);
        P.row_stride = (size_t)q.n * q.k + q.n;
        P.part = nullptr; P.part_b = nullptr;
        P.dW = q.dW; P.db = q.db;
        P.wg_begin = wg; wg += tn_wgs(P.tiles, S);
        P.out_begin = oo; oo += (int64_t)P.row_stride;
        P.part = reinterpret_cast<float*>(so * sizeof(float));
        so += (int64_t)S * (int64_t)P.row_stride;
        so = (so + 3) / 4 * 4;
    }
    *scratch_elems = so; *out_elems = oo; *blocks = wg;
    return IA_OK;
}
}

extern "C" int64_t ia_gemm_tn_grouped_scratch_elems(const ia_tn_problem* problems, int count) {
    TnGroup g; int64_t so = 0, oo = 0; int blocks = 0;
    if (tn_group_plan(problems, count, &g, &so, &oo, &blocks) != IA_OK) return 0;
    return so;
}

extern "C" int ia_gemm_tn_bf16_grouped(const ia_tn_problem* problems, int count, float* scratch, ia_stream_t stream) {
    if (!scratch) return IA_INVALID_VALUE;
    TnGroup g; int64_t so = 0, oo = 0; int blocks = 0;
    const int rc = tn_group_plan(problems, count, &g, &so, &oo, &blocks);
    if (rc != IA_OK) return rc;
    for (int i = 0; i < count; ++i) {
        TnProblem& P = g.p[i];
        if (!P.dY || !P.X || !P.dW || !ia_is_aligned(P.dY, 16) || !ia_is_aligned(P.X, 16) || !ia_is_aligned(P.dW, 16) ||
            (P.db && !ia_is_aligned(P.db, 16)))
            return IA_INVALID_VALUE;
        P.part = scratch + reinterpret_cast<size_t>(P.part) / sizeof(float);
        P.part_b = P.db ? P.part + (size_t)P.n * P.k : nullptr;
    }
    hipStream_t st = (hipStream_t)stream;
    hipLaunchKernelGGL(gemm_tn_grouped_kernel, dim3(blocks), dim3(256), 0, st, g);
    IA_RETURN_IF_LAUNCH_FAILED();
    const int64_t total4 = oo / 4;
    const int64_t fb = (total4 + 255) / 256;
    hipLaunchKernelGGL(gemm_tn_grouped_finish_kernel, dim3((unsigned)(fb < 2048 ? fb : 2048)), dim3(256), 0, st, g, total4);
    IA_RETURN_IF_LAUNCH_FAILED();
    return IA_OK;
}
```

indic_cl_asr_amd/csrc/partials.h:

```cpp
#pragma once
#include <hip/hip_runtime.h>

namespace {
__global__ __launch_bounds__(1024) void ia_partials_finish_kernel(const float* __restrict__ part, int G, int C, int C0,
                                                                  float* __restrict__ out0, float* __restrict__ out1) {
    __shared__ float red[16][64];
    const int cl = threadIdx.x & 63, rg = threadIdx.x >> 6;
    const int c = blockIdx.x * 64 + cl;
    float a0 = 0.f, a1 = 0.f;
    if (c < C) {
        int r = rg;
        for (; r + 112 < G; r += 128) {
            float v[8];
#pragma unroll
            for (int k = 0; k < 8; ++k) v[k] = part[(size_t)(r + 16 * k) * C + c];
            a0 += (v[0] + v[2]) + (v[4] + v[6]);
            a1 += (v[1] + v[3]) + (v[5] + v[7]);
        }
        for (; r < G; r += 16) a0 += part[(size_t)r * C + c];
    }
    red[rg][cl] = a0 + a1;
    __syncthreads();
    if (rg == 0 && c < C) {
        float s = 0.f;
#pragma unroll
        for (int k = 0; k < 16; ++k) s += red[k][cl];
        if (c < C0) out0[c] = s; else out1[c - C0] = s;
    }
}

__global__ __launch_bounds__(256) void ia_partials_finish_wide_kernel(const float* __restrict__ part, int G, int64_t C4,
                                                                      int64_t S4, float* __restrict__ out) {
    for (int64_t i = (int64_t)blockIdx.x * 256 + threadIdx.x; i < C4; i += (int64_t)gridDim.x * 256) {
        const float4* p = reinterpret_cast<const float4*>(part) + i;
        float4 a = make_float4(0.f, 0.f, 0.f, 0.f), b = a;
        int g = 0;
        for (; g + 1 < G; g += 2) {
            const float4 x = p[(int64_t)g * S4], y = p[(int64_t)(g + 1) * S4];
            a.x += x.x; a.y += x.y; a.z += x.z; a.w += x.w;
            b.x += y.x; b.y += y.y; b.z += y.z; b.w += y.w;
        }
        if (g < G) { const float4 x = p[(int64_t)g * S4]; a.x += x.x; a.y += x.y; a.z += x.z; a.w += x.w; }
        reinterpret_cast<float4*>(out)[i] = make_float4(a.x + b.x, a.y + b.y, a.z + b.z, a.w + b.w);
    }
}

inline void ia_partials_finish_wide_strided(const float* part, int G, int64_t C, int64_t stride, float* out, hipStream_t st) {
    const int64_t c4 = C / 4, blocks = (c4 + 255) / 256;
    hipLaunchKernelGGL(ia_partials_finish_wide_kernel, dim3((unsigned)(blocks < 4096 ? blocks : 4096)), dim3(256), 0, st, part, G,
                       c4, stride / 4, out);
}
inline void ia_partials_finish_wide(const float* part, int G, int64_t C, float* out, hipStream_t st) {
    ia_partials_finish_wide_strided(part, G, C, C, out, st);
}

inline void ia_partials_finish(const float* part, int G, int C, int C0, float* out0, float* out1, hipStream_t st) {
    hipLaunchKernelGGL(ia_partials_finish_kernel, dim3((C + 63) / 64), dim3(1024), 0, st, part, G, C, C0, out0, out1);
}
}
```

Baseline: 3806 utterances/s.

## Fuse per-block weight-gradient finish reductions and grad accumulation into one commit kernel

Adds a single block_commit_kernel that, in the merged-wgrad path, performs the TN grouped GEMM split-K finish, the five layernorm partial column sums, the depthwise-conv weight-gradient finish, and the multi-add gradient accumulation in one launch instead of several separate kernels. The dwconv wgrad and grouped TN GEMM now have no-finish variants that leave partials in scratch (a new dwp workspace region) to be reduced later. The aim is to cut kernel launch count and tail/serialization overhead in each conformer block backward. In exchange, the kernel adds per-element range lookups against the add table, which costs extra ALU work, and the workspace grows.

```diff
diff --git a/include/indicasr.h b/include/indicasr.h
--- a/include/indicasr.h
+++ b/include/indicasr.h
@@ -149,6 +149,8 @@
                       ia_stream_t stream);
 int ia_dwconv_glu_wgrad(const void* c2, const int64_t* lens, const float* dy, int B, int T, int d, int ksz, float* dw, float* db,
                         float* scratch, ia_stream_t stream);
+int ia_dwconv_glu_wgrad_partials(const void* c2, const int64_t* lens, const float* dy, int B, int T, int d, int ksz,
+                                 float* scratch, int* rows_out, int* kmax_out, ia_stream_t stream);
 int ia_bn_silu(const float* z, int64_t n_rows, int d, const float* bn_sum, const float* bn_sumsq, const float* gamma,
                const float* beta, float* running_mean, float* running_var, int64_t* num_batches_tracked,
                float momentum, float eps, int training, void* out, ia_stream_t stream);
@@ -225,6 +227,14 @@
 } ia_tn_problem;
 int64_t ia_gemm_tn_grouped_scratch_elems(const ia_tn_problem* problems, int count);
 int ia_gemm_tn_bf16_grouped(const ia_tn_problem* problems, int count, float* scratch, ia_stream_t stream);
+typedef struct ia_tn_finish_item {
+    const float* part; float* dW; float* db;
+    int64_t out_begin, nk, row_stride;
+    int S;
+} ia_tn_finish_item;
+int ia_gemm_tn_bf16_grouped_nofinish(const ia_tn_problem* problems, int count, float* scratch, ia_stream_t stream);
+int ia_gemm_tn_grouped_finish_plan(const ia_tn_problem* problems, int count, float* scratch, ia_tn_finish_item* items,
+                                   int64_t* out_elems);
 int64_t ia_gemm_tn_scratch_elems(int M, int n, int k);
 int ia_gemm_tn_bf16(const void* dY, int ldy, const void* X, int ldx, int M, int n, int k, float* dW, float* db,
                     float* scratch, ia_stream_t stream);
@@ -307,6 +317,9 @@
 typedef struct ia_finish_job { const float* part; int G, C, C0; float* out0; float* out1; } ia_finish_job;
 int ia_layernorm_bwd_partial_rows(int N);
 int ia_partials_finish_multi(const ia_finish_job* jobs, int count, ia_stream_t stream);
+int ia_conformer_block_commit(const ia_tn_problem* problems, int n_problems, float* tn_scratch, const ia_finish_job* ln_jobs,
+                              int n_ln, const float* dw_part, int dw_rows, int dw_kmax, int d, int ksz, float* dw_w, float* dw_b,
+                              const void* add_table, int n_add, ia_stream_t stream);
 int64_t ia_layernorm_bwd_scratch_elems(int N, int d);
 int ia_silu_dropout(const void* h_pre, int64_t M, int N, float dropout_p, unsigned seed, void* out, ia_stream_t stream);
 int ia_silu_dropout_bwd(const void* h_pre, const void* dh, int64_t M, int N, float dropout_p, unsigned seed, void* out,
diff --git a/indic_cl_asr_amd/_lib.py b/indic_cl_asr_amd/_lib.py
--- a/indic_cl_asr_amd/_lib.py
+++ b/indic_cl_asr_amd/_lib.py
@@ -168,6 +168,10 @@
     "ia_conformer_block_bwd_a": (_i, [_vp, _vp, _vp, _vp, _vp, _i, _i, _c.c_uint, _vp, _sz, _vp, _vp, _vp]),
     "ia_conformer_block_bwd_a_phase": (_i, [_vp, _vp, _vp, _vp, _vp, _i, _i, _c.c_uint, _vp, _sz, _vp, _vp, _i, _vp, _vp]),
     "ia_conformer_block_bwd_b": (_i, [_vp, _vp, _vp, _vp, _vp, _i, _vp, _vp, _i, _i, _c.c_uint, _vp, _sz, _vp, _vp, _i, _vp]),
+    "ia_gemm_tn_bf16_grouped_nofinish": (_i, [_vp, _i, _vp, _vp]),
+    "ia_gemm_tn_grouped_finish_plan": (_i, [_vp, _i, _vp, _vp, _vp]),
+    "ia_dwconv_glu_wgrad_partials": (_i, [_vp, _vp, _vp, _i, _i, _i, _i, _vp, _vp, _vp, _vp]),
+    "ia_conformer_block_commit": (_i, [_vp, _i, _vp, _vp, _i, _vp, _i, _i, _i, _i, _vp, _vp, _vp, _i, _vp]),
     "ia_layernorm_bwd": (_i, [_vp, _i, _vp, _vp, _i, _i, _i, _vp, _f, _vp, _vp, _i, _vp, _vp, _vp, _vp]),
     "ia_layernorm_bwd_drop": (_i, [_vp, _i, _vp, _vp, _i, _i, _i, _vp, _f, _vp, _vp, _i, _vp, _vp, _f, _f, _c.c_uint, _vp, _i, _vp, _vp]),
     "ia_layernorm_bwd_partial_rows": (_i, [_i]),
diff --git a/indic_cl_asr_amd/csrc/block_train.hip b/indic_cl_asr_amd/csrc/block_train.hip
--- a/indic_cl_asr_amd/csrc/block_train.hip
+++ b/indic_cl_asr_amd/csrc/block_train.hip
@@ -6,6 +6,7 @@
 #include <cstdlib>
 
 #include "ia_common.h"
+#include "partials.h"
 
 namespace {
 
@@ -108,8 +109,128 @@
     }
 }
 
+constexpr int CM_MAX_TN = 12, CM_MAX_LN = 8, CM_MAX_ROWS = 64;
+struct CommitArgs {
+    ia_tn_finish_item tn[CM_MAX_TN];
+    ia_finish_job ln[CM_MAX_LN];
+    int ln_first[CM_MAX_LN + 1];
+    int n_tn, n_ln;
+    int64_t tn_total4;
+    const float* dw_part; float* dw_w; float* dw_b;
+    int dw_G, d, kmax, ksz;
+    const AddRow* table; int n_add;
+    int b_dw, b_direct, b_tn;
+};
+struct CommitRows { const float* src[CM_MAX_ROWS]; float* dst[CM_MAX_ROWS]; int64_t n[CM_MAX_ROWS]; int count; };
+
+__device__ __forceinline__ int commit_row(const CommitRows& R, const float* a) {
+    int found = -1;
+    for (int k = 0; k < R.count; ++k) {
+        const float* s = R.src[k];
+        found = (a >= s && a < s + R.n[k]) ? k : found;
+    }
+    return found;
+}
+__device__ __forceinline__ void commit1(const CommitRows& R, float* a, float v) {
+    const int k = commit_row(R, a);
+    if (k < 0) *a = v;
+    else R.dst[k][a - R.src[k]] += v;
+}
+__device__ __forceinline__ void commit4(const CommitRows& R, float* a, float4 v) {
+    const int k = commit_row(R, a);
+    if (k < 0 && commit_row(R, a + 3) < 0) { *reinterpret_cast<float4*>(a) = v; return; }
+    if (k >= 0 && a + 3 < R.src[k] + R.n[k]) {
+        float* g = R.dst[k] + (a - R.src[k]);
+        if ((reinterpret_cast<uintptr_t>(g) & 15) == 0) {
+            float4 x = *reinterpret_cast<float4*>(g);
+            x.x += v.x; x.y += v.y; x.z += v.z; x.w += v.w;
+            *reinterpret_cast<float4*>(g) = x;
+        } else {
+            g[0] += v.x; g[1] += v.y; g[2] += v.z; g[3] += v.w;
+        }
+        return;
+    }
+    commit1(R, a, v.x); commit1(R, a + 1, v.y); commit1(R, a + 2, v.z); commit1(R, a + 3, v.w);
+}
+__device__ __forceinline__ bool commit_reduced(const CommitArgs& A, const float* p) {
+    for (int i = 0; i < A.n_tn; ++i) {
+        const ia_tn_finish_item& P = A.tn[i];
+        if (p >= P.dW && p < P.dW + P.nk) return true;
+        if (P.db && p >= P.db && p < P.db + (P.row_stride - P.nk)) return true;
+    }
+    for (int i = 0; i < A.n_ln; ++i) {
+        const ia_finish_job& J = A.ln[i];
+        if (p >= J.out0 && p < J.out0 + J.C0) return true;
+        if (J.out1 && p >= J.out1 && p < J.out1 + (J.C - J.C0)) return true;
+    }
+    if (A.dw_part) {
+        if (p >= A.dw_w && p < A.dw_w + (size_t)A.d * A.ksz) return true;
+        if (A.dw_b && p >= A.dw_b && p < A.dw_b + A.d) return true;
+    }
+    return false;
+}
+
+__global__ __launch_bounds__(1024) void block_commit_kernel(CommitArgs A) {
+    __shared__ CommitRows R;
+    __shared__ float red[16][64];
+    __shared__ int direct[CM_MAX_ROWS];
+    const int tid = threadIdx.x, b = blockIdx.x;
+    if (tid < A.n_add) {
+        const AddRow r = A.table[tid];
+        R.src[tid] = r.src; R.dst[tid] = r.dst; R.n[tid] = r.n;
+    }
+    if (tid == 0) R.count = A.n_add;
+    __syncthreads();
+    if (b < A.b_dw) {
+        int k = 0;
+        while (k + 1 < A.n_ln && b >= A.ln_first[k + 1]) ++k;
+        const ia_finish_job J = A.ln[k];
+        const int cl = tid & 63, rg = tid >> 6;
+        const int c = (b - A.ln_first[k]) * 64 + cl;
+        red[rg][cl] = c < J.C ? ia_colsum_share(J.part, J.G, J.C, c, rg) : 0.f;
+        __syncthreads();
+        if (rg == 0 && c < J.C) commit1(R, c < J.C0 ? J.out0 + c : J.out1 + (c - J.C0), ia_colsum_join(red, cl));
+    } else if (b < A.b_direct) {
+        const int q = tid >> 8, t = tid & 255, o = t & 31, sl = t >> 5;
+        const int idx = ((b - A.b_dw) * 4 + q) * 32 + o, total = (A.kmax + 1) * A.d;
+        float (*rd)[32] = reinterpret_cast<float (*)[32]>(&red[q * 4][0]);
+        rd[sl][o] = idx < total ? ia_dwsum_share(A.dw_part, A.dw_G, total, idx, sl) : 0.f;
+        __syncthreads();
+        if (sl != 0 || idx >= total) return;
+        const float s = ia_dwsum_join(rd, o);
+        const int jj = idx / A.d, c = idx - jj * A.d;
+        if (jj == A.kmax) {
+            if (A.dw_b) commit1(R, A.dw_b + c, s);
+        } else {
+            const int j = jj - ((A.kmax - 1) / 2 - (A.ksz - 1) / 2);
+            if (j >= 0 && j < A.ksz) commit1(R, A.dw_w + c * A.ksz + j, s);
+        }
+    } else if (b < A.b_tn) {
+        if (tid < R.count) direct[tid] = commit_reduced(A, R.src[tid]) ? 0 : 1;
+        __syncthreads();
+        for (int k = 0; k < R.count; ++k) {
+            if (!direct[k]) continue;
+            for (int64_t i = tid; i < R.n[k]; i += 1024) R.dst[k][i] += R.src[k][i];
+        }
+    } else {
+        const int64_t stride = (int64_t)(gridDim.x - A.b_tn) * 1024;
+        for (int64_t i = (int64_t)(b - A.b_tn) * 1024 + tid; i < A.tn_total4; i += stride) {
+            const int64_t e = i * 4;
+            int pi = 0;
+#pragma unroll
+            for (int j = 1; j < CM_MAX_TN; ++j)
+                if (j < A.n_tn && e >= A.tn[j].out_begin) pi = j;
+            const ia_tn_finish_item& P = A.tn[pi];
+            const int64_t off = e - P.out_begin;
+            if (off >= P.nk && !P.db) continue;
+            const float4 a = ia_split_sum4(P.part + off, P.S, (size_t)P.row_stride);
+            commit4(R, off < P.nk ? P.dW + off : P.db + (off - P.nk), a);
+        }
+    }
+}
+
 struct BwdWs {
-    size_t dxa, dxb, dB, dB1, dB2, dB3, dh, dhp, dy, dc3, dz, dG, dc2, dctx, wt, scr, total;
+    size_t dxa, dxb, dB, dB1, dB2, dB3, dh, dhp, dy, dc3, dz, dG, dc2, dctx, wt, scr, dwp, total;
 };
 
 size_t max3(size_t a, size_t b, size_t c) { return a > b ? (a > c ? a : c) : (b > c ? b : c); }
@@ -158,6 +279,7 @@
         scr = scr > (size_t)ia_gemm_tn_grouped_scratch_elems(gall, 9) ? scr : (size_t)ia_gemm_tn_grouped_scratch_elems(gall, 9);
     }
     w.scr = o;  o = up256(o + scr * 4);
+    w.dwp = o;  o = up256(o + (size_t)ia_dwconv_scratch_elems(B, T, d, ksz) * 4);
     w.total = o;
     return w;
 }
@@ -211,13 +333,21 @@
     }
     return c.ok ? &c : nullptr;
 }
-struct PendingGroup { ia_tn_problem grp[8]; int n = 0; const void* ws = nullptr; };
+struct PendingGroup {
+    ia_tn_problem grp[8]; int n = 0; const void* ws = nullptr;
+    bool commit = false;
+    int dw_rows = 0, dw_kmax = 0;
+};
 PendingGroup* pending_group() {
     static PendingGroup pg[16];
     int dev = 0;
     if (hipGetDevice(&dev) != hipSuccess || dev < 0 || dev >= 16) return nullptr;
     return &pg[dev];
 }
+bool block_plan_enabled() {
+    const char* e = getenv("IA_BLOCK_PLAN");
+    return !(e && e[0] == '0');
+}
 bool merged_wgrads() {
     const char* e = getenv("IA_TN_MERGE");
     return !(e && e[0] == '0') && tn_grouping_enabled();
@@ -239,6 +369,41 @@
     if (d <= 0 || H <= 0 || d % H != 0) return 0;
     const int dk = d / H;
     return (d % 8 == 0 && d <= 1024 && d_ff % 8 == 0 && ksz <= 31 && (ksz & 1) == 1 && dk <= 64 && dk % 4 == 0 && T >= 1) ? 1 : 0;
+}
+
+extern "C" int ia_conformer_block_commit(const ia_tn_problem* problems, int n_problems, float* tn_scratch, const ia_finish_job* ln_jobs,
+                                         int n_ln, const float* dw_part, int dw_rows, int dw_kmax, int d, int ksz, float* dw_w, float* dw_b,
+                                         const void* add_table, int n_add, ia_stream_t stream) {
+    if (n_problems < 0 || n_problems > CM_MAX_TN || n_ln < 0 || n_ln > CM_MAX_LN || n_add < 0 || n_add > CM_MAX_ROWS) return IA_INVALID_VALUE;
+    if ((n_problems > 0 && (!problems || !tn_scratch)) || (n_ln > 0 && !ln_jobs) || (n_add > 0 && !add_table)) return IA_INVALID_VALUE;
+    if (dw_part && (!dw_w || dw_rows <= 0 || dw_kmax <= 0 || d <= 0 || ksz <= 0 || ksz > dw_kmax)) return IA_INVALID_VALUE;
+    CommitArgs A{};
+    A.n_tn = n_problems; A.n_ln = n_ln;
+    int64_t out_elems = 0;
+    if (n_problems > 0) IA_TRY(ia_gemm_tn_grouped_finish_plan(problems, n_problems, tn_scratch, A.tn, &out_elems));
+    A.tn_total4 = out_elems / 4;
+    int blocks = 0;
+    for (int i = 0; i < n_ln; ++i) {
+        const ia_finish_job& J = ln_jobs[i];
+        if (!J.part || !J.out0 || J.G <= 0 || J.C <= 0 || J.C0 < 0 || J.C0 > J.C || (J.C0 < J.C && !J.out1)) return IA_INVALID_VALUE;
+        A.ln[i] = J;
+        A.ln_first[i] = blocks;
+        blocks += (J.C + 63) / 64;
+    }
+    A.ln_first[n_ln] = blocks;
+    A.b_dw = blocks;
+    A.dw_part = dw_part; A.dw_w = dw_w; A.dw_b = dw_b; A.dw_G = dw_rows; A.d = d; A.kmax = dw_kmax; A.ksz = ksz;
+    if (dw_part) blocks += ((dw_kmax + 1) * d + 127) / 128;
+    A.b_direct = blocks;
+    if (n_add > 0) blocks += 1;
+    A.b_tn = blocks;
+    const int64_t tb = (A.tn_total4 + 1023) / 1024;
+    blocks += (int)(tb < 1024 ? tb : 1024);
+    A.table = (const AddRow*)add_table; A.n_add = n_add;
+    if (blocks == 0) return IA_OK;
+    hipLaunchKernelGGL(block_commit_kernel, dim3(blocks), dim3(1024), 0, (hipStream_t)stream, A);
+    IA_RETURN_IF_LAUNCH_FAILED();
+    return IA_OK;
 }
 
 extern "C" int ia_conformer_block_fwd(const ia_block_params* Lp, const float* x0, const void* pos_emb, int pos_rows,
@@ -350,9 +515,14 @@
     IA_TRY(ia_dwconv_glu_bwd(dz, S.c2, lens, B, T, d, ksz, L.dw_w, dc2, stream));
     SideCtx* side = phase == 0 ? side_ctx() : nullptr;
     hipStream_t main = (hipStream_t)stream;
+    const bool merge = !side && phase == 0 && merged_wgrads() && pending_group();
+    const bool commit_later = merge && block_plan_enabled();
+    int dw_rows = 0, dw_kmax = 0;
     if (side) {
         IA_TRY(stream_after(main, side->s, side->ev[0]));
         IA_TRY(ia_dwconv_glu_wgrad(S.c2, lens, dz, B, T, d, ksz, G.dw_w, G.dw_b, scr, (ia_stream_t)side->s));
+    } else if (commit_later) {
+        IA_TRY(ia_dwconv_glu_wgrad_partials(S.c2, lens, dz, B, T, d, ksz, (float*)(ws + w.dwp), &dw_rows, &dw_kmax, stream));
     } else {
         IA_TRY(ia_dwconv_glu_wgrad(S.c2, lens, dz, B, T, d, ksz, G.dw_w, G.dw_b, scr, stream));
     }
@@ -365,10 +535,11 @@
         IA_TRY(flush_group(grp, ngrp, scr, (ia_stream_t)side->s));
         if (hipEventRecord(side->ev[2], side->s) != hipSuccess) return IA_LAUNCH_FAILED;
         side->a_pending = true;
-    } else if (phase == 0 && merged_wgrads() && pending_group()) {
+    } else if (merge) {
         PendingGroup* pg = pending_group();
         for (int i = 0; i < ngrp; ++i) pg->grp[i] = grp[i];
         pg->n = ngrp; pg->ws = workspace;
+        pg->commit = commit_later; pg->dw_rows = dw_rows; pg->dw_kmax = dw_kmax;
     } else {
         IA_TRY(flush_group(grp, ngrp, scr, stream));
     }
@@ -394,6 +565,8 @@
     const size_t lnp_set = (size_t)ia_layernorm_bwd_scratch_elems(N, d);
     PendingGroup* pg = pending_group();
     const bool carried = pg && pg->n > 0 && pg->ws == workspace;
+    const bool commit = carried && pg->commit;
+    const int dw_rows = commit ? pg->dw_rows : 0, dw_kmax = commit ? pg->dw_kmax : 0;
     void *dB = ws + (carried ? w.dB3 : w.dB), *dhp = ws + (carried ? w.dh : w.dhp), *dy = ws + w.dy, *wt = ws + w.wt;
     const float p = L.p_drop, pff = L.p_ff;
     ia_tn_problem grp[12];
@@ -440,19 +613,26 @@
     if (side) {
         IA_TRY(stream_after(main, side->s, side->ev[5]));
         stream = (ia_stream_t)side->s;
+    } else if (commit) {
+        IA_TRY(ia_gemm_tn_bf16_grouped_nofinish(grp, ngrp, scr, stream));
     } else {
         IA_TRY(flush_group(grp, ngrp, scr, stream));
     }
-    {
-        const int rows = ia_layernorm_bwd_partial_rows(N);
-        const ia_finish_job jobs[5] = {{lnp + 0 * lnp_set, rows, 2 * d, d, G.ln_out_g, G.ln_out_b},
-                                       {lnp + 1 * lnp_set, rows, 2 * d, d, G.ln_ff2_g, G.ln_ff2_b},
-                                       {lnp + 2 * lnp_set, rows, 2 * d, d, G.ln_conv_g, G.ln_conv_b},
-                                       {lnp + 3 * lnp_set, rows, 2 * d, d, G.ln_att_g, G.ln_att_b},
-                                       {lnp + 4 * lnp_set, rows, 2 * d, d, G.ln_ff1_g, G.ln_ff1_b}};
+    const int rows = ia_layernorm_bwd_partial_rows(N);
+    const ia_finish_job jobs[5] = {{lnp + 0 * lnp_set, rows, 2 * d, d, G.ln_out_g, G.ln_out_b},
+                                   {lnp + 1 * lnp_set, rows, 2 * d, d, G.ln_ff2_g, G.ln_ff2_b},
+                                   {lnp + 2 * lnp_set, rows, 2 * d, d, G.ln_conv_g, G.ln_conv_b},
+                                   {lnp + 3 * lnp_set, rows, 2 * d, d, G.ln_att_g, G.ln_att_b},
+                                   {lnp + 4 * lnp_set, rows, 2 * d, d, G.ln_ff1_g, G.ln_ff1_b}};
+    bool added = false;
+    if (commit) {
+        added = add_table && n_add > 0 && n_add <= CM_MAX_ROWS;
+        IA_TRY(ia_conformer_block_commit(grp, ngrp, scr, jobs, 5, (const float*)(ws + w.dwp), dw_rows, dw_kmax, d, ksz, G.dw_w, G.dw_b,
+                                         added ? add_table : nullptr, added ? n_add : 0, stream));
+    } else {
         IA_TRY(ia_partials_finish_multi(jobs, 5, stream));
     }
-    if (add_table && n_add > 0) {
+    if (add_table && n_add > 0 && !added) {
         hipLaunchKernelGGL(multi_add_kernel, dim3(64, n_add < 64 ? n_add : 64), dim3(256), 0, (hipStream_t)stream,
                            (const AddRow*)add_table, n_add);
         IA_RETURN_IF_LAUNCH_FAILED();
diff --git a/indic_cl_asr_amd/csrc/dwconv.hip b/indic_cl_asr_amd/csrc/dwconv.hip
--- a/indic_cl_asr_amd/csrc/dwconv.hip
+++ b/indic_cl_asr_amd/csrc/dwconv.hip
@@ -166,16 +166,10 @@
     __shared__ float red[8][32];
     const int o = threadIdx.x & 31, sl = threadIdx.x >> 5;
     const int idx = blockIdx.x * 32 + o, total = (kmax + 1) * d;
-    float a0 = 0.f, a1 = 0.f;
-    if (idx < total) {
-        int g = sl;
-        for (; g + 8 < G; g += 16) { a0 += part[(size_t)g * total + idx]; a1 += part[(size_t)(g + 8) * total + idx]; }
-        for (; g < G; g += 8) a0 += part[(size_t)g * total + idx];
-    }
-    red[sl][o] = a0 + a1;
+    red[sl][o] = idx < total ? ia_dwsum_share(part, G, total, idx, sl) : 0.f;
     __syncthreads();
     if (sl != 0 || idx >= total) return;
-    const float s = ((red[0][o] + red[1][o]) + (red[2][o] + red[3][o])) + ((red[4][o] + red[5][o]) + (red[6][o] + red[7][o]));
+    const float s = ia_dwsum_join(red, o);
     const int jj = idx / d, c = idx - jj * d;
     if (jj == kmax) {
         if (db) db[c] = s;
@@ -315,9 +309,9 @@
     return IA_OK;
 }
 
-extern "C" int ia_dwconv_glu_wgrad(const void* c2, const int64_t* lens, const float* dy, int B, int T, int d, int ksz, float* dw,
-                                   float* db, float* scratch, ia_stream_t stream) {
-    if (!c2 || !lens || !dy || !dw || !scratch || B <= 0 || T <= 0) return IA_INVALID_VALUE;
+extern "C" int ia_dwconv_glu_wgrad_partials(const void* c2, const int64_t* lens, const float* dy, int B, int T, int d, int ksz,
+                                            float* scratch, int* rows_out, int* kmax_out, ia_stream_t stream) {
+    if (!c2 || !lens || !dy || !scratch || !rows_out || !kmax_out || B <= 0 || T <= 0) return IA_INVALID_VALUE;
     if (!dw_shape_ok(d, ksz)) return IA_UNSUPPORTED;
     hipStream_t st = (hipStream_t)stream;
     const int ns = wgrad_splits(B, T, d), kmax = kmax_for(ksz);
@@ -330,7 +324,17 @@
     }
 #undef IA_DWG
     IA_RETURN_IF_LAUNCH_FAILED();
-    hipLaunchKernelGGL(dwconv_wgrad_finish_kernel, dim3(((kmax + 1) * d + 31) / 32), dim3(256), 0, st, scratch, (int)grid.x, d,
+    *rows_out = (int)grid.x; *kmax_out = kmax;
+    return IA_OK;
+}
+
+extern "C" int ia_dwconv_glu_wgrad(const void* c2, const int64_t* lens, const float* dy, int B, int T, int d, int ksz, float* dw,
+                                   float* db, float* scratch, ia_stream_t stream) {
+    if (!dw) return IA_INVALID_VALUE;
+    int rows = 0, kmax = 0;
+    const int rc = ia_dwconv_glu_wgrad_partials(c2, lens, dy, B, T, d, ksz, scratch, &rows, &kmax, stream);
+    if (rc != IA_OK) return rc;
+    hipLaunchKernelGGL(dwconv_wgrad_finish_kernel, dim3(((kmax + 1) * d + 31) / 32), dim3(256), 0, (hipStream_t)stream, scratch, rows, d,
                        kmax, ksz, dw, db);
     IA_RETURN_IF_LAUNCH_FAILED();
     return IA_OK;
diff --git a/indic_cl_asr_amd/csrc/encoder_bwd.hip b/indic_cl_asr_amd/csrc/encoder_bwd.hip
--- a/indic_cl_asr_amd/csrc/encoder_bwd.hip
+++ b/indic_cl_asr_amd/csrc/encoder_bwd.hip
@@ -318,24 +318,10 @@
     const ia_finish_job J = f.j[k];
     const int cl = threadIdx.x & 63, rg = threadIdx.x >> 6;
     const int c = ((int)blockIdx.x - f.first_block[k]) * 64 + cl;
-    float a0 = 0.f, a1 = 0.f;
-    if (c < J.C) {
-        int r = rg;
-        for (; r + 112 < J.G; r += 128) {
-            float v[8];
-#pragma unroll
-            for (int q = 0; q < 8; ++q) v[q] = J.part[(size_t)(r + 16 * q) * J.C + c];
-            a0 += (v[0] + v[2]) + (v[4] + v[6]);
-            a1 += (v[1] + v[3]) + (v[5] + v[7]);
-        }
-        for (; r < J.G; r += 16) a0 += J.part[(size_t)r * J.C + c];
-    }
-    red[rg][cl] = a0 + a1;
+    red[rg][cl] = c < J.C ? ia_colsum_share(J.part, J.G, J.C, c, rg) : 0.f;
     __syncthreads();
     if (rg == 0 && c < J.C) {
-        float s = 0.f;
-#pragma unroll
-        for (int q = 0; q < 16; ++q) s += red[q][cl];
+        const float s = ia_colsum_join(red, cl);
         if (c < J.C0) J.out0[c] = s; else J.out1[c - J.C0] = s;
     }
 }
diff --git a/indic_cl_asr_amd/csrc/gemm_tn.hip b/indic_cl_asr_amd/csrc/gemm_tn.hip
--- a/indic_cl_asr_amd/csrc/gemm_tn.hip
+++ b/indic_cl_asr_amd/csrc/gemm_tn.hip
@@ -226,12 +226,7 @@
         const int64_t off = e - P.out_begin;
         const int64_t nk = (int64_t)P.n * P.k;
         if (off >= nk && !P.db) continue;
-        float4 a = make_float4(0.f, 0.f, 0.f, 0.f);
-        const float* src = P.part + off;
-        for (int s_ = 0; s_ < P.S; ++s_) {
-            const float4 x = *reinterpret_cast<const float4*>(src + (size_t)s_ * P.row_stride);
-            a.x += x.x; a.y += x.y; a.z += x.z; a.w += x.w;
-        }
+        const float4 a = ia_split_sum4(P.part + off, P.S, P.row_stride);
         float* dst = off < nk ? P.dW + off : P.db + (off - nk);
         *reinterpret_cast<float4*>(dst) = a;
     }
@@ -321,19 +316,50 @@
     return so;
 }
 
-extern "C" int ia_gemm_tn_bf16_grouped(const ia_tn_problem* problems, int count, float* scratch, ia_stream_t stream) {
+namespace {
+inline int tn_group_bind(const ia_tn_problem* problems, int count, float* scratch, TnGroup* g, int64_t* out_elems, int* blocks) {
     if (!scratch) return IA_INVALID_VALUE;
-    TnGroup g; int64_t so = 0, oo = 0; int blocks = 0;
-    const int rc = tn_group_plan(problems, count, &g, &so, &oo, &blocks);
+    int64_t so = 0;
+    const int rc = tn_group_plan(problems, count, g, &so, out_elems, blocks);
     if (rc != IA_OK) return rc;
     for (int i = 0; i < count; ++i) {
-        TnProblem& P = g.p[i];
+        TnProblem& P = g->p[i];
         if (!P.dY || !P.X || !P.dW || !ia_is_aligned(P.dY, 16) || !ia_is_aligned(P.X, 16) || !ia_is_aligned(P.dW, 16) ||
             (P.db && !ia_is_aligned(P.db, 16)))
             return IA_INVALID_VALUE;
         P.part = scratch + reinterpret_cast<size_t>(P.part) / sizeof(float);
         P.part_b = P.db ? P.part + (size_t)P.n * P.k : nullptr;
     }
+    return IA_OK;
+}
+}
+
+extern "C" int ia_gemm_tn_bf16_grouped_nofinish(const ia_tn_problem* problems, int count, float* scratch, ia_stream_t stream) {
+    TnGroup g; int64_t oo = 0; int blocks = 0;
+    const int rc = tn_group_bind(problems, count, scratch, &g, &oo, &blocks);
+    if (rc != IA_OK) return rc;
+    hipLaunchKernelGGL(gemm_tn_grouped_kernel, dim3(blocks), dim3(256), 0, (hipStream_t)stream, g);
+    IA_RETURN_IF_LAUNCH_FAILED();
+    return IA_OK;
+}
+
+extern "C" int ia_gemm_tn_grouped_finish_plan(const ia_tn_problem* problems, int count, float* scratch, ia_tn_finish_item* items,
+                                              int64_t* out_elems) {
+    if (!items || !out_elems) return IA_INVALID_VALUE;
+    TnGroup g; int blocks = 0;
+    const int rc = tn_group_bind(problems, count, scratch, &g, out_elems, &blocks);
+    if (rc != IA_OK) return rc;
+    for (int i = 0; i < count; ++i) {
+        const TnProblem& P = g.p[i];
+        items[i] = ia_tn_finish_item{P.part, P.dW, P.db, P.out_begin, (int64_t)P.n * P.k, (int64_t)P.row_stride, P.S};
+    }
+    return IA_OK;
+}
+
+extern "C" int ia_gemm_tn_bf16_grouped(const ia_tn_problem* problems, int count, float* scratch, ia_stream_t stream) {
+    TnGroup g; int64_t oo = 0; int blocks = 0;
+    const int rc = tn_group_bind(problems, count, scratch, &g, &oo, &blocks);
+    if (rc != IA_OK) return rc;
     hipStream_t st = (hipStream_t)stream;
     hipLaunchKernelGGL(gemm_tn_grouped_kernel, dim3(blocks), dim3(256), 0, st, g);
     IA_RETURN_IF_LAUNCH_FAILED();
diff --git a/indic_cl_asr_amd/csrc/partials.h b/indic_cl_asr_amd/csrc/partials.h
--- a/indic_cl_asr_amd/csrc/partials.h
+++ b/indic_cl_asr_amd/csrc/partials.h
@@ -2,29 +2,53 @@
 #include <hip/hip_runtime.h>
 
 namespace {
+__device__ __forceinline__ float ia_colsum_share(const float* __restrict__ part, int G, int C, int c, int rg) {
+    float a0 = 0.f, a1 = 0.f;
+    int r = rg;
+    for (; r + 112 < G; r += 128) {
+        float v[8];
+#pragma unroll
+        for (int k = 0; k < 8; ++k) v[k] = part[(size_t)(r + 16 * k) * C + c];
+        a0 += (v[0] + v[2]) + (v[4] + v[6]);
+        a1 += (v[1] + v[3]) + (v[5] + v[7]);
+    }
+    for (; r < G; r += 16) a0 += part[(size_t)r * C + c];
+    return a0 + a1;
+}
+__device__ __forceinline__ float ia_colsum_join(const float (*red)[64], int cl) {
+    float s = 0.f;
+#pragma unroll
+    for (int k = 0; k < 16; ++k) s += red[k][cl];
+    return s;
+}
+__device__ __forceinline__ float4 ia_split_sum4(const float* __restrict__ src, int S, size_t row_stride) {
+    float4 a = make_float4(0.f, 0.f, 0.f, 0.f);
+    for (int s_ = 0; s_ < S; ++s_) {
+        const float4 x = *reinterpret_cast<const float4*>(src + (size_t)s_ * row_stride);
+        a.x += x.x; a.y += x.y; a.z += x.z; a.w += x.w;
+    }
+    return a;
+}
+__device__ __forceinline__ float ia_dwsum_share(const float* __restrict__ part, int G, int total, int idx, int sl) {
+    float a0 = 0.f, a1 = 0.f;
+    int g = sl;
+    for (; g + 8 < G; g += 16) { a0 += part[(size_t)g * total + idx]; a1 += part[(size_t)(g + 8) * total + idx]; }
+    for (; g < G; g += 8) a0 += part[(size_t)g * total + idx];
+    return a0 + a1;
+}
+__device__ __forceinline__ float ia_dwsum_join(const float (*red)[32], int o) {
+    return ((red[0][o] + red[1][o]) + (red[2][o] + red[3][o])) + ((red[4][o] + red[5][o]) + (red[6][o] + red[7][o]));
+}
+
 __global__ __launch_bounds__(1024) void ia_partials_finish_kernel(const float* __restrict__ part, int G, int C, int C0,
                                                                   float* __restrict__ out0, float* __restrict__ out1) {
     __shared__ float red[16][64];
     const int cl = threadIdx.x & 63, rg = threadIdx.x >> 6;
     const int c = blockIdx.x * 64 + cl;
-    float a0 = 0.f, a1 = 0.f;
-    if (c < C) {
-        int r = rg;
-        for (; r + 112 < G; r += 128) {
-            float v[8];
-#pragma unroll
-            for (int k = 0; k < 8; ++k) v[k] = part[(size_t)(r + 16 * k) * C + c];
-            a0 += (v[0] + v[2]) + (v[4] + v[6]);
-            a1 += (v[1] + v[3]) + (v[5] + v[7]);
-        }
-        for (; r < G; r += 16) a0 += part[(size_t)r * C + c];
-    }
-    red[rg][cl] = a0 + a1;
+    red[rg][cl] = c < C ? ia_colsum_share(part, G, C, c, rg) : 0.f;
     __syncthreads();
     if (rg == 0 && c < C) {
-        float s = 0.f;
-#pragma unroll
-        for (int k = 0; k < 16; ++k) s += red[k][cl];
+        const float s = ia_colsum_join(red, cl);
         if (c < C0) out0[c] = s; else out1[c - C0] = s;
     }
 }
```

Result: slower. 3743 utterances/s (-1.7%).
